# UCL-CCS/SCEMa

Hardware: AMD Instinct MI355X
Metric: stress_evals_per_sec (higher is better)
Workload: dtype f64; 1 GPU; 576 x PE-10368 OPLS replicas per update(), 10+100 MD steps each (dt 2 fs, 300 K, lj/cut/coul/long 12/9 + PPPM 1e-4 + SHAKE + NVT), persistent per-QP state, replica equilibrated for 2000 steps before the timed region; force_field=opls, strain_set=balanced (load/unload: odd updates take the draw with the opposite sign), n_sims=576, atoms_per_replica=10368, sims_on_rank0=576, allgathers=0

## Files before the change

include/scema_md.h:

```cpp
#ifndef SCEMA_MD_H
#define SCEMA_MD_H

#include <stdint.h>

#ifdef __cplusplus
extern "C" {
#endif

#define SCEMA_MD_OK 0
#define SCEMA_MD_ERR_ARG 1
#define SCEMA_MD_ERR_NOSTATE 2
#define SCEMA_MD_ERR_DEVICE 3
#define SCEMA_MD_ERR_BOX 4
#define SCEMA_MD_ERR_IO 5
#define SCEMA_MD_ERR_OVERFLOW 6

#define SCEMA_MD_NPART 8
#define SCEMA_MD_QP_NONE ((int32_t)0xFFFFFFFF)

typedef struct scema_md_engine scema_md_engine;

typedef struct {
  double cut_lj;
  double cut_coul;
// ... 106 lines not shown
int32_t scema_md_local_stress_count(const scema_md_engine *e);
int32_t scema_md_local_result_doubles(const scema_md_engine *e);
int scema_md_copy_local_stress(scema_md_engine *e, void *dst, int32_t dst_on_device);
int scema_md_scatter_gathered(scema_md_engine *e, const double *gathered, scema_mdsim *sims, int32_t n_sims);
int scema_md_settle_update(scema_md_engine *e, int32_t failed);
int64_t scema_md_unsettled_updates(const scema_md_engine *e);

typedef struct scema_plan_dir scema_plan_dir;
scema_plan_dir *scema_plan_dir_create(void);
void scema_plan_dir_destroy(scema_plan_dir *d);
int scema_plan_update(scema_plan_dir *d, const scema_mdsim *sims, int32_t n_sims, const double *cost, int32_t world,
                      int32_t *owner, int32_t *pos, int32_t *cap, int32_t *moves ,
                      int32_t *n_moves, int32_t commit);

int scema_md_has_state(const scema_md_engine *e, int32_t qp_id, const char *matid, int32_t replica);
int scema_md_get_state(scema_md_engine *e, int32_t qp_id, const char *matid, int32_t replica,
                       double box[9], double *x, double *v);
int scema_md_set_state(scema_md_engine *e, int32_t qp_id, const char *matid, int32_t replica,
                       const double box[9], const double *x, const double *v);
int scema_md_drop_state(scema_md_engine *e, int32_t qp_id, const char *matid, int32_t replica);
int scema_md_save_state_file(scema_md_engine *e, int32_t qp_id, const char *matid, int32_t replica, const char *path);
int scema_md_load_state_file(scema_md_engine *e, int32_t qp_id, const char *matid, int32_t replica, const char *path);
int scema_md_save_state_lammps(scema_md_engine *e, int32_t qp_id, const char *matid, int32_t replica, const char *path,
                               double timestep, int64_t ntimestep);

int scema_md_save_state_dump(scema_md_engine *e, int32_t qp_id, const char *matid, int32_t replica, const char *path,
                             int64_t ntimestep, int32_t precise);

typedef struct {
  double timestep_length;
  double temperature;
  int32_t nsteps_sample;
  double strain_ampl;
  double strain_rate;
} scema_md_eqparams;
int scema_md_init_material(scema_md_engine *e, const char *matid, int32_t replica, const scema_md_eqparams *p,
                           double length[3], double stress[6], double stiff[36]);

typedef struct {
  int32_t nsteps_equil;
  double timestep_length;
  double temperature;
  int64_t seed;
} scema_md_equilparams;
int scema_md_equilibrate(scema_md_engine *e, const char *matid, int32_t replica, const scema_md_equilparams *p, double length[3],
                         double *info);

int scema_md_debug_minimize(scema_md_engine *e, int32_t qp_id, const char *matid, int32_t replica, double etol, double ftol,
                            int32_t maxiter, int32_t maxeval, double *info);
int scema_md_debug_run_nh(scema_md_engine *e, int32_t qp_id, const char *matid, int32_t replica, int32_t nsteps, double dt,
                          double t_start, double t_stop, int32_t npt, double p_target, double p_period, double *lavg);
int scema_md_debug_compute(scema_md_engine *e, int32_t qp_id, const char *matid, int32_t replica, int32_t use_shake,
                           double *f, double *energies, double *virials, double *info );
int scema_md_debug_run(scema_md_engine *e, int32_t qp_id, const char *matid, int32_t replica, int32_t nsteps,
                       double dt, double temperature, int32_t nvt, int32_t use_shake, const double *rates,
                       double *press_avg);

int scema_md_reax_configure(scema_md_engine *e, const char *ffield_path, const char *const *elements, int32_t n_elements,
                            double qeq_tol, double skin);
int scema_md_reax_activate(scema_md_engine *e, int32_t on);
int scema_md_reax_set(scema_md_engine *e, int32_t exact_gradient, int32_t terms, int32_t qeq_maxiter);
int scema_md_reax_concurrency(scema_md_engine *e, int32_t halves, int32_t overlap);
int scema_md_batch_split(scema_md_engine *e, int32_t on);
int scema_md_get_concurrency(const scema_md_engine *e, int32_t *out);
int scema_md_pppm_tiling(scema_md_engine *e, int32_t mode, int32_t lds_bytes);
int scema_md_pppm_paths(const scema_md_engine *e, int32_t out[8]);
int scema_md_pppm_tile_shape(const int32_t grid[3], int32_t lds_bytes, int32_t which , int32_t out[4]);
int scema_md_pppm_plan_count(const scema_md_engine *e);
int scema_md_reax_debug_compute(scema_md_engine *e, int32_t qp_id, const char *matid, int32_t replica, double *f, double *eparts,
                                double *virial, double *q, double *info);
int scema_md_reax_stats(const scema_md_engine *e, double *out);

int scema_md_sw_configure(scema_md_engine *e, const char *matid, const char *sw_path, const char *const *elements, int32_t n_elements,
                          int32_t energy_unit, double skin);
int scema_md_sw_debug_compute(scema_md_engine *e, int32_t qp_id, const char *matid, int32_t replica, double *f, double *e2, double *e3,
                              double *virial, double *info);
int scema_md_sw_read_params(const char *sw_path, const char *const *elements, int32_t n_elements, int32_t energy_unit, int32_t *n_kept,
                            int32_t *type_map, double *values, char *errbuf, int32_t errcap);

int scema_md_tersoff_configure(scema_md_engine *e, const char *matid, const char *path, const char *const *elements, int32_t n_elements,
                               int32_t energy_unit, double skin);
int scema_md_tersoff_debug_compute(scema_md_engine *e, int32_t qp_id, const char *matid, int32_t replica, double *f, double *e_rep,
                                   double *e_att, double *virial, double *info);
int scema_md_tersoff_read_params(const char *path, const char *const *elements, int32_t n_elements, int32_t energy_unit, int32_t *n_kept,
                                 int32_t *type_map, double *values, char *errbuf, int32_t errcap);

int scema_md_tersoff_mod_configure(scema_md_engine *e, const char *matid, const char *path, const char *const *elements, int32_t n_elements,
                                   int32_t energy_unit, double skin);
int scema_md_tersoff_mod_debug_compute(scema_md_engine *e, int32_t qp_id, const char *matid, int32_t replica, double *f, double *e_rep,
                                       double *e_att, double *virial, double *info);
int scema_md_tersoff_zbl_configure(scema_md_engine *e, const char *matid, const char *path, const char *const *elements, int32_t n_elements,
                                   int32_t energy_unit, double skin);
int scema_md_tersoff_zbl_debug_compute(scema_md_engine *e, int32_t qp_id, const char *matid, int32_t replica, double *f, double *e_rep,
                                       double *e_att, double *virial, double *info);
int scema_md_tersoff_mod_read_params(const char *path, const char *const *elements, int32_t n_elements, int32_t energy_unit, int32_t *n_kept,
                                     int32_t *type_map, double *values, char *errbuf, int32_t errcap);
int scema_md_tersoff_zbl_read_params(const char *path, const char *const *elements, int32_t n_elements, int32_t energy_unit, int32_t *n_kept,
                                     int32_t *type_map, double *values, char *errbuf, int32_t errcap);

int scema_md_eam_configure(scema_md_engine *e, const char *matid, const char *path, const char *const *elements, int32_t n_elements,
                           int32_t energy_unit, double skin);
int scema_md_eam_debug_compute(scema_md_engine *e, int32_t qp_id, const char *matid, int32_t replica, double *f, double *e_pair,
                               double *e_embed, double *virial, double *info);
int scema_md_eam_read_setfl(const char *path, const char *const *elements, int32_t n_elements, int32_t energy_unit, int32_t *n_kept,
                            int32_t *type_map, double *head, double *masses, double *tables, int64_t tables_cap, char *errbuf, int32_t errcap);

// ... 48 lines not shown
```

scema_amd/capi.py:

```python
from __future__ import annotations

import ctypes as C
import os

import numpy as np

_HERE = os.path.dirname(os.path.abspath(__file__))
LIB_PATH = os.path.join(_HERE, os.environ.get("SCEMA_MD_LIB") or ("libscema_md_asan.so" if os.environ.get("SCEMA_SANITIZE") == "1" else "libscema_md.so"))

NPART = 8
PARTS = ["lj", "coul", "bond", "angle", "dihedral", "improper", "kspace", "shake"]
QP_NONE = -1

SYMBOLS = [
    "scema_md_default_params", "scema_md_create", "scema_md_destroy", "scema_md_last_error",
    "scema_md_register_replica", "scema_md_load_replica_file", "scema_md_write_replica_file",
    "scema_md_load_lammps_data", "scema_md_convert_lammps_data",
    "scema_md_probe_lammps_restart", "scema_md_read_lammps_restart_atoms", "scema_md_load_lammps_restart",
    "scema_md_convert_lammps_restart", "scema_md_write_lammps_restart",
    "scema_md_strain_batch", "scema_md_strain", "scema_md_local_stress_device_ptr",
    "scema_md_local_stress_count", "scema_md_local_result_doubles", "scema_md_copy_local_stress", "scema_md_scatter_gathered", "scema_md_settle_update", "scema_md_has_state", "scema_md_get_state",
    "scema_md_set_state", "scema_md_drop_state", "scema_md_save_state_file", "scema_md_load_state_file", "scema_md_save_state_lammps",
    "scema_md_init_material", "scema_md_debug_compute", "scema_md_debug_run", "scema_md_get_profile", "scema_md_env_overrides",
    "scema_md_comm_unique_id", "scema_md_comm_init_rccl", "scema_md_comm_init_host", "scema_md_comm_destroy",
    "scema_md_comm_world", "scema_md_comm_rank", "scema_md_comm_stats", "scema_md_comm_handshakes", "scema_md_state_owner", "scema_md_last_plan",
    "scema_plan_dir_create", "scema_plan_dir_destroy", "scema_plan_update", "scema_md_kspace_setup",
    "scema_md_save_state_dump", "scema_md_replica_natoms", "scema_md_save_replica_file", "scema_md_equilibrate", "scema_md_debug_minimize", "scema_md_debug_run_nh",
    "scema_md_reax_configure", "scema_md_reax_activate", "scema_md_reax_set", "scema_md_reax_concurrency", "scema_md_batch_split", "scema_md_get_concurrency", "scema_md_pppm_plan_count", "scema_md_pppm_tiling", "scema_md_pppm_paths", "scema_md_pppm_tile_shape", "scema_md_unsettled_updates", "scema_md_reax_debug_compute", "scema_md_reax_stats", "scema_md_box_fma_tflops",
    "scema_md_sw_configure", "scema_md_sw_debug_compute", "scema_md_sw_read_params",
    "scema_md_tersoff_configure", "scema_md_tersoff_debug_compute", "scema_md_tersoff_read_params",
    "scema_md_eam_configure", "scema_md_eam_debug_compute", "scema_md_eam_read_setfl",
    "scema_md_tersoff_mod_configure", "scema_md_tersoff_mod_debug_compute", "scema_md_tersoff_mod_read_params",
    "scema_md_tersoff_zbl_configure", "scema_md_tersoff_zbl_debug_compute", "scema_md_tersoff_zbl_read_params",
    "scema_md_vashishta_configure", "scema_md_vashishta_debug_compute", "scema_md_vashishta_read_params",
    "scema_md_adp_configure", "scema_md_adp_debug_compute", "scema_md_adp_read_setfl",
]
COMM_ID_BYTES = 128
HOST_ALLGATHER_FN = C.CFUNCTYPE(C.c_int, C.c_void_p, C.c_void_p, C.c_void_p, C.c_int64)
HOST_SEND_FN = C.CFUNCTYPE(C.c_int, C.c_void_p, C.c_void_p, C.c_int64, C.c_int32)
HOST_RECV_FN = C.CFUNCTYPE(C.c_int, C.c_void_p, C.c_void_p, C.c_int64, C.c_int32)


class EquilParams(C.Structure):
    _fields_ = [("nsteps_equil", C.c_int32), ("timestep_length", C.c_double), ("temperature", C.c_double), ("seed", C.c_int64)]


class Params(C.Structure):
    _fields_ = [("cut_lj", C.c_double), ("cut_coul", C.c_double), ("skin", C.c_double), ("neigh_delay", C.c_int32),
                ("kspace_accuracy", C.c_double), ("shake_tol", C.c_double), ("shake_maxiter", C.c_int32),
                ("shake_mass", C.c_double), ("t_period", C.c_double), ("t_chain", C.c_int32), ("device", C.c_int32),
                ("max_batch", C.c_int32), ("profile", C.c_int32), ("kspace_style", C.c_int32)]


_P = C.c_void_p


class System(C.Structure):
    _fields_ = [("natoms", C.c_int32), ("ntypes", C.c_int32), ("type", _P), ("charge", _P), ("mass", _P),
                ("eps", _P), ("sigma", _P),
                ("nbonds", C.c_int32), ("nbondtypes", C.c_int32), ("bond_atoms", _P), ("bond_type", _P), ("bond_coeff", _P),
                ("nangles", C.c_int32), ("nangletypes", C.c_int32), ("angle_atoms", _P), ("angle_type", _P), ("angle_coeff", _P),
                ("ndihedrals", C.c_int32), ("ndihedraltypes", C.c_int32), ("dihedral_atoms", _P), ("dihedral_type", _P),
                ("dihedral_coeff", _P),
                ("nimpropers", C.c_int32), ("nimpropertypes", C.c_int32), ("improper_atoms", _P), ("improper_type", _P),
                ("improper_coeff", _P),
                ("special_lj", C.c_double * 3), ("special_coul", C.c_double * 3), ("box", C.c_double * 9), ("x", _P), ("v", _P)]


class MDSim(C.Structure):
    _fields_ = [("qp_id", C.c_int32), ("most_recent_qp_id", C.c_int32), ("replica", C.c_int32), ("material", C.c_int32),
                ("matid", C.c_char_p), ("time_id", C.c_char_p), ("output_folder", C.c_char_p),
                ("restart_folder", C.c_char_p), ("scripts_folder", C.c_char_p), ("log_file", C.c_char_p),
                ("force_field", C.c_char_p),
                ("strain", C.c_double * 6), ("stiffness", C.c_double * 36),
                ("timestep_length", C.c_double), ("temperature", C.c_double), ("strain_rate", C.c_double),
                ("nsteps_sample", C.c_int32), ("output_homog", C.c_int32), ("checkpoint", C.c_int32),
# ... 264 lines not shown
        return bool(lib().scema_md_has_state(self.h, C.c_int32(qp), matid.encode(), C.c_int32(replica)))

    def natoms(self, matid, replica) -> int:
        if (matid, replica) not in self._natoms:
            n = int(lib().scema_md_replica_natoms(self.h, matid.encode(), C.c_int32(replica)))
            if n <= 0:
                raise EngineError(f"replica {matid}_{replica} is not registered")
            self._natoms[(matid, replica)] = n
        return self._natoms[(matid, replica)]

    def get_state(self, qp, matid, replica):
        n = self.natoms(matid, replica)
        box = np.zeros(9); x = np.zeros((n, 3)); v = np.zeros((n, 3))
        self._chk(lib().scema_md_get_state(self.h, C.c_int32(qp), matid.encode(), C.c_int32(replica), _p(box), _p(x), _p(v)))
        return box, x, v

    def set_state(self, qp, matid, replica, box, x, v):
        box = np.ascontiguousarray(box, np.float64); x = np.ascontiguousarray(x, np.float64); v = np.ascontiguousarray(v, np.float64)
        self._chk(lib().scema_md_set_state(self.h, C.c_int32(qp), matid.encode(), C.c_int32(replica), _p(box), _p(x), _p(v)))

    def drop_state(self, qp, matid, replica):
        self._chk(lib().scema_md_drop_state(self.h, C.c_int32(qp), matid.encode(), C.c_int32(replica)))

    def save_state_file(self, qp, matid, replica, path):
        self._chk(lib().scema_md_save_state_file(self.h, C.c_int32(qp), matid.encode(), C.c_int32(replica), path.encode()))

    def save_state_lammps(self, qp, matid, replica, path, timestep=2.0, ntimestep=0):
        self._chk(lib().scema_md_save_state_lammps(self.h, C.c_int32(qp), matid.encode(), C.c_int32(replica), path.encode(),
                                                   C.c_double(timestep), C.c_int64(ntimestep)))

    def save_state_dump(self, qp, matid, replica, path, ntimestep=0, precise=True):
        self._chk(lib().scema_md_save_state_dump(self.h, C.c_int32(qp), matid.encode(), C.c_int32(replica), path.encode(), C.c_int64(ntimestep),
                                                 C.c_int32(1 if precise else 0)))

    def load_state_file(self, qp, matid, replica, path):
        self._chk(lib().scema_md_load_state_file(self.h, C.c_int32(qp), matid.encode(), C.c_int32(replica), path.encode()))

    def debug_compute(self, matid, replica, qp=QP_NONE, use_shake=False):
        n = self._natoms[(matid, replica)]
        f = np.zeros((n, 3)); e = np.zeros(NPART); w = np.zeros((NPART, 6)); info = np.zeros(8)
        self._chk(lib().scema_md_debug_compute(self.h, C.c_int32(qp), matid.encode(), C.c_int32(replica),
                                               C.c_int32(1 if use_shake else 0), _p(f), _p(e), _p(w), _p(info)))
        return f, e, w, dict(g_ewald=info[0], nk=int(info[1]), npairs=info[2], tdof=info[3], t_current=info[4],
                             maxneigh_seen=int(info[5]), maxneigh=int(info[6]), nclus=int(info[7]))

    def debug_run(self, matid, replica, nsteps, dt, temperature, qp=QP_NONE, nvt=True, use_shake=True, rates=None, sample=False):
        r = None if rates is None else np.ascontiguousarray(rates, np.float64)
        pavg = np.zeros(6) if sample else None
        self._chk(lib().scema_md_debug_run(self.h, C.c_int32(qp), matid.encode(), C.c_int32(replica), C.c_int32(nsteps),
                                           C.c_double(dt), C.c_double(temperature), C.c_int32(1 if nvt else 0),
                                           C.c_int32(1 if use_shake else 0), _p(r), _p(pavg)))
        return pavg

    def init_material(self, matid, replica, dt=2.0, temperature=300.0, nss=100, strain_ampl=0.005, strain_rate=1e-4):
        p = EqParams(dt, temperature, nss, strain_ampl, strain_rate)
        length, stress, stiff = np.zeros(3), np.zeros(6), np.zeros(36)
        self._chk(lib().scema_md_init_material(self.h, matid.encode(), C.c_int32(replica), C.byref(p), _p(length), _p(stress), _p(stiff)))
        return length, stress, stiff.reshape(6, 6)

    def reax_configure(self, ffield: str, elements=("H", "C", "N", "O"), qeq_tol: float = 1e-6, skin: float = -1.0):
        arr = (C.c_char_p * len(elements))(*[e.encode() for e in elements])
        self._chk(lib().scema_md_reax_configure(self.h, ffield.encode(), arr, C.c_int32(len(elements)), C.c_double(qeq_tol), C.c_double(skin)))

    def reax_activate(self, on: bool = True):
        self._chk(lib().scema_md_reax_activate(self.h, C.c_int32(1 if on else 0)))

    def reax_set(self, exact_gradient: int = -1, terms: int = -1, qeq_maxiter: int = -1):
        self._chk(lib().scema_md_reax_set(self.h, C.c_int32(exact_gradient), C.c_int32(terms), C.c_int32(qeq_maxiter)))

    def reax_concurrency(self, halves: int = -1, overlap: int = -1):
        self._chk(lib().scema_md_reax_concurrency(self.h, C.c_int32(halves), C.c_int32(overlap)))

    def unsettled_updates(self) -> int:
        lib().scema_md_unsettled_updates.restype = C.c_int64
        return int(lib().scema_md_unsettled_updates(self.h))

    def batch_split(self, on: int = -1):
        self._chk(lib().scema_md_batch_split(self.h, C.c_int32(on)))

    def pppm_plan_count(self) -> int:
        lib().scema_md_pppm_plan_count.restype = C.c_int
        return int(lib().scema_md_pppm_plan_count(self.h))

    def pppm_tiling(self, mode: int = -1, lds_bytes: int = -1):
        self._chk(lib().scema_md_pppm_tiling(self.h, C.c_int32(mode), C.c_int32(lds_bytes)))

    def pppm_paths(self) -> dict:
        out = (C.c_int32 * 8)()
        self._chk(lib().scema_md_pppm_paths(self.h, out))
        return dict(spread=int(out[0]), force=int(out[1]), spread_tiles=(int(out[2]), int(out[3])), force_tiles=(int(out[4]), int(out[5])),
                    lds_bytes=int(out[6]), mode=int(out[7]))

    def concurrency(self) -> dict:
        out = (C.c_int32 * 3)()
        self._chk(lib().scema_md_get_concurrency(self.h, out))
        return dict(split=int(out[0]), reax_halves=int(out[1]), reax_overlap=int(out[2]))

    def reax_compute(self, matid, replica, qp=QP_NONE):
        n = self._natoms[(matid, replica)]
        f = np.zeros((n, 3)); e = np.zeros(len(REAX_PARTS)); w = np.zeros(6); q = np.zeros(n); info = np.zeros(6)
        self._chk(lib().scema_md_reax_debug_compute(self.h, C.c_int32(qp), matid.encode(), C.c_int32(replica), _p(f), _p(e), _p(w), _p(q), _p(info)))
        return dict(f=f, e=dict(zip(REAX_PARTS, e)), w=w, q=q, maxneigh_seen=int(info[0]), maxnb=int(info[1]), maxbd=int(info[2]),
                    qeq_iters=int(info[3]), image_search=int(info[4]), maxbonds_seen=int(info[5]))

    def _row_configure(self, symbol, matid, path, elements, energy_unit, skin):
        arr = (C.c_char_p * len(elements))(*[e.encode() for e in elements])
# ... 275 lines not shown
```

scema_amd/csrc/engine/engine.h:

```cpp
#pragma once
#include <hip/hip_runtime.h>
#include <rccl/rccl.h>

#include <algorithm>
#include <cmath>
#include <cstdarg>
#include <cstdio>
#include <cstdlib>
#include <chrono>
#include <thread>
#include <cstring>
#include <ctime>
#include <array>
#include <atomic>
#include <functional>
#include <map>
#include <memory>
#include <sstream>
#include <fstream>
#include <string>
#include <vector>

#include "../../../include/scema_md.h"
#include "host/reax_ffield.h"
// ... 112 lines not shown
  double skin_extra = 0.0;
  DevBuf qhist;
  bool qhist_valid = false;
};

struct RxSlot {
  int cap_pad = 0, cap_nb = 0, cap_bd = 0, cap_nbn = 0;
  size_t cap_col = 0;
  DevBuf nbn_cnt, nbn, nbnT, qpart, pm_len, pm_col, pm_raw, pm_val;
  DevBuf nb_cnt, nb_own0, nbT, hval, hcol, hlen, hown, hownlen, bd_cnt, bd, bd_rev, bd_bop, bd_c, bd_bo, bd_g, bd_cb, deltap, total_bo, cd_delta, hd, q, s, t, s_hist, t_hist, qwork, misc;
};

struct RowSlot {
  int cap_pad = 0;
  size_t cap_rows = 0;
  DevBuf cnt, rows, misc;
  DevBuf fp;
  DevBuf adp;
};

enum class RowKind { Opls, Reax, Sw, Tersoff, Eam, TersoffMod, TersoffZbl, Vashishta, Adp };

struct RowMaterial {
  RowKind kind = RowKind::Sw;
  std::vector<int> type_map;
  double cutmax = 0.0;
  double skin = 1.0;
  long long stamp = 0;
  DevBuf d_tab;
};

struct ListSig {
  bool valid = false;
  RowKind kind = RowKind::Opls;
  unsigned long long topo = 0;
  unsigned long long state = 0;
  int npad = 0;
  double rlist = 0.0;
  int nc[3] = {0, 0, 0}, capj = 0, maxneigh = 0;
  double cut_lj = 0.0, cut_coul = 0.0;
  long long stamp = 0;
  int mimg[3] = {0, 0, 0}, cap[2] = {0, 0};
  double corners_hold[24];
  int ago = 0, maxj_seen = 0;
  unsigned long long nentries = 0, nentries_ref = 0, nrowent = 0;
};
struct Slot {
  std::unique_ptr<RxSlot> rx;
  std::unique_ptr<RowSlot> row;
  ListSig sig;
  int cap_atoms = 0, cap_pad = 0, cap_neigh = 0, cap_cells = 0, cap_k = 0;
  size_t cap_jtab = 0;
  DevBuf virp, virb, fb, fs, slot_of, tile_nj, tile_jtab, tile_order, tile_wstart;
    DevBuf f, xq, stype, perm, slot_tmp, wrapn, xhold, cell_of, ckey, cell_count, cell_start, cell_fill, numneigh, neigh, sfac, kvec,
      xbak, vbak;
};

struct ActiveSim {
  State *st = nullptr;
  int user_index = -1;
  int nsteps = 0;
  double rates[6] = {0, 0, 0, 0, 0, 0};
  double dt = 0, temperature = 0;
  int nts = 0, nss = 0;
  double pavg[6];
  double box0[9], skin0 = 0.0;
};

struct CreatedState { std::string key; std::unique_ptr<State> displaced; };
struct PendingUpdate {
  bool active = false;
  std::vector<ActiveSim> act;
  std::vector<CreatedState> created;
  scema::SimPlan plan;
  std::vector<std::string> dst_keys;
  int rank = 0;
};

struct Comm {
  int kind = 0;
  int rank = 0, world = 1;
  ncclComm_t nccl = nullptr;
  scema_md_host_allgather_fn ag = nullptr;
  scema_md_host_send_fn send = nullptr;
  scema_md_host_recv_fn recv = nullptr;
  void *ctx = nullptr;
  DevBuf d_gather, d_box, d_word;
  std::vector<double> h_gather;
  std::vector<State *> mig_src, mig_dst;
  std::vector<double> h_box;
  long long migrations = 0, allgathers = 0, handshakes = 0;
};

double event_union_ms(const std::vector<hipEvent_t> &ev, size_t n);
struct Profile {
  long long pair_launches = 0;
  double pair_ms = 0, pair_alg_bytes = 0;
  long long pair_sims = 0;
  double pair_union_ms = 0.0, rx_sweep_union_ms = 0.0;
  long long box_flips = 0;
  long long md_steps = 0, neigh_builds = 0, evals = 0;
  double unique_pairs_sum = 0;
  long long unique_pairs_n = 0;
  double skin_sum = 0;
  long long rx_sweep_launches = 0;
  double rx_sweep_ms = 0, rx_sweep_entries = 0, rx_sweep_rows = 0;
  long long rx_sweep_col_bytes = 0, rx_sweep_symmetric = 0;
// ... 119 lines not shown
    ncclResult_t _r = (call);                                                                             \
    if (_r != ncclSuccess) return fail(e, SCEMA_MD_ERR_DEVICE, "%s failed: %s", #call, ncclGetErrorString(_r)); \
  } while (0)

std::string topo_key(const char *matid, int replica);
std::string state_key(int qp, const char *matid, int replica);

template <class T>
int upload(scema_md_engine *e, DevBuf &b, const std::vector<T> &v) {
  HIPCHK(b.ensure(v.size() * sizeof(T)));
  if (!v.empty()) HIPCHK(hipMemcpy(b.p, v.data(), v.size() * sizeof(T), hipMemcpyHostToDevice));
  return SCEMA_MD_OK;
}

int build_topo(scema_md_engine *e, const scema_md_system *s, Topo &t);
void ewald_setup(const scema_md_params &p, const Topo &t, const double *box, EwaldSetup &out, bool g_only = false);
void ewald_tables(EwaldSetup &out);
void pppm_setup_host(const scema_md_params &p, const Topo &t, const double *box, double &g, int pg[3]);
double cached_coul_poly(scema_md_engine *, double g, double rc, double *poly, int *npoly, double *uscale);
void tilt_closest(double tilt[3], double xprd_new, double yprd_new, double xy, double xz, double yz, double xprd, double yprd);
int tilt_flip(const double tilt[3], double xprd, double yprd, double flipped[3], int nflip[3]);
bool deform_trajectory(const double *box0, const double *rates, double dt, int nsteps, double *box_end, std::vector<FlipEvent> &events,
                       std::vector<HostBox> &extremes);
double wall_s();
double round_trip(const char *fmt, double v);
int settle_pending(scema_md_engine *e, bool failed);
int ensure_slot(scema_md_engine *e, Slot &sl, int natoms, int maxneigh, int ncells, int nk, int capj);
int run_phase(scema_md_engine *e, std::vector<ActiveSim> &sims, const RunSpec &spec);
int run_phase_reax(scema_md_engine *e, std::vector<ActiveSim> &sims, const RunSpec &spec);
int prepare_slots(scema_md_engine *e, std::vector<ActiveSim> &sims);
int reupload_scalars(scema_md_engine *e, int ns);
struct Part { int off = 0, n = 0; hipStream_t st = nullptr; };
std::vector<int> batch_order(const std::vector<ActiveSim> &sims, int nparts, const std::function<long(int)> &tie = nullptr);
std::vector<Part> split_parts(int ns, int nparts);
int part_of(const std::vector<Part> &parts, int pos);
int active_prefix(const std::vector<SimDev> &h_sims, const Part &p, int step);
int fork_parts(scema_md_engine *e, const std::vector<Part> &parts, hipEvent_t ev);
int join_parts(scema_md_engine *e, const std::vector<Part> &parts, const hipEvent_t *done);
struct BoxRange {
  std::vector<HostBox> boxes;
  double w[3] = {1e300, 1e300, 1e300};
  double vol_min = 1e300, vol_max = 0.0;
};
bool box_range(const RunSpec &spec, const ActiveSim &A, const double *box, BoxRange &out, std::vector<FlipEvent> &flips);
void sim_common(SimDev &S, const scema_md_params &P, const RunSpec &spec, const ActiveSim &A, const Slot &sl, SimScalars *sc);
int run_minimiser(scema_md_engine *e, const std::vector<int> &order, int maxatoms, const RunSpec &spec, bool stop_on_any_overflow,
                  const std::function<int()> &force, const std::function<int(int)> &map_fault);
using FlipSchedule = std::map<int, std::vector<std::pair<int, int>>>;
FlipSchedule flip_schedule(const std::vector<std::vector<FlipEvent>> &flips, const std::vector<SimDev> &h_sims);
int sum_timed_launches(scema_md_engine *e, size_t n, double &ms, long long &launches, double &union_ms);
int collect_faults(scema_md_engine *e, int ns);
void lists_hold(scema_md_engine *e, const std::vector<ActiveSim> &sims, bool valid, bool counts);
bool keep_list_switch();
void grow_after_overflow(scema_md_engine *e);
int eval_static(scema_md_engine *e, State *s, const RunSpec &spec);

struct RowNeed {
  double rlist = 0.0, skin = 0.0;
  long long stamp = 0;
  int cap[2] = {0, 0};
  int mimg[3] = {0, 0, 0};
};
struct RowRun;
struct RowStage {
  const RowKind kind;
  const int zero_extra;
  RowRun *run = nullptr;
  RowStage(RowKind kind_, int zero_extra_) : kind(kind_), zero_extra(zero_extra_) {}
  virtual ~RowStage() = default;
  virtual int nparts() const = 0;
  virtual int rows(Topo &T, const BoxRange &R, RowNeed &need) = 0;
  virtual int bind(int pos, const ActiveSim &A, Slot &sl, const SimDev &S, const RowNeed &need) = 0;
  virtual int upload() = 0;
  virtual int setup() = 0;
  virtual void forces(hipStream_t st, int pos0, int n, int step, int part) = 0;
  virtual int part_streams(std::vector<Part> &parts, std::vector<hipEvent_t> &done) = 0;
  virtual int read_back() = 0;
  virtual int after_read_back(int fault, double &need) = 0;
  virtual int faults(int fault) = 0;
};
struct RowRun {
  scema_md_engine *e;
  std::vector<ActiveSim> &sims;
  const RunSpec &spec;
  RowStage &stage;
  const int ns;
  std::vector<int> order;
  std::vector<std::vector<FlipEvent>> flips;
  std::vector<Part> parts;
  std::vector<hipEvent_t> done;
  int maxatoms = 0, maxpad = 0, maxsteps = 0;
  bool any_validate = false;
  const SimDev *D = nullptr;

  RowRun(scema_md_engine *e_, std::vector<ActiveSim> &sims_, const RunSpec &spec_, RowStage &stage_)
      : e(e_), sims(sims_), spec(spec_), stage(stage_), ns((int)sims_.size()), flips(sims_.size()) { stage.run = this; }
  int lay_out();
  int lay_out_sim(int pos);
  int setup_step();
  int minimise();
  int make_parts(int nparts);
  void run_steps();
  int read_scalars();
  int finish();
};
int run_rows(scema_md_engine *e, std::vector<ActiveSim> &sims, const RunSpec &spec, RowStage &stage);
// ... 33 lines not shown
```

scema_amd/csrc/engine/engine_core.cpp:

```cpp
#include <algorithm>
#include "engine.h"
#include "../md_env.h"

namespace scema_eng {

int fail(scema_md_engine *e, int code, const char *fmt, ...) {
  char buf[1024];
  va_list ap;
  va_start(ap, fmt);
  vsnprintf(buf, sizeof buf, fmt, ap);
  va_end(ap);
  if (e) e->err = buf;
  return code;
}

std::string topo_key(const char *matid, int replica) { return std::string(matid ? matid : "") + "_" + std::to_string(replica); }
std::string state_key(int qp, const char *matid, int replica) { return std::to_string(qp) + "." + topo_key(matid, replica); }

}

namespace scema_eng {
double event_union_ms(const std::vector<hipEvent_t> &ev, size_t n) {
  if (n == 0) return 0.0;
  std::vector<std::pair<float, float>> iv(n);
  for (size_t l = 0; l < n; l++) {
    float a = 0.f, b = 0.f;
    if (hipEventElapsedTime(&a, ev[0], ev[2 * l]) != hipSuccess || hipEventElapsedTime(&b, ev[0], ev[2 * l + 1]) != hipSuccess) return 0.0;
    iv[l] = {a, b};
  }
  std::sort(iv.begin(), iv.end());
  double total = 0.0;
  float lo = iv[0].first, hi = iv[0].second;
  for (size_t l = 1; l < n; l++) {
    if (iv[l].first > hi) { total += hi - lo; lo = iv[l].first; hi = iv[l].second; }
    else hi = std::max(hi, iv[l].second);
  }
  return total + (hi - lo);
}
}

namespace {
struct EnvSwitch { const char *name, *what; };
const EnvSwitch k_env[] = {
    {"SCEMA_MD_SPLIT", "0: never run a launch group of 9 simulations and more as part batches on streams of their own"},
    {"SCEMA_MD_PARTS", "2-4: this many part batches for every launch group that is split, if it has 2 replicas per part (default: by the size of the group, engine_run.cpp)"},
    {"SCEMA_MD_ONE_STREAM", "no side stream (bonded / k-space chain beside the pair kernel)"},
    {"SCEMA_MD_KEEP_LIST", "0: the sampling run of an evaluation rebuilds its neighbour rows at its start even where those of the straining run still hold"},
    {"SCEMA_MD_SKIN_EXTRA", "list skin = params.skin + this many Angstrom (results do not depend on it)"},
    {"SCEMA_MD_SKIN_ADAPT", "1: per-state adaptation of the extra skin from the rebuild interval (round-1 behaviour)"},
    {"SCEMA_MD_PPPM_SOLVE_WIDE", "1 / 0: the in-LDS PPPM solve with 1 024 threads and three LDS grids / 512 threads and two (default: by batch size)"},
    {"SCEMA_MD_PPPM_SOLVE_TWO", "0 / 1: the in-LDS PPPM solve of the 1 024-thread shape as one / two workgroups per replica, one per transform back (default: two for batches under 8 replicas)"},
    {"SCEMA_MD_PPPM_PADX", "0: the LDS grid of the PPPM spreading kernel without the five pad points per x row (an address addition per stencil point instead of a constant offset)"},
    {"SCEMA_MD_PPPM_FFT", "hipFFT for every PPPM grid (default: grids of up to 2 900 points are solved in LDS)"},
    {"SCEMA_MD_FUSED_TAIL", "0 / 1: force assembly + SHAKE + second kick as three kernels / as k_finish (default: by batch size)"},
    {"SCEMA_MD_BONDED_SIDE", "0: the bonded kernel of a small batch always on the main stream behind the pair kernel (default: behind the PPPM chain on the side stream on steps without a new influence function)"},
    {"SCEMA_MD_SMALL_BATCH_MAX", "largest batch that takes the cell grid with the most cells instead of the largest cells (default: launch groups of up to 31 replicas that run whole, i.e. not as part batches)"},
    {"SCEMA_MD_REBUILD_TOGETHER", "0 / 1: every replica rebuilds its neighbour rows on its own trigger / the replicas of a launch rebuild together as soon as one asks for it (default: together in launches of fewer than 128 replicas)"},
    {"SCEMA_MD_CELL_BUILD", "0: cell binning as k_bin + k_cell_scan + k_cell_fill instead of the one-launch k_cell_build"},
    {"SCEMA_MD_POLY_TOL", "fit target of the real-space Ewald polynomial (default 2e-13); parity tolerances assume the default"},
    {"SCEMA_REAX_DROP_DSBO2", "ReaxFF valence-angle gradient without the dSBO2 term, as USER-REAXC is believed to compute it"},
    {"SCEMA_MD_RX_ITEM_LDS", "0 (test hook): the ReaxFF angle and torsion items add forces and dE/dDelta to the work set with device-wide atomics instead of through a workgroup's LDS tables (replicas too large for the tables do)"},
    {"SCEMA_MD_RX_NEAR_FULL", "1 (test hook): the ReaxFF near rows hold every pair within the 5 A bond cutoff + skin instead of the pairs within reach of their type pair's bond order"},
    {"SCEMA_REAX_SKIN", "ReaxFF list skin in Angstrom"},
    {"SCEMA_REAX_HALVES", "number of part batches a ReaxFF batch runs as, each on its own stream (default 2; 0 or 1: one sequence of launches)"},
    {"SCEMA_REAX_OVERLAP", "0: the bond-order chain of the ReaxFF force stage on the same stream as the charge chain instead of next to it"},
    {"SCEMA_REAX_QEQ_PRECOND", "0: the conjugate gradients of the charge equilibration with the Jacobi preconditioner of fix qeq/reax instead of the bonded-pattern approximate inverse"},
    {"SCEMA_REAX_QEQ_SYM", "0: the matrix of the charge equilibration as full rows (every pair in both rows) instead of each pair once in its owner's row"},
    {"SCEMA_REAX_QEQ_ZLDS", "0: the matrix sweep of the charge equilibration gathers through the caches instead of from an LDS copy"},
    {"SCEMA_REAX_QEQ_LAUNCH", "conjugate-gradient iterations issued as launches per charge solve (default: adaptive)"},
    {"SCEMA_MD_NEIGH_GROW0", "start with undersized neighbour capacities: overflow -> restore -> regrow"},
    {"SCEMA_MD_NEIGH_EXACT", "1: every list build tests its candidates in FP64 at the exact list radius; 0: none does (default: the first build of a run)"},
    {"SCEMA_MD_TEST_FAIL_INCOMING", "rank on which the allocation of a state that migrates in fails (-1: on whichever rank receives one); the failure must reach every rank through the handshake"},
    {"SCEMA_MD_TEST_FAIL_MIGRATE", "<what>[:<rank>] -- an injected failure of the exchange of replica states: dbox / upload (before the handshake: every rank ends the call, nothing is posted), enqueue / group / hostcopy (after it: the exchange is completed, the error travels in the status word of the stress all-gather)"},
    {"SCEMA_MD_TEST_SELF_MOVE", "1 (RCCL, one rank): every simulation that continues from a state held here receives it through ncclSend / ncclRecv from this very rank"},
    {"SCEMA_MD_TEST_QEQ_PRECOND_FAILS", "1: a ReaxFF run whose charge solve uses the approximate-inverse preconditioner reports that it did not converge (the evaluation must come back from its one retry with the Jacobi preconditioner)"},
    {"SCEMA_MD_QCAP16", "capacity of k_neigh_build's group lists in sixteenths of the table: small values force the whole-table walk"},
    {"SCEMA_MD_RX_COL32", "32-bit column indices in the ReaxFF charge matrix whatever the replica size"},
    {"SCEMA_MD_RX_NB_ONCE", "0: the both-ends ReaxFF non-bonded kernel"},
    {"SCEMA_MD_RX_ITEMCAP", "capacity of the work-item lists of the ReaxFF angle and torsion kernels: small values force their in-place path"},
    {"SCEMA_MD_TIMING", "per-chunk wall times and the PAIR_TIMING / PAIR_COUNT counters on stderr"},
};
}

const char *scema_env(const char *name) {
  for (const EnvSwitch &s : k_env)
    if (strcmp(s.name, name) == 0) return getenv(name);
  fprintf(stderr, "[scema_md] environment switch %s is not declared in engine_core.cpp\n", name);
  abort();
}

extern "C" {

int scema_md_env_overrides(char *buf, int cap) {
  std::string out;
  int n = 0;
  for (const EnvSwitch &s : k_env)
    if (const char *v = getenv(s.name)) { out += (n ? "\n" : ""); out += s.name; out += "="; out += v; n++; }
  if (buf && cap > 0) { strncpy(buf, out.c_str(), (size_t)cap - 1); buf[cap - 1] = 0; }
  return n;
}
// ... 137 lines not shown
```

scema_amd/csrc/engine/engine_debug.cpp:

```cpp
#include "engine.h"
#include "../md_env.h"

namespace scema_eng {

void print_run_timing(const scema_md_engine *e, int ns, double layout_ms, double kspace_ms, double box_ms, double grid_ms, double rest_ms) {
  if (!scema_env("SCEMA_MD_TIMING") || ns <= 0) return;
  const SimScalars &c = e->h_sc[0];
  const SimDev &S0 = e->h_sims[0];
  fprintf(stderr, "[scema_md] sim 0: cells %dx%dx%d, j table max %d of %d, row max %d of %d, row entries/cluster %.1f, listed pairs/atom %.1f, builds %d\n",
          S0.nc[0], S0.nc[1], S0.nc[2], c.maxj_seen, S0.capj, c.maxneigh_seen, S0.maxneigh, (double)c.nrowent / (S0.npad / MD_CLUSTER),
          (double)c.nentries / S0.natoms, c.nbuilds);
  fprintf(stderr, "[scema_md] host: %.2f ms laying out %d simulations before the first launch of this run (k-space set-up on host threads %.2f, box range %.2f, cell grid %.2f, rest of the loop %.2f)\n",
          layout_ms, ns, kspace_ms, box_ms, grid_ms, rest_ms);
  fprintf(stderr, "[scema_md] sim 0: far skin band walked on %d of %d steps; list skin %.2f A\n", c.nfar_steps, c.step, S0.skin);
#ifdef PAIR_COUNT
  fprintf(stderr, "[scema_md] k_pair lanes (sim 0, this run): %llu wave-chunks (%llu with work); atom blocks run %llu = %.2f per working chunk, %.1f lanes of 64 in them; "
          "LJ block run in %llu of them with %.1f lanes; coulomb block in %llu with %.1f lanes; pairs inside the LJ cutoff %llu, inside the coulomb cutoff %llu\n",
          c.dbg[0], c.dbg[1], c.dbg[2], (double)c.dbg[2] / std::max(1ull, c.dbg[1]), (double)c.dbg[3] / std::max(1ull, c.dbg[2]), c.dbg[5],
          (double)c.dbg[4] / std::max(1ull, c.dbg[5]), c.dbg[7], (double)c.dbg[6] / std::max(1ull, c.dbg[7]), c.dbg[4], c.dbg[6]);
#endif
#ifdef PAIR_TIMING
  if (c.dbg2[7])
    fprintf(stderr, "[scema_md] k_pppm_solve clocks (sim 0, thread 0, mean per launch): grid in %.0f, forward passes %.0f, spectra %.0f + %.0f, inverse passes %.0f + %.0f, out + sums %.0f\n",
            (double)c.dbg2[0] / c.dbg2[7], (double)c.dbg2[1] / c.dbg2[7], (double)c.dbg2[2] / c.dbg2[7], (double)c.dbg2[4] / c.dbg2[7], (double)c.dbg2[3] / c.dbg2[7],
            (double)c.dbg2[5] / c.dbg2[7], (double)c.dbg2[6] / c.dbg2[7]);
  fprintf(stderr, "[scema_md] k_pair wave clocks (sim 0, mean per wave): prologue %.0f, rows %.0f, barrier wait %.0f, flush %.0f (%llu waves)\n",
          (double)c.dbg[0] / c.dbg[4], (double)c.dbg[1] / c.dbg[4], (double)c.dbg[2] / c.dbg[4], (double)c.dbg[3] / c.dbg[4], c.dbg[4]);
  {
    unsigned long long a[6] = {0, 0, 0, 0, 0, 0};
    for (int i = 0; i < ns; i++) for (int k = 0; k < 6; k++) a[k] += e->h_sc[i].dbg[k];
    if (a[4]) fprintf(stderr, "[scema_md] pair kernel wave clocks (whole batch, mean per wave and tile visit): prologue %.0f, rows %.0f, wait %.0f, flush %.0f (of which staging %.0f) (%llu visits)\n",
                      (double)a[0] / a[4], (double)a[1] / a[4], (double)a[2] / a[4], (double)a[3] / a[4], (double)a[5] / a[4], a[4]);
  }
  if (c.nbuilds > 0) {
    const double nw = (double)c.nbuilds * S0.ncells * MD_TILE_WAVES;
    fprintf(stderr, "[scema_md] k_neigh_build wave clocks (sim 0, mean per wave and build): table %.0f (boxes and runs %.0f, candidates %.0f), rows %.0f, schedule %.0f; %llu waves of %.0f; %.2f rows per wave of %.1f chunks\n",
            (double)c.dbg[5] / nw, (double)c.dbg[8] / nw, (double)(c.dbg[5] - c.dbg[8]) / nw, (double)c.dbg[6] / nw, (double)c.dbg[7] / nw, c.dbg[9], nw,
            (double)c.dbg[11] / nw, (double)c.dbg[10] / std::max(1ull, c.dbg[11]));
    const double nr = (double)std::max(1ull, c.dbg[11]);
    fprintf(stderr, "[scema_md] k_neigh_build per row (sim 0, cycles): set-up %.0f, chunk loop %.0f = %.0f per chunk, row end %.0f; of %.1f chunks %.2f walk exclusion lists, %.2f are own-cell chunks\n",
            (double)c.dbg[12] / nr, (double)c.dbg[13] / nr, (double)c.dbg[13] / std::max(1ull, c.dbg[10]), (double)c.dbg[14] / nr, (double)c.dbg[10] / nr,
            (double)c.dbg[15] / nr, (double)c.dbg[16] / nr);
  }
#endif
}

int debug_state(scema_md_engine *e, int32_t qp_id, const char *matid, int32_t replica, State **out, std::unique_ptr<State> &tmp) {
  Topo *t = find_topo(e, matid, replica);
  if (!t) return fail(e, SCEMA_MD_ERR_NOSTATE, "replica %s_%d not registered", matid, replica);
  if (qp_id == SCEMA_MD_QP_NONE) {
    int rc = make_state(e, t, t->init_box, t->init_x.data(), t->init_v.data(), false, tmp);
    if (rc) return rc;
    *out = tmp.get();
    return SCEMA_MD_OK;
  }
  State *s = find_state(e, qp_id, matid, replica);
  if (!s) return fail(e, SCEMA_MD_ERR_NOSTATE, "no state for qp %d", qp_id);
  *out = s;
  return SCEMA_MD_OK;
}

}

extern "C" {

int scema_md_debug_compute(scema_md_engine *e, int32_t qp_id, const char *matid, int32_t replica, int32_t use_shake, double *f,
                           double *energies, double *virials, double *info) {
  if (e) (void)settle_pending(e, false);
  if (!e) return SCEMA_MD_ERR_ARG;
  HIPCHK(hipSetDevice(e->p.device));
  State *s = nullptr;
  std::unique_ptr<State> tmp;
  int rc = debug_state(e, qp_id, matid, replica, &s, tmp);
  if (rc) return rc;
  RunSpec R;
  R.use_shake = use_shake;
  R.ev_always = 1;
  R.static_only = 1;
  R.nvt = 0;
  if ((rc = eval_static(e, s, R))) return rc;
  const SimScalars &sc = e->h_sc[0];
  if (f) HIPCHK(hipMemcpy(f, e->slots[0]->f.p, 3 * (size_t)s->topo->natoms * 8, hipMemcpyDeviceToHost));
  if (energies) std::memcpy(energies, sc.eng, sizeof sc.eng);
  if (virials) std::memcpy(virials, sc.vir, sizeof sc.vir);
  if (info) {
    info[0] = e->h_sims[0].g_ewald;
    info[1] = e->h_sims[0].nk;
    info[2] = 0.5 * (double)sc.nentries;
    info[3] = e->h_sims[0].tdof;
    info[4] = sc.t_current;
    info[5] = sc.maxneigh_seen;
    info[4] = (double)sc.nrowent;
    info[6] = e->h_sims[0].maxneigh;
    info[7] = s->topo->nclus;
  }
  return SCEMA_MD_OK;
}

int scema_md_debug_run(scema_md_engine *e, int32_t qp_id, const char *matid, int32_t replica, int32_t nsteps, double dt,
                       double temperature, int32_t nvt, int32_t use_shake, const double *rates, double *press_avg) {
  if (e) (void)settle_pending(e, false);
  if (!e || nsteps < 0) return SCEMA_MD_ERR_ARG;
  HIPCHK(hipSetDevice(e->p.device));
  if (qp_id == SCEMA_MD_QP_NONE) return fail(e, SCEMA_MD_ERR_ARG, "debug_run needs a stored state (scema_md_set_state first)");
  State *s = nullptr;
  std::unique_ptr<State> tmp;
  int rc = debug_state(e, qp_id, matid, replica, &s, tmp);
  if (rc) return rc;
  std::vector<ActiveSim> sims(1);
  sims[0].st = s;
  sims[0].nsteps = nsteps;
  sims[0].dt = dt;
  sims[0].temperature = temperature;
  if (rates) for (int k = 0; k < 6; k++) sims[0].rates[k] = rates[k];
  if ((rc = prepare_slots(e, sims))) return rc;
  RunSpec R;
  R.nvt = nvt;
  R.use_shake = use_shake;
  R.deform = rates ? 1 : 0;
  R.sample = press_avg ? 1 : 0;
  rc = run_phase(e, sims, R);
  if (rc) return rc;
  const SimScalars &sc = e->h_sc[0];
  std::memcpy(s->box, sc.box, 9 * sizeof(double));
  if (press_avg) for (int k = 0; k < 6; k++) press_avg[k] = sc.psum[k] / (double)std::max(sc.nsamples, 1);
  return SCEMA_MD_OK;
}

}
```

scema_amd/csrc/engine/engine_rows.cpp:

```cpp
#include "engine.h"
#include "../md_env.h"

namespace scema_eng {

std::vector<int> batch_order(const std::vector<ActiveSim> &sims, int nparts, const std::function<long(int)> &tie) {
  const int ns = (int)sims.size();
  std::vector<int> by_len(ns), order;
  for (int i = 0; i < ns; i++) by_len[i] = i;
  std::stable_sort(by_len.begin(), by_len.end(), [&](int a, int b) {
    if (sims[a].nsteps != sims[b].nsteps) return sims[a].nsteps > sims[b].nsteps;
    return tie && tie(a) < tie(b);
  });
  order.reserve(ns);
  for (int p = 0; p < nparts; p++)
    for (int r = p; r < ns; r += nparts) order.push_back(by_len[r]);
  return order;
}
std::vector<Part> split_parts(int ns, int nparts) {
  std::vector<Part> parts(nparts);
  for (int p = 0, off = 0; p < nparts; p++) {
    parts[p].off = off;
    parts[p].n = (ns - p + nparts - 1) / nparts;
    off += parts[p].n;
  }
// ... 122 lines not shown
  }
  HIPCHK(hipGetLastError());
  int fault = 0;
  for (int i = 0; i < ns; i++) fault |= e->h_sc[i].overflow;
  if (fault & 16) return fail(e, SCEMA_MD_ERR_ARG, "a simulation became unstable during the minimisation (non-finite positions)");
  e->overflow_need_j = e->overflow_need_row = 1.0;
  if (const int rc = map_fault(fault)) return rc;
  if (!done) return fail(e, SCEMA_MD_ERR_ARG, "minimiser did not stop within its evaluation budget");
  return SCEMA_MD_OK;
}

FlipSchedule flip_schedule(const std::vector<std::vector<FlipEvent>> &flips, const std::vector<SimDev> &h_sims) {
  FlipSchedule at;
  for (size_t pos = 0; pos < flips.size(); pos++)
    for (size_t k = 0; k < flips[pos].size(); k++)
      if (flips[pos][k].step < h_sims[pos].nsteps) at[flips[pos][k].step].push_back({(int)pos, (int)k});
  return at;
}

int sum_timed_launches(scema_md_engine *e, size_t n, double &ms, long long &launches, double &union_ms) {
  for (size_t l = 0; l < n; l++) {
    float t = 0.f;
    HIPCHK(hipEventElapsedTime(&t, e->ev_pool[2 * l], e->ev_pool[2 * l + 1]));
    ms += t;
    launches += 1;
  }
  union_ms += event_union_ms(e->ev_pool, n);
  return SCEMA_MD_OK;
}

int collect_faults(scema_md_engine *e, int ns) {
  int fault = 0;
  for (int i = 0; i < ns; i++) {
    fault |= e->h_sc[i].overflow;
    e->prof.neigh_builds += e->h_sc[i].nbuilds;
  }
  return fault;
}

void lists_hold(scema_md_engine *e, const std::vector<ActiveSim> &sims, bool valid, bool counts) {
  for (size_t i = 0; i < sims.size(); i++) {
    ListSig &g = e->slots[i]->sig;
    const SimScalars &c = e->h_sc[i];
    g.valid = valid;
    g.state = sims[i].st->id;
    std::memcpy(g.corners_hold, c.corners_hold, sizeof g.corners_hold);
    g.ago = c.ago;
    if (counts) { g.maxj_seen = c.maxj_seen; g.nentries = c.nentries; g.nentries_ref = c.nentries_ref; g.nrowent = c.nrowent; }
  }
}

bool keep_list_switch() {
  static const bool on = !(scema_env("SCEMA_MD_KEEP_LIST") && atoi(scema_env("SCEMA_MD_KEEP_LIST")) == 0);
  return on;
}

void grow_after_overflow(scema_md_engine *e) {
  if (e->overflow_bits & 4) e->jtab_grow *= std::max(1.25, std::min(8.0, 1.1 * e->overflow_need_j));
  if ((e->overflow_bits & 8) || !(e->overflow_bits & 4)) e->neigh_grow *= std::max(1.5, std::min(8.0, 1.1 * e->overflow_need_row));
}

int eval_static(scema_md_engine *e, State *s, const RunSpec &spec) {
  std::vector<ActiveSim> sims(1);
  sims[0].st = s;
  sims[0].nsteps = 0;
  sims[0].dt = 1.0;
  sims[0].temperature = 300.0;
  int rc = SCEMA_MD_OK;
  for (int attempt = 0; attempt < 6; attempt++) {
    if ((rc = prepare_slots(e, sims))) return rc;
    rc = run_phase(e, sims, spec);
    if (rc != SCEMA_MD_ERR_OVERFLOW) break;
    grow_after_overflow(e);
  }
  return rc;
}


int RowRun::lay_out_sim(int pos) {
  const int i = order[pos];
  ActiveSim &A = sims[i];
  Topo &T = *A.st->topo;
  const SimScalars &hsc = e->h_sc[i];
  BoxRange R;
  if (!box_range(spec, A, hsc.box, R, flips[pos]))
    return fail(e, SCEMA_MD_ERR_BOX, "fix deform is changing yz too much with xy: the strain would tilt yz past half the box");
  RowNeed N;
  int rc = stage.rows(T, R, N);
  if (rc) return rc;
  bool small = false;
  for (int d = 0; d < 3; d++) small = small || R.w[d] < 2.0 * N.rlist;
  for (int d = 0; d < 3; d++) {
    N.mimg[d] = small ? (int)std::ceil(N.rlist / R.w[d]) : 0;
    if (N.mimg[d] > 2) return fail(e, SCEMA_MD_ERR_BOX, "box width %.3f < (cutoff+skin)/2 = %.3f in dim %d", R.w[d], 0.5 * N.rlist, d);
  }
  const int n = T.natoms, npad = (n + 63) / 64 * 64;
  Slot &sl = *e->slots[i];
  ListSig &g = sl.sig;
  const bool keep = spec.keep_list && keep_list_switch() && g.valid && g.kind == stage.kind && g.stamp == N.stamp && g.topo == T.id && g.rlist == N.rlist &&
                    g.npad == npad && (spec.keep_list == 1 || g.state == A.st->id) && !hsc.force_rebuild && !hsc.overflow && N.cap[0] <= g.cap[0] &&
                    N.cap[1] <= g.cap[1] && g.mimg[0] == N.mimg[0] && g.mimg[1] == N.mimg[1] && g.mimg[2] == N.mimg[2];
  if (keep)
    for (int k = 0; k < 2; k++) N.cap[k] = g.cap[k];
  g.valid = false;
  g.kind = stage.kind;
  g.stamp = N.stamp;
  g.topo = T.id;
  g.rlist = N.rlist; g.npad = npad;
  for (int k = 0; k < 2; k++) g.cap[k] = N.cap[k];
  for (int d = 0; d < 3; d++) g.mimg[d] = N.mimg[d];
  if ((rc = ensure_slot(e, sl, n, 64, 1, 0, 64))) return rc;
  SimDev S;
  std::memset(&S, 0, sizeof S);
  S.keep_list = keep ? spec.keep_list : 0;
  any_validate = any_validate || S.keep_list == 2;
  sim_common(S, e->p, spec, A, sl, e->d_sc.as<SimScalars>() + i);
  S.natoms = n; S.npad = npad; S.ntypes = T.ntypes;
  S.use_shake = 0;
  if (spec.minimize) S.min_incremental = 1;
  S.neigh_delay = 0;
  S.tdof = 3.0 * n - 3.0;
  S.skin = N.skin;
  S.far_band = N.skin;
  e->h_zerotab.push_back(MdkZero{sl.wrapn.as<int>(), 3 * (long long)n});
  if ((rc = stage.bind(pos, A, sl, S, N))) return rc;
  e->h_sims[pos] = S;
  maxatoms = std::max(maxatoms, n); maxpad = std::max(maxpad, npad); maxsteps = std::max(maxsteps, A.nsteps);
  return SCEMA_MD_OK;
}

int RowRun::lay_out() {
  e->h_sims.assign(ns, SimDev());
  e->h_zerotab.clear();
  for (int pos = 0; pos < ns; pos++)
    if (const int rc = lay_out_sim(pos)) return rc;
  HIPCHK(e->d_sims.ensure((size_t)ns * sizeof(SimDev)));
  HIPCHK(hipMemcpyAsync(e->d_sims.p, e->h_sims.data(), (size_t)ns * sizeof(SimDev), hipMemcpyHostToDevice, e->stream));
  D = e->d_sims.as<SimDev>();
  if (const int rc = stage.upload()) return rc;
  HIPCHK(e->d_zerotab.ensure(e->h_zerotab.size() * sizeof(MdkZero)));
  HIPCHK(hipMemcpyAsync(e->d_zerotab.p, e->h_zerotab.data(), e->h_zerotab.size() * sizeof(MdkZero), hipMemcpyHostToDevice, e->stream));
  mdk_zero_many(e->stream, e->d_zerotab.as<MdkZero>(), (int)e->h_zerotab.size(), 3 * (long long)maxatoms + stage.zero_extra);
  return SCEMA_MD_OK;
}

int RowRun::setup_step() {
  hipStream_t st = e->stream;
  mdk_phase_init(st, D, ns);
  if (any_validate) mdk_keep_validate(st, D, ns, maxatoms);
  if (const int rc = stage.setup()) return rc;
  stage.forces(st, 0, ns, 0, 0);
  mdk_final_integrate(st, D, ns, maxatoms, 0);
  if (spec.nh) mdk_setup_post_nh(st, D, ns);
  else mdk_setup_post(st, D, ns);
  return SCEMA_MD_OK;
}

int RowRun::minimise() {
  auto force = [&] {
    stage.forces(e->stream, 0, ns, 1, 0);
    return SCEMA_MD_OK;
  };
  auto map_fault = [&](int fault) {
    if (const int rc = stage.faults(fault)) return rc;
    e->overflow_bits = (fault & 1) ? (1 | 8) : 0;
    return (fault & 1) ? SCEMA_MD_ERR_OVERFLOW : SCEMA_MD_OK;
  };
  return run_minimiser(e, order, maxatoms, spec, false, force, map_fault);
}

int RowRun::make_parts(int nparts) {
  parts = split_parts(ns, nparts);
  parts[0].st = e->stream;
  if (nparts > 1) {
    if (const int rc = stage.part_streams(parts, done)) return rc;
    if (!e->row_fork) HIPCHK(hipEventCreateWithFlags(&e->row_fork, hipEventDisableTiming));
// ... 74 lines not shown
```

scema_amd/csrc/engine/engine_run.cpp:

```cpp
#include "engine.h"
#include "../md_env.h"

namespace scema_eng {

static int padded_slots(int natoms, int ncells) { return (natoms + (MD_CLUSTER - 1) * ncells + 255) / 256 * 256; }

int ensure_slot(scema_md_engine *e, Slot &sl, int natoms, int maxneigh, int ncells, int nk, int capj) {
  const int npad = padded_slots(natoms, ncells);
  if (natoms > sl.cap_atoms || npad > sl.cap_pad) {
    HIPCHK(sl.f.ensure(3 * (size_t)natoms * 8));
    HIPCHK(sl.slot_of.ensure((size_t)natoms * 4));
    HIPCHK(sl.fs.ensure(3 * (size_t)npad * 8));
    HIPCHK(sl.fb.ensure(3 * (size_t)npad * 8));
    HIPCHK(sl.virb.ensure(((size_t)natoms / BT_OWNERS + 2) * 6 * 8));
    HIPCHK(sl.tile_order.ensure((size_t)npad * 4));
    HIPCHK(sl.wrapn.ensure(3 * (size_t)natoms * 4));
    HIPCHK(sl.xhold.ensure(3 * (size_t)natoms * 8));
    HIPCHK(sl.cell_of.ensure((size_t)natoms * 4));
    HIPCHK(sl.ckey.ensure((size_t)natoms * 4));
    HIPCHK(sl.slot_tmp.ensure((size_t)npad * 4));
    HIPCHK(sl.xbak.ensure(3 * (size_t)natoms * 8));
    HIPCHK(sl.vbak.ensure(3 * (size_t)natoms * 8));
    HIPCHK(sl.xq.ensure((size_t)npad * 32));
    HIPCHK(sl.stype.ensure((size_t)npad * 4));
    HIPCHK(sl.perm.ensure((size_t)npad * 4));
    HIPCHK(sl.numneigh.ensure((size_t)npad * 4));
    sl.cap_atoms = natoms;
    sl.cap_pad = npad;
    sl.cap_neigh = 0;
  }
  if (maxneigh > sl.cap_neigh || sl.cap_neigh == 0) {
    HIPCHK(sl.neigh.ensure((size_t)maxneigh * (npad / MD_CLUSTER) * 4 + 8192));
    sl.cap_neigh = maxneigh;
  }
  if (ncells + 1 > sl.cap_cells) {
    HIPCHK(sl.cell_count.ensure((size_t)(ncells + 1) * 4));
    HIPCHK(sl.cell_start.ensure((size_t)(ncells + 1) * 4));
    HIPCHK(sl.cell_fill.ensure((size_t)(ncells + 1) * 4));
    HIPCHK(sl.tile_nj.ensure((size_t)(ncells + 1) * 4));
    HIPCHK(sl.tile_wstart.ensure((size_t)(ncells + 1) * 9 * 4));
    HIPCHK(sl.virp.ensure((size_t)(ncells + 1) * MD_TILE_WAVES * 6 * 8));
    sl.cap_cells = ncells + 1;
  }
  if ((size_t)ncells * capj > sl.cap_jtab || sl.cap_jtab == 0) {
    HIPCHK(sl.tile_jtab.ensure((size_t)ncells * capj * 4 + 1024));
    sl.cap_jtab = (size_t)ncells * capj;
  }
  if (nk > sl.cap_k || sl.cap_k == 0) {
    const int kc = std::max(nk, 64);
    HIPCHK(sl.sfac.ensure((size_t)kc * 2 * 8));
    HIPCHK(sl.kvec.ensure((size_t)kc * 4 * 8));
    sl.cap_k = kc;
  }
  return SCEMA_MD_OK;
}

namespace {

constexpr int MAXP = 4;

struct Policy {
  int kspace_threads = 1;
  int nparts = 1;
  int launch = 0;
  bool small_batch = false, nb_together = false, fuse_pack = false, keep_lists = true;
  bool pppm_in_lds = false, pppm_side = false, fused_tail = false, bonded_side = false, recip_side = false;
  bool recip_side_for(int na) const { return recip_side && na >= 16; }
};

Policy plan_launch(const scema_md_engine *e, int ns) {
  static const int parts_env = [] { const char *s = scema_env("SCEMA_MD_PARTS"); return s ? std::min(4, std::max(2, atoi(s))) : 0; }();
  static const int small_max = scema_env("SCEMA_MD_SMALL_BATCH_MAX") ? atoi(scema_env("SCEMA_MD_SMALL_BATCH_MAX")) : -1;
  static const int together_env = scema_env("SCEMA_MD_REBUILD_TOGETHER") ? atoi(scema_env("SCEMA_MD_REBUILD_TOGETHER")) : -1;
  Policy pol;
  pol.kspace_threads = ns >= 64 ? std::max(1, std::min(8, (int)std::thread::hardware_concurrency())) : 1;
  if (e->split_streams && e->stream3 != nullptr && ns >= 9) {
    pol.nparts = parts_env > 0 ? (ns >= 2 * parts_env ? parts_env : 2) : ns < 10 ? 3 : ns < 64 ? 4 : 2;
    if (e->stream2 == nullptr || e->rx_side1 == nullptr) pol.nparts = std::min(pol.nparts, 2);
    pol.nparts = std::max(1, std::min(pol.nparts, ns / 2));
// ... 212 lines not shown
  if (!box_range(spec, A, hsc.box, R, flips[pos]))
    return fail(e, SCEMA_MD_ERR_BOX, "fix deform is changing yz too much with xy: the strain would tilt yz past half the box (a yz flip changes xz by xy, "
                "which LAMMPS refuses while xy is deformed too, as in.strain.lammps always does)");
  SimDev S;
  std::memset(&S, 0, sizeof S);
  if (!e->skin_adapt) A.st->skin_extra = e->skin_extra_fixed;
  for (int d = 0; d < 3; d++)
    if (R.w[d] < 2.0 * (cutmax_all + P.skin + A.st->skin_extra)) A.st->skin_extra = 0.0;
  const double skin_i = P.skin + A.st->skin_extra;
  const double rlist = cutmax_all + skin_i;
  for (int d = 0; d < 3; d++)
    if (R.w[d] < 2.0 * rlist) return fail(e, SCEMA_MD_ERR_BOX, "box width %.3f < 2*(cutoff+skin) = %.3f in dim %d", R.w[d], 2 * rlist, d);
  const auto tl1 = Clock::now();
  Slot &sl = *e->slots[i];
  const ListSig &g = sl.sig;
  const bool may_keep = spec.keep_list && pol.keep_lists && g.valid && g.kind == RowKind::Opls && g.topo == T.id && g.rlist == rlist && g.cut_lj == P.cut_lj &&
                        g.cut_coul == P.cut_coul && (spec.keep_list == 1 || g.state == A.st->id) && !hsc.force_rebuild && !hsc.overflow;
  int capj = 0, maxneigh = 0;
  bool keep = false;
  if (!choose_grid(e, T.natoms, R, rlist, pol.small_batch, may_keep ? &g : nullptr, S, capj, maxneigh, keep))
    return fail(e, SCEMA_MD_ERR_ARG, "the j table of a cell tile (%d entries) does not fit the LDS of the pair kernel (system too dense for the cutoff)", capj);
  S.keep_list = keep ? spec.keep_list : 0;
  L.any_validate = L.any_validate || S.keep_list != 0;
  S.ncells = S.nc[0] * S.nc[1] * S.nc[2];
  const auto tl2 = Clock::now();
  const EwaldSetup &ew = ews[pos];
  if (P.kspace_style == 1 && T.qsqsum > 0.0) {
    for (int d = 0; d < 3; d++) S.pg[d] = -ew.kmaxd[d];
    L.maxgrid = std::max(L.maxgrid, S.pg[0] * S.pg[1] * S.pg[2]);
    if (S.pg[0] < 5) L.padx_ok = false;
    L.maxgridp = std::max(L.maxgridp, (S.pg[0] + 5) * S.pg[1] * S.pg[2]);
    for (int which = 0; which < 2; which++) {
      const PppmTile t = pppm_tile_shape(S.pg[0], S.pg[1], S.pg[2], L.tl.budget, which);
      bool &fits = which ? L.tl_fo_fits : L.tl_sp_fits;
      if (t.ty == 0) { fits = false; continue; }
      int &my = which ? L.tl.fo_ty : L.tl.sp_ty, &mz = which ? L.tl.fo_tz : L.tl.sp_tz, &mt = which ? L.tl.fo_tiles : L.tl.sp_tiles;
      size_t &ml = which ? L.tl.fo_lds : L.tl.sp_lds;
      my = std::max(my, t.ty); mz = std::max(mz, t.tz); mt = std::max(mt, t.ty * t.tz);
      ml = std::max(ml, (size_t)pppm_tile_bytes(S.pg[0], S.pg[1], S.pg[2], t.by, t.bz, which));
    }
  }
  S.nk = (int)ew.kn.size() / 3;
  for (int d = 0; d < 3; d++) S.kmaxd[d] = std::max(ew.kmaxd[d], 0);
  S.g_ewald = ew.g;
  {
    const double perr = cached_coul_poly(e, ew.g, P.cut_coul, S.coul_poly, &S.coul_npoly, &S.coul_uscale);
    if (perr > 1e-12 && !scema_env("SCEMA_MD_POLY_TOL")) return fail(e, SCEMA_MD_ERR_ARG, "real-space Ewald polynomial fit error %.3e too large (g*rc = %.3f)", perr, ew.g * P.cut_coul);
    for (int m = 0; m < MD_MAXPOLY; m++) S.coul_poly_g[m] = S.coul_poly[m] * ew.g;
  }
  {
    const double m = 0.1 * P.skin;
    S.seg_a2 = (P.cut_coul + m) * (P.cut_coul + m);
    S.seg_b2 = (P.cut_lj + m) * (P.cut_lj + m);
    double frac = 0.65;
    S.far_band = frac * skin_i;
    const double cm = std::max(P.cut_coul, P.cut_lj) + S.far_band;
    S.seg_c2 = cm * cm;
  }
  S.natoms = T.natoms;
  S.npad = padded_slots(T.natoms, S.ncells);
  S.ntypes = T.ntypes;
  int rc = ensure_slot(e, sl, T.natoms, maxneigh, S.ncells, S.nk, capj);
  if (rc) return rc;
  S.maxneigh = maxneigh;
  S.capj = capj;
  {
    ListSig &gs = sl.sig;
    gs.valid = false;
    gs.kind = RowKind::Opls;
    gs.topo = T.id;
    for (int d = 0; d < 3; d++) gs.nc[d] = S.nc[d];
    gs.capj = capj; gs.maxneigh = maxneigh; gs.npad = S.npad;
    gs.rlist = rlist; gs.cut_lj = P.cut_lj; gs.cut_coul = P.cut_coul;
  }
  sim_common(S, P, spec, A, sl, e->d_sc.as<SimScalars>() + i);
  S.nbonds = T.nbonds; S.nbonds_noshake = T.nbonds_noshake; S.nangles = T.nangles; S.ndihedrals = T.ndihedrals;
  S.nimpropers = T.nimpropers; S.nspecial = T.nspecial; S.nclus = T.nclus;
  S.use_shake = (spec.use_shake && T.nclus > 0) ? 1 : 0;
  S.neigh_delay = P.neigh_delay;
  S.shake_maxiter = P.shake_maxiter;
  S.tdof = 3.0 * T.natoms - 3.0 - (S.use_shake ? T.ncons : 0);
  S.qsqsum = T.qsqsum; S.qsum = T.qsum;
  S.cut_lj2 = P.cut_lj * P.cut_lj; S.cut_coul2 = P.cut_coul * P.cut_coul; S.rlist2 = rlist * rlist;
  S.skin = skin_i;
  S.rlist_ref2 = (cutmax_all + P.skin) * (cutmax_all + P.skin);
  S.excl_cut2 = std::min(T.excl_cut * T.excl_cut, S.rlist2);
  S.shake_tol = P.shake_tol;
  S.lj = T.d_lj.as<double>();
  S.bt_terms = T.d_bt_terms.as<unsigned long long>(); S.bt_coef = T.d_bt_coef.as<double>(); S.bt_ncoef = T.bt_ncoef;
  for (int k = 0; k < 4; k++) S.bt_cf_off[k] = T.bt_cf_off[k];
  for (int k = 0; k < 6; k++) S.sp_w[k] = T.sp_w[k];
  S.ex_start = T.d_ex_start.as<int>(); S.ex_list = T.d_ex_list.as<int>();
  S.bt_desc = T.d_bt_desc.as<int>(); S.bt_atoms = T.d_bt_atoms.as<int>(); S.bt_rank = T.d_bt_rank.as<int>(); S.bt_ntile = T.bt_ntile;
  S.clus_at = T.d_clus_at.as<int>(); S.clus_n = T.d_clus_n.as<int>(); S.clus_d = T.d_clus_d.as<double>();
  S.free_at = T.d_free_at.as<int>(); S.nfree = T.nfree;
  S.xq = sl.xq.as<double4>(); S.stype = sl.stype.as<int>(); S.perm = sl.perm.as<int>(); S.slot_tmp = sl.slot_tmp.as<int>();
  S.cell_of = sl.cell_of.as<int>(); S.ckey = sl.ckey.as<int>(); S.cell_start = sl.cell_start.as<int>();
  S.cell_fill = sl.cell_fill.as<int>(); S.numneigh = sl.numneigh.as<int>(); S.neigh = sl.neigh.as<int>();
  S.fs = sl.fs.as<double>(); S.fb = sl.fb.as<double>(); S.slot_of = sl.slot_of.as<int>(); S.tile_nj = sl.tile_nj.as<int>(); S.tile_jtab = sl.tile_jtab.as<int>(); S.tile_order = sl.tile_order.as<int>(); S.tile_wstart = sl.tile_wstart.as<int>(); S.virp = sl.virp.as<double>(); S.virb = sl.virb.as<double>();
  S.kvec = sl.kvec.as<double>();
  if (S.nk > 0) {
    std::vector<int> &kpack = e->h_kpack;
    koff[pos] = kpack.size();
    kpack.insert(kpack.end(), ew.kn.begin(), ew.kn.end());
    kpack.insert(kpack.end(), ew.krun.begin(), ew.krun.end());
    while (kpack.size() % 4) kpack.push_back(0);
    kpack.insert(kpack.end(), ew.kgrp.begin(), ew.kgrp.end());
    S.ngrp = (int)ew.kgrp.size() / 8;
    L.maxgrp = std::max(L.maxgrp, S.ngrp);
  }
  e->h_sims[pos] = S;
  t_box += ms_between(tl0, tl1); t_grid += ms_between(tl1, tl2); t_rest += ms_between(tl2, Clock::now());
  L.maxrow = std::max(L.maxrow, maxneigh); L.maxcapj = std::max(L.maxcapj, capj);
  L.maxbt = std::max(L.maxbt, T.bt_ntile); L.maxloc = std::max(L.maxloc, T.bt_maxloc); L.maxcoef = std::max(L.maxcoef, T.bt_ncoef);
  L.maxatoms = std::max(L.maxatoms, S.natoms); L.maxpad = std::max(L.maxpad, S.npad); L.maxcells = std::max(L.maxcells, S.ncells);
  L.maxk = std::max(L.maxk, S.nk);
  L.maxpoly = std::max(L.maxpoly, S.coul_npoly);
  for (int d = 0; d < 3; d++) L.mmax = std::max(L.mmax, S.kmaxd[d] + 1);
  L.maxclus = std::max(L.maxclus, S.use_shake ? S.nclus : 0);
  L.maxunits = std::max(L.maxunits, S.use_shake ? S.nclus + S.nfree : S.natoms);
  L.maxsteps = std::max(L.maxsteps, A.nsteps);
  return SCEMA_MD_OK;
}

int OplsRun::lay_out_kspace() {
  if ((size_t)64 * 3 * L.mmax * 16 + 4096 > 160 * 1024)
    return fail(e, SCEMA_MD_ERR_ARG, "k-space index range (|n| up to %d) too large for the LDS phase tables; raise cut_coul or loosen kspace_accuracy", L.mmax - 1);
  const std::vector<int> &kpack = e->h_kpack;
  HIPCHK(e->d_kpack.ensure(kpack.size() * sizeof(int) + 64));
  if (!kpack.empty()) HIPCHK(hipMemcpyAsync(e->d_kpack.p, kpack.data(), kpack.size() * sizeof(int), hipMemcpyHostToDevice, e->stream));
  for (int pos = 0; pos < ns; pos++) {
    SimDev &S = e->h_sims[pos];
    if (S.nk <= 0) continue;
    const int *base = e->d_kpack.as<int>() + koff[pos];
    S.kn = base;
    S.krun = base + 3 * (size_t)S.nk;
    S.kgrp = base + ((4 * (size_t)S.nk + 3) / 4) * 4;
  }
  if (!L.tl_sp_fits) L.tl.sp_tiles = 0;
  if (!L.tl_fo_fits) L.tl.fo_tiles = 0;
  if (L.maxgrid > 0) {
    const size_t mg = (size_t)L.maxgrid;
    const size_t gfs = mg + ((size_t)L.maxatoms + 1) / 2;
    HIPCHK(e->d_pppm.ensure((size_t)ns * (mg * 4 * sizeof(double2) + gfs * sizeof(double))));
    double *gbase = e->d_pppm.as<double>(), *ebase = gbase + (size_t)ns * mg * 2, *fbase = gbase + (size_t)ns * mg * 8;
    for (int pos = 0; pos < ns; pos++) {
      SimDev &S = e->h_sims[pos];
      S.pgrid = gbase + (size_t)pos * mg * 2;
      S.pfield = ebase + (size_t)pos * mg * 6;
      S.pgstride = (long long)L.maxgrid;
      S.pgf = fbase + (size_t)pos * gfs;
// ... 362 lines not shown
```

scema_amd/csrc/md_equil.hip:

```cpp
#include <hip/hip_runtime.h>

#include "md_device.h"
#include "md_equil.h"
#include "md_types.h"

__device__ inline double pressure_scalar(const SimDev &S, const SimScalars &sc) {
  BoxD b;
  box_derive(sc.box, b);
  double w = 0.0;
  for (int p = 0; p < MD_NPART; p++) w += sc.vir[p * 6] + sc.vir[p * 6 + 1] + sc.vir[p * 6 + 2];
  return (S.tdof * MD_BOLTZ * sc.t_current + w) / (3.0 * b.vol) * MD_NKTV2P;
}
__device__ inline void nhc_press_half(const SimDev &S, SimScalars &sc, double t_target) {
  const int mp = 3;
  const double dt = S.dt, dthalf = 0.5 * dt, dt4 = 0.25 * dt, dt8 = 0.125 * dt, kt = MD_BOLTZ * t_target;
  double kecurrent = 3.0 * sc.omega_mass * sc.omega_dot * sc.omega_dot;
  sc.etap_dotdot[0] = (kecurrent - kt) / sc.etap_mass[0];
  double expfac;
  for (int k = mp - 1; k > 0; k--) {
    expfac = exp(-dt8 * sc.etap_dot[k + 1]);
    sc.etap_dot[k] *= expfac;
    sc.etap_dot[k] += sc.etap_dotdot[k] * dt4;
    sc.etap_dot[k] *= expfac;
  }
// ... 44 lines not shown
  for (int d = 0; d < 3; d++) { sc.lsum[d] = 0.0; sc.lrun[d] = 0.0; }
  sc.nlwin = 0;
  if (S.npt) {
    const double pf2 = S.p_freq * S.p_freq;
    sc.omega_mass = (S.natoms + 1) * kt / pf2;
    for (int k = 0; k < 3; k++) sc.etap_mass[k] = kt / pf2;
    for (int k = 1; k < 3; k++) sc.etap_dotdot[k] = (sc.etap_mass[k - 1] * sc.etap_dot[k - 1] * sc.etap_dot[k - 1] - kt) / sc.etap_mass[k];
  }
}

__global__ void k_pre_nh(const SimDev *sims) {
  const SimDev &S = sims[blockIdx.x];
  SimScalars &sc = *S.sc;
  if (threadIdx.x == 0) {
    sc.step += 1;
    sc.nh_step += 1;
    sc.ago += 1;
    sc.rebuild = sc.force_rebuild;
    sc.force_rebuild = 0;
    sc.check = (sc.ago >= S.neigh_delay) ? 1 : 0;
    if (S.npt) nhc_press_half(S, sc, sc.t_target_now);
    sc.t_target_now = S.t_start + (S.t_stop - S.t_start) * ((double)sc.nh_step / (double)S.nh_total);
    double vs = nhc_half(S, sc);
    sc.dil = 1.0;
    if (S.npt) {
      nh_omega_dot(S, sc);
      const double fp = exp(-0.25 * S.dt * (sc.omega_dot + sc.mtk_term2));
      vs *= fp;
      vs *= fp;
      const double E = exp(0.5 * S.dt * sc.omega_dot);
      sc.dil = E;
      for (int d = 0; d < 3; d++) {
        const double c = 0.5 * (sc.box[d] + sc.box[3 + d]);
        sc.cen[d] = c;
        double lo = sc.box[d], hi = sc.box[3 + d];
        lo = (lo - c) * E + c; hi = (hi - c) * E + c;
        lo = (lo - c) * E + c; hi = (hi - c) * E + c;
        sc.box[d] = lo; sc.box[3 + d] = hi;
      }
      for (int k = 6; k < 9; k++) { sc.box[k] *= E; sc.box[k] *= E; }
    }
    sc.vscale *= vs;
    double c[24];
    box_corners(sc.box, c);
    double d1 = 0.0, d2 = 0.0;
    for (int k = 0; k < 8; k++) {
      const double dx = c[3 * k] - sc.corners_hold[3 * k], dy = c[3 * k + 1] - sc.corners_hold[3 * k + 1], dz = c[3 * k + 2] - sc.corners_hold[3 * k + 2];
      const double d = sqrt(dx * dx + dy * dy + dz * dz);
      if (d > d1) { d2 = d1; d1 = d; }
      else if (d > d2) d2 = d;
    }
    const double delta = 0.5 * (S.skin - (d1 + d2));
    sc.deltasq = (delta > 0.0) ? delta * delta : -1.0;
    const double far = 0.5 * (S.far_band - (d1 + d2));
    sc.far_dsq = (far > 0.0) ? far * far * (1.0 - 1.0e-9) : -1.0;
    sc.need_far = 0;
    for (int k = 0; k < 6; k++) sc.ke[k] = 0.0;
    for (int k = 0; k < MD_NPART * 6; k++) sc.vir[k] = 0.0;
    for (int k = 0; k < MD_NPART; k++) sc.eng[k] = 0.0;
  }
  for (int k = threadIdx.x; k < 2 * S.nk; k += blockDim.x) S.sfac[k] = 0.0;
  for (int k = threadIdx.x; k < S.ncells; k += blockDim.x) S.cell_count[k] = 0;
}

__global__ __launch_bounds__(TPB) void k_initial_integrate_nh(const SimDev *sims) {
  const SimDev &S = sims[blockIdx.y];
  const int i = blockIdx.x * TPB + threadIdx.x;
  if (i >= S.natoms) return;
  SimScalars &sc = *S.sc;
  const double vs = sc.vscale, E = sc.dil;
  const double dtfm = 0.5 * S.dt * MD_FTM2V / S.mass[i];
  double dsq = 0.0, vn[3], xn[3];
  bool sane = true;
#pragma unroll
  for (int k = 0; k < 3; k++) {
    vn[k] = S.v[3 * i + k] * vs + dtfm * S.f[3 * i + k];
    const double x1 = S.npt ? sc.cen[k] + (S.x[3 * i + k] - sc.cen[k]) * E : S.x[3 * i + k];
    const double x2 = x1 + S.dt * vn[k];
    xn[k] = S.npt ? sc.cen[k] + (x2 - sc.cen[k]) * E : x2;
    sane = sane && fabs(xn[k]) < 1.0e8;
  }
  if (!sane) {
    atomicOr(&sc.overflow, 16);
#pragma unroll
    for (int k = 0; k < 3; k++) { vn[k] = 0.0; xn[k] = S.x[3 * i + k]; }
  }
#pragma unroll
  for (int k = 0; k < 3; k++) {
    S.v[3 * i + k] = vn[k];
    S.x[3 * i + k] = xn[k];
    const double d = xn[k] - S.xhold[3 * i + k];
    dsq += d * d;
  }
  if (sc.check && dsq > sc.deltasq) sc.rebuild = 1;
  if (dsq >= sc.far_dsq) sc.need_far = 1;
}

__global__ void k_post_nh(const SimDev *sims) {
  const SimDev &S = sims[blockIdx.x];
  SimScalars &sc = *S.sc;
  if (threadIdx.x != 0) return;
  sc.nfar_steps += sc.need_far;
  double f2 = 1.0;
  if (S.npt) {
    const double fp = exp(-0.25 * S.dt * (sc.omega_dot + sc.mtk_term2));
    f2 *= fp;
    f2 *= fp;
    for (int k = 0; k < 6; k++) sc.ke[k] *= f2 * f2;
  }
  sc.t_current = (sc.ke[0] + sc.ke[1] + sc.ke[2]) / (S.tdof * MD_BOLTZ);
  if (S.npt) nh_omega_dot(S, sc);
  const double ft = nhc_half(S, sc);
  for (int k = 0; k < 6; k++) sc.ke[k] *= ft * ft;
  sc.vscale = f2 * ft;
  if (S.npt) nhc_press_half(S, sc, sc.t_target_now);
  if (S.lavg_nav > 0 && sc.nh_step <= 2 * S.lavg_nav) {
    for (int d = 0; d < 3; d++) sc.lsum[d] += sc.box[3 + d] - sc.box[d];
    if (sc.nh_step % S.lavg_nav == 0) {
      for (int d = 0; d < 3; d++) { sc.lrun[d] += sc.lsum[d] / S.lavg_nav; sc.lsum[d] = 0.0; }
      sc.nlwin += 1;
    }
  }
  if (S.npt)
    for (int d = 0; d < 3; d++) {
      const double r = (sc.box[3 + d] - sc.box[d]) / sc.len0[d];
      if (r > 1.0 + S.box_margin || r < 1.0 - S.box_margin) atomicOr(&sc.overflow, 64);
    }
}

enum { MIN_INIT = 0, MIN_TRIAL = 1, MIN_QUAD = 2, MIN_RESET = 3, MIN_DONE = 4 };
#define MIN_ALPHA_MAX 1.0
#define MIN_ALPHA_REDUCE 0.5
#define MIN_BACKTRACK_SLOPE 0.4
#define MIN_QUADRATIC_TOL 0.1
#define MIN_EMACH 1.0e-8
#define MIN_EPS_QUAD 1.0e-28
#define MIN_EPS_ENERGY 1.0e-8

__global__ void k_min_pre(const SimDev *sims) {
  const SimDev &S = sims[blockIdx.x];
  SimScalars &sc = *S.sc;
  if (threadIdx.x == 0) {
    sc.step += 1;
    sc.ago += 1;
    sc.rebuild = 0;
    sc.check = 1;
    const double delta = 0.5 * S.skin;
    sc.deltasq = delta * delta;
    const double far = 0.5 * S.far_band;
    sc.far_dsq = far * far * (1.0 - 1.0e-9);
    sc.need_far = 0;
    for (int k = 0; k < 6; k++) sc.ke[k] = 0.0;
    for (int k = 0; k < MD_NPART * 6; k++) sc.vir[k] = 0.0;
    for (int k = 0; k < MD_NPART; k++) sc.eng[k] = 0.0;
    for (int k = 0; k < 4; k++) sc.min_dots[k] = 0.0;
    sc.min_alpha_now = sc.min_alpha_next;
    sc.min_alpha_next = (sc.min_phase == MIN_RESET) ? 0.0 : sc.min_alpha;
  }
  for (int k = threadIdx.x; k < 2 * S.nk; k += blockDim.x) S.sfac[k] = 0.0;
  for (int k = threadIdx.x; k < S.ncells; k += blockDim.x) S.cell_count[k] = 0;
}
__global__ __launch_bounds__(TPB) void k_min_move(const SimDev *sims, double *const *x0s, double *const *hs) {
  const SimDev &S = sims[blockIdx.y];
  const int i = blockIdx.x * TPB + threadIdx.x;
  if (i >= S.natoms) return;
  SimScalars &sc = *S.sc;
  if (sc.min_phase == MIN_DONE) return;
  double *x0 = x0s[blockIdx.y], *h = hs[blockIdx.y];
  const double alpha = (sc.min_phase == MIN_RESET) ? 0.0 : sc.min_alpha;
  const double anow = sc.min_newdir ? 0.0 : sc.min_alpha_now;
  double dsq = 0.0;
#pragma unroll
  for (int k = 0; k < 3; k++) {
    if (sc.min_newdir) { x0[3 * i + k] = S.x[3 * i + k]; h[3 * i + k] = S.f[3 * i + k]; }
    const double xn = S.min_incremental ? S.x[3 * i + k] + (alpha - anow) * h[3 * i + k] : x0[3 * i + k] + alpha * h[3 * i + k];
    S.x[3 * i + k] = xn;
    const double d = xn - S.xhold[3 * i + k];
    dsq += d * d;
  }
  if (dsq > sc.deltasq) sc.rebuild = 1;
  if (dsq >= sc.far_dsq) sc.need_far = 1;
}
__global__ __launch_bounds__(TPB) void k_min_reduce(const SimDev *sims, double *const *hs) {
  const SimDev &S = sims[blockIdx.y];
  SimScalars &sc = *S.sc;
  __shared__ double s_red[3][TPB / 64];
  const int i = blockIdx.x * TPB + threadIdx.x;
  double fh = 0.0, ff = 0.0, fm = 0.0;
  if (i < S.natoms) {
    const double *h = hs[blockIdx.y];
#pragma unroll
    for (int k = 0; k < 3; k++) {
      const double f = S.f[3 * i + k];
      fh += f * h[3 * i + k];
      ff += f * f;
      fm = fmax(fm, fabs(f));
    }
  }
  fh = wave_sum(fh); ff = wave_sum(ff);
#pragma unroll
  for (int o = 32; o > 0; o >>= 1) fm = fmax(fm, __shfl_down(fm, o, 64));
  const int lane = threadIdx.x & 63, wave = threadIdx.x >> 6;
  if (lane == 0) { s_red[0][wave] = fh; s_red[1][wave] = ff; s_red[2][wave] = fm; }
  __syncthreads();
  if (threadIdx.x == 0) {
    double a = 0.0, b = 0.0, c = 0.0;
    for (int w = 0; w < TPB / 64; w++) { a += s_red[0][w]; b += s_red[1][w]; c = fmax(c, s_red[2][w]); }
    atomicAdd(&sc.min_dots[0], a);
    atomicAdd(&sc.min_dots[1], b);
    atomicMax((unsigned long long *)&sc.min_dots[2], (unsigned long long)__double_as_longlong(c));
  }
}
__global__ void k_min_decide(const SimDev *sims) {
  const SimDev &S = sims[blockIdx.x];
  SimScalars &sc = *S.sc;
  if (threadIdx.x != 0 || sc.min_phase == MIN_DONE) return;
  double ecurrent = 0.0;
  for (int k = 0; k < MD_NPART; k++) ecurrent += sc.eng[k];
  const double fh = sc.min_dots[0], ff = sc.min_dots[1], fmaxv = sc.min_dots[2];
  sc.min_ecur = ecurrent;
  sc.min_newdir = 0;
  bool accept = false, backtrack = false;
  switch (sc.min_phase) {
    case MIN_INIT:
      sc.min_einit = ecurrent;
      sc.min_eprev = ecurrent;
      sc.min_iter = 0;
      sc.min_neval = 0;
      accept = true;
      break;
    case MIN_TRIAL: {
      sc.min_neval += 1;
      const double delfh = fh - sc.min_fhprev;
      if (fabs(fh) < MIN_EPS_QUAD || fabs(delfh) < MIN_EPS_QUAD) { sc.min_phase = MIN_RESET; sc.min_stop = 4; return; }
// ... 94 lines not shown
```

scema_amd/csrc/md_kernels.h:

```cpp
#pragma once
#include <hip/hip_runtime.h>
struct SimDev;
void mdk_phase_init(hipStream_t st, const SimDev *d, int ns);
void mdk_keep_validate(hipStream_t st, const SimDev *d, int ns, int maxatoms);
void mdk_setup_post(hipStream_t st, const SimDev *d, int ns);
void mdk_pre(hipStream_t st, const SimDev *d, int ns);
void mdk_initial_integrate(hipStream_t st, const SimDev *d, int ns, int maxatoms, bool pack = false);
void mdk_neighbor(hipStream_t st, const SimDev *d, int ns, int maxatoms, int maxpad, int maxcells, int maxrow, int capj, bool pack = true, bool together = false);
void mdk_neigh_build(hipStream_t st, const SimDev *d, int ns, int maxcells, int maxrow, int capj);
size_t mdk_pair_lds_bytes(int capj);
size_t mdk_neigh_lds_bytes(int capj, int maxrow);
void mdk_pair(hipStream_t st, const SimDev *d, int ns, int maxcells, int capj, int vir, int eng, int npoly, int cle = 0);
void mdk_bonded(hipStream_t st, const SimDev *d, int ns, int maxtiles, int maxloc, int maxcoef, int parts);
void mdk_ewald_recip(hipStream_t st, const SimDev *d, int ns, int maxk, int mmax, int maxgrp);
void mdk_ewald_force(hipStream_t st, const SimDev *d, int ns, int maxatoms, int pairvir, int fkeep = 0);
void mdk_shake(hipStream_t st, const SimDev *d, int ns, int maxclus, double dtfsq_scale);
void mdk_finish(hipStream_t st, const SimDev *d, int ns, int maxunits, int pairvir, int fkeep);
void mdk_final_integrate(hipStream_t st, const SimDev *d, int ns, int maxatoms, int kick);
void mdk_post(hipStream_t st, const SimDev *d, int ns, int next_pre = 0);
void mdk_remap(hipStream_t st, const SimDev *d, int ns, int maxatoms);
void mdk_flip(hipStream_t st, const SimDev *sim, double xy, double xz, double yz);
void mdk_phase_end(hipStream_t st, const SimDev *d, int ns, int maxatoms);
struct MdkCopy { const double *src; double *dst; long long n; };
void mdk_copy_many(hipStream_t st, const MdkCopy *tab, int ncopies, long long maxn);
struct MdkZero { int *p; long long n; };
void mdk_zero_many(hipStream_t st, const MdkZero *tab, int nfills, long long maxn);
```

scema_amd/csrc/md_kernels.hip:

```cpp
#include <hip/hip_runtime.h>

#include <algorithm>
#include <cstdlib>

#include "md_device.h"
#include "md_env.h"
#include "md_kernels.h"
#include "md_types.h"


__global__ void k_phase_init(const SimDev *sims) {
  const SimDev &S = sims[blockIdx.x];
  SimScalars &sc = *S.sc;
  if (threadIdx.x == 0) {
    if (!sc.keep_nh)
      for (int k = 0; k <= MD_MAXCHAIN; k++) sc.eta[k] = sc.eta_dot[k] = sc.eta_dotdot[k] = sc.eta_mass[k] = 0.0;
    for (int k = 0; k < 9; k++) { sc.box0[k] = sc.box[k]; sc.box_prev[k] = sc.box[k]; }
    for (int k = 0; k < 6; k++) { sc.psum[k] = 0.0; sc.ke[k] = 0.0; }
    for (int k = 0; k < MD_NPART * 6; k++) sc.vir[k] = 0.0;
    for (int k = 0; k < MD_NPART; k++) sc.eng[k] = 0.0;
    sc.vscale = 1.0;
    sc.nsamples = 0;
    sc.step = 0;
    int keep = S.keep_list && !sc.force_rebuild;
    sc.deltasq = 0.0;
    if (keep) {
      double c[24];
      box_corners(sc.box, c);
      double d1 = 0.0, d2 = 0.0;
      for (int k = 0; k < 8; k++) {
        const double dx = c[3 * k] - sc.corners_hold[3 * k], dy = c[3 * k + 1] - sc.corners_hold[3 * k + 1], dz = c[3 * k + 2] - sc.corners_hold[3 * k + 2];
        const double d = sqrt(dx * dx + dy * dy + dz * dz);
        if (d > d1) { d2 = d1; d1 = d; }
        else if (d > d2) d2 = d;
      }
      const double delta = 0.5 * (S.skin - (d1 + d2));
      if (delta > 0.0) sc.deltasq = delta * delta;
      else keep = 0;
    }
    if (!keep) sc.ago = 0;
    sc.check = 1;
    sc.rebuild = keep ? 0 : 1;
    sc.force_rebuild = 0;
    sc.far_dsq = 1.0e300;
    sc.need_far = keep ? 1 : 0;
    sc.nfar_steps = 0;
#if defined(PAIR_TIMING) || defined(PAIR_COUNT)
    for (int k = 0; k < 20; k++) sc.dbg[k] = 0;
    for (int k = 0; k < 8; k++) sc.dbg2[k] = 0;
#endif
  }
  for (int k = threadIdx.x; k < 2 * S.nk; k += blockDim.x) S.sfac[k] = 0.0;
  for (int k = threadIdx.x; k < S.ncells; k += blockDim.x) S.cell_count[k] = 0;
}

__global__ __launch_bounds__(TPB) void k_keep_validate(const SimDev *sims) {
  const SimDev &S = sims[blockIdx.y];
  if (!S.keep_list) return;
  SimScalars &sc = *S.sc;
  if (sc.rebuild) return;
  const int i = blockIdx.x * TPB + threadIdx.x;
  if (i >= S.natoms) return;
  const double dx = S.x[3 * i] - S.xhold[3 * i], dy = S.x[3 * i + 1] - S.xhold[3 * i + 1], dz = S.x[3 * i + 2] - S.xhold[3 * i + 2];
  if (!(dx * dx + dy * dy + dz * dz <= sc.deltasq)) sc.rebuild = 1;
}

__global__ void k_setup_post(const SimDev *sims) {
  const SimDev &S = sims[blockIdx.x];
  SimScalars &sc = *S.sc;
  if (threadIdx.x == 0) {
    sc.t_current = (sc.ke[0] + sc.ke[1] + sc.ke[2]) / (S.tdof * MD_BOLTZ);
    if (S.nvt) {
      const double tf2 = S.t_freq * S.t_freq;
      sc.eta_mass[0] = S.tdof * MD_BOLTZ * S.t_target / tf2;
      for (int k = 1; k < S.t_chain; k++) sc.eta_mass[k] = MD_BOLTZ * S.t_target / tf2;
      for (int k = 1; k < S.t_chain; k++)
        sc.eta_dotdot[k] = (sc.eta_mass[k - 1] * sc.eta_dot[k - 1] * sc.eta_dot[k - 1] - MD_BOLTZ * S.t_target) / sc.eta_mass[k];
    }
  }
}

__device__ __forceinline__ double corner_disp(const SimScalars &sc, int k) {
  BoxD b;
  box_derive(sc.box, b);
  const int ix = k & 1, iy = (k >> 1) & 1, iz = k >> 2;
  const double dx = b.h[0] * ix + b.h[5] * iy + b.h[4] * iz + b.lo[0] - sc.corners_hold[3 * k];
  const double dy = b.h[1] * iy + b.h[3] * iz + b.lo[1] - sc.corners_hold[3 * k + 1];
  const double dz = b.h[2] * iz + b.lo[2] - sc.corners_hold[3 * k + 2];
  return sqrt(dx * dx + dy * dy + dz * dz);
}
__device__ __forceinline__ void two_largest(const double *d, double &d1, double &d2) {
  d1 = 0.0; d2 = 0.0;
  for (int k = 0; k < 8; k++) {
    if (d[k] > d1) { d2 = d1; d1 = d[k]; }
    else if (d[k] > d2) d2 = d[k];
  }
}
__device__ __forceinline__ void pre_scalars(const SimDev &S, SimScalars &sc, double d1, double d2) {
  {
    sc.step += 1;
    sc.ago += 1;
    sc.rebuild = sc.force_rebuild;
    sc.force_rebuild = 0;
    sc.check = (sc.ago >= S.neigh_delay) ? 1 : 0;
    const double delta = 0.5 * (S.skin - (d1 + d2));
    sc.deltasq = delta > 0.0 ? delta * delta : 0.0;
    const double far = 0.5 * (S.far_band - (d1 + d2));
    sc.far_dsq = (far > 0.0) ? far * far * (1.0 - 1.0e-9) : -1.0;
    sc.need_far = 0;
    if (S.nvt) sc.vscale *= nhc_half(S, sc);
    for (int k = 0; k < 6; k++) sc.ke[k] = 0.0;
    for (int k = 0; k < MD_NPART * 6; k++) sc.vir[k] = 0.0;
    for (int k = 0; k < MD_NPART; k++) sc.eng[k] = 0.0;
  }
}
__device__ __forceinline__ void pre_scalars(const SimDev &S, SimScalars &sc) {
  double d[8], d1, d2;
  for (int k = 0; k < 8; k++) d[k] = corner_disp(sc, k);
  two_largest(d, d1, d2);
  pre_scalars(S, sc, d1, d2);
}
__global__ void k_pre(const SimDev *sims) {
  const SimDev &S = sims[blockIdx.x];
  if (threadIdx.x == 0) pre_scalars(S, *S.sc);
  for (int k = threadIdx.x; k < 2 * S.nk; k += blockDim.x) S.sfac[k] = 0.0;
  for (int k = threadIdx.x; k < S.ncells; k += blockDim.x) S.cell_count[k] = 0;
}

template <bool PACK>
__global__ __launch_bounds__(TPB) void k_initial_integrate(const SimDev *sims) {
  const SimDev &S = sims[blockIdx.y];
  const int i = blockIdx.x * TPB + threadIdx.x;
  if (i >= S.natoms) return;
  SimScalars &sc = *S.sc;
  const double vs = sc.vscale;
  const double dtfm = 0.5 * S.dt * MD_FTM2V / S.mass[i];
  double dsq = 0.0;
  double vn[3], xn[3];
  bool sane = true;
#pragma unroll
  for (int k = 0; k < 3; k++) {
    vn[k] = S.v[3 * i + k] * vs + dtfm * S.f[3 * i + k];
    xn[k] = S.x[3 * i + k] + S.dt * vn[k];
    sane = sane && fabs(xn[k]) < 1.0e8;
  }
  if (!sane) {
    atomicOr(&sc.overflow, 16);
#pragma unroll
    for (int k = 0; k < 3; k++) { vn[k] = 0.0; xn[k] = S.x[3 * i + k]; }
  }
#pragma unroll
  for (int k = 0; k < 3; k++) {
    S.v[3 * i + k] = vn[k];
    S.x[3 * i + k] = xn[k];
    double d = xn[k] - S.xhold[3 * i + k];
    dsq += d * d;
  }
  if (sc.check && dsq > sc.deltasq) sc.rebuild = 1;
  if (dsq >= sc.far_dsq) sc.need_far = 1;
  if (PACK) {
    BoxD b;
    box_derive(sc.box, b);
    const size_t s = (size_t)S.slot_of[i], np = (size_t)S.npad;
    const int w0 = S.wrapn[3 * i], w1 = S.wrapn[3 * i + 1], w2 = S.wrapn[3 * i + 2];
    double *xy = (double *)S.xq + 2 * s, *zq = (double *)S.xq + 2 * np + 2 * s;
    xy[0] = xn[0] - (b.h[0] * w0 + b.h[5] * w1 + b.h[4] * w2);
    xy[1] = xn[1] - (b.h[1] * w1 + b.h[3] * w2);
    zq[0] = xn[2] - (b.h[2] * w2);
    S.fs[s] = 0.0; S.fs[np + s] = 0.0; S.fs[2 * np + s] = 0.0;
  }
}

#define BIN_APT 4
#define BIN_MAXCELLS 2048
__global__ __launch_bounds__(TPB) void k_bin(const SimDev *sims) {
  const SimDev &S = sims[blockIdx.y];
  SimScalars &sc = *S.sc;
  if (!sc.rebuild) return;
  if ((int)(blockIdx.x * TPB * BIN_APT) >= S.natoms) return;
  __shared__ int s_cnt[BIN_MAXCELLS];
  const bool in_lds = S.ncells <= BIN_MAXCELLS;
  if (in_lds) {
    for (int k = threadIdx.x; k < S.ncells; k += TPB) s_cnt[k] = 0;
    __syncthreads();
  }
  if (blockIdx.x == 0 && threadIdx.x == 0) {
    box_corners(sc.box, sc.corners_hold);
    sc.force_rebuild = 0;
    sc.far_dsq = 1.0e300;
    sc.need_far = 0;
  }
  BoxD b;
  box_derive(sc.box, b);
  int nsub[3];
#pragma unroll
  for (int d = 0; d < 3; d++) {
    const double edge = (d == 0 ? b.h[0] : d == 1 ? b.h[1] : b.h[2]) / S.nc[d];
    const int n = (int)ceil(edge / 1.1);
    nsub[d] = n < 2 ? 2 : (n > 16 ? 16 : n);
  }
  for (int u = 0; u < BIN_APT; u++) {
    const int i = (blockIdx.x * BIN_APT + u) * TPB + threadIdx.x;
    if (i >= S.natoms) break;
    double x0 = S.x[3 * i], x1 = S.x[3 * i + 1], x2 = S.x[3 * i + 2];
    S.xhold[3 * i] = x0; S.xhold[3 * i + 1] = x1; S.xhold[3 * i + 2] = x2;
    double d0 = x0 - b.lo[0], d1 = x1 - b.lo[1], d2 = x2 - b.lo[2];
    double l[3];
    l[0] = b.hinv[0] * d0 + b.hinv[5] * d1 + b.hinv[4] * d2;
    l[1] = b.hinv[1] * d1 + b.hinv[3] * d2;
    l[2] = b.hinv[2] * d2;
    int c[3];
    int key = 0;
#pragma unroll
    for (int d = 0; d < 3; d++) {
      double fl = floor(l[d]);
      double w = l[d] - fl;
      if (w >= 1.0) { w = 0.0; fl += 1.0; }
      S.wrapn[3 * i + d] = (int)fl;
      int cc = (int)(w * S.nc[d]);
      if (cc >= S.nc[d]) cc = S.nc[d] - 1;
      if (cc < 0) cc = 0;
      c[d] = cc;
      int sub = (int)((w * S.nc[d] - cc) * nsub[d]);
      sub = sub < 0 ? 0 : (sub > nsub[d] - 1 ? nsub[d] - 1 : sub);
      key |= ((sub & 1) << d) | ((sub & 2) << (d + 2)) | ((sub & 4) << (d + 4)) | ((sub & 8) << (d + 6));
    }
    S.ckey[i] = key;
    const int cell = (c[2] * S.nc[1] + c[1]) * S.nc[0] + c[0];
    S.cell_of[i] = cell;
    if (in_lds) atomicAdd(&s_cnt[cell], 1);
    else atomicAdd(&S.cell_count[cell], 1);
  }
  if (in_lds) {
    __syncthreads();
    for (int k = threadIdx.x; k < S.ncells; k += TPB) {
      const int n = s_cnt[k];
      if (n) atomicAdd(&S.cell_count[k], n);
    }
  }
}

__global__ __launch_bounds__(TPB) void k_cell_scan(const SimDev *sims) {
  const SimDev &S = sims[blockIdx.x];
  SimScalars &sc = *S.sc;
// ... 24 lines not shown
    if (threadIdx.x == TPB - 1) s_base = base + incl;
    __syncthreads();
  }
  if (threadIdx.x == 0) {
    S.cell_start[S.ncells] = s_base;
    sc.ago = 0;
    sc.nbuilds += 1;
    sc.nentries = 0ull;
    if (!(S.rlist_ref2 < S.rlist2) || sc.step == 0) sc.nentries_ref = 0ull;
    sc.nrowent = 0ull;
  }
}

__global__ __launch_bounds__(TPB) void k_cell_fill(const SimDev *sims) {
  const SimDev &S = sims[blockIdx.y];
  if (!S.sc->rebuild) return;
  if ((int)(blockIdx.x * TPB * BIN_APT) >= S.natoms) return;
  __shared__ int s_cnt[BIN_MAXCELLS];
  const bool in_lds = S.ncells <= BIN_MAXCELLS;
  int cell[BIN_APT], rank[BIN_APT];
  if (in_lds) {
    for (int k = threadIdx.x; k < S.ncells; k += TPB) s_cnt[k] = 0;
    __syncthreads();
  }
#pragma unroll
  for (int u = 0; u < BIN_APT; u++) {
    const int i = (blockIdx.x * BIN_APT + u) * TPB + threadIdx.x;
    cell[u] = -1; rank[u] = 0;
    if (i < S.natoms) {
      cell[u] = S.cell_of[i];
      rank[u] = in_lds ? atomicAdd(&s_cnt[cell[u]], 1) : atomicAdd(&S.cell_fill[cell[u]], 1);
    }
  }
  if (in_lds) {
    __syncthreads();
    for (int k = threadIdx.x; k < S.ncells; k += TPB) {
      const int n = s_cnt[k];
      s_cnt[k] = n ? atomicAdd(&S.cell_fill[k], n) : 0;
    }
    __syncthreads();
  }
#pragma unroll
  for (int u = 0; u < BIN_APT; u++) {
    const int i = (blockIdx.x * BIN_APT + u) * TPB + threadIdx.x;
    if (cell[u] >= 0) S.slot_tmp[S.cell_start[cell[u]] + (in_lds ? s_cnt[cell[u]] : 0) + rank[u]] = i;
  }
}

__device__ __forceinline__ void pack_slot(const SimDev &S, int s, int a, double x, double y, double z) {
  double *xy = (double *)S.xq + 2 * (size_t)s, *zq = (double *)S.xq + 2 * (size_t)S.npad + 2 * (size_t)s;
  if (a < 0) { xy[0] = 1.0e15 + 1.0e6 * (double)s; xy[1] = 1.0e15; zq[0] = 1.0e15; zq[1] = 0.0; S.stype[s] = 0; }
  else { xy[0] = x; xy[1] = y; zq[0] = z; zq[1] = S.q[a]; S.stype[s] = S.type[a]; }
  S.fs[s] = 0.0; S.fs[(size_t)S.npad + s] = 0.0; S.fs[2 * (size_t)S.npad + s] = 0.0;
}

#define CB_TPB 1024
#define CB_MAXATOMS 65536
__global__ __launch_bounds__(CB_TPB) void k_cell_build(const SimDev *sims, int coord) {
  const SimDev &S = sims[blockIdx.x];
  SimScalars &sc = *S.sc;
  if (coord > 0) {
    int any = 0;
    for (int j = threadIdx.x; j < coord; j += CB_TPB) any |= sims[j].sc->rebuild;
    any = __syncthreads_or(any);
    if (!any) return;
    if (threadIdx.x == 0) sc.rebuild = 1;
  } else if (!sc.rebuild) return;
  __shared__ int s_cnt[BIN_MAXCELLS], s_start[BIN_MAXCELLS];
  __shared__ int s_wsum[CB_TPB / 64];
  const int ncells = S.ncells, natoms = S.natoms;
  for (int k = threadIdx.x; k < ncells; k += CB_TPB) s_cnt[k] = 0;
  if (threadIdx.x == 0) {
    box_corners(sc.box, sc.corners_hold);
    sc.force_rebuild = 0;
    sc.far_dsq = 1.0e300;
    sc.need_far = 0;
  }
  BoxD b;
  box_derive(sc.box, b);
  int nsub[3];
#pragma unroll
  for (int d = 0; d < 3; d++) {
    const double edge = (d == 0 ? b.h[0] : d == 1 ? b.h[1] : b.h[2]) / S.nc[d];
    const int n = (int)ceil(edge / 1.1);
    nsub[d] = n < 2 ? 2 : (n > 16 ? 16 : n);
  }
  __syncthreads();
  for (int i = threadIdx.x; i < natoms; i += CB_TPB) {
    const double x0 = S.x[3 * i], x1 = S.x[3 * i + 1], x2 = S.x[3 * i + 2];
    S.xhold[3 * i] = x0; S.xhold[3 * i + 1] = x1; S.xhold[3 * i + 2] = x2;
    const double d0 = x0 - b.lo[0], d1 = x1 - b.lo[1], d2 = x2 - b.lo[2];
    double l[3];
    l[0] = b.hinv[0] * d0 + b.hinv[5] * d1 + b.hinv[4] * d2;
    l[1] = b.hinv[1] * d1 + b.hinv[3] * d2;
    l[2] = b.hinv[2] * d2;
    int c[3];
    int key = 0;
#pragma unroll
    for (int d = 0; d < 3; d++) {
      double fl = floor(l[d]);
      double w = l[d] - fl;
      if (w >= 1.0) { w = 0.0; fl += 1.0; }
      S.wrapn[3 * i + d] = (int)fl;
      int cc = (int)(w * S.nc[d]);
      if (cc >= S.nc[d]) cc = S.nc[d] - 1;
      if (cc < 0) cc = 0;
      c[d] = cc;
      int sub = (int)((w * S.nc[d] - cc) * nsub[d]);
      sub = sub < 0 ? 0 : (sub > nsub[d] - 1 ? nsub[d] - 1 : sub);
      key |= ((sub & 1) << d) | ((sub & 2) << (d + 2)) | ((sub & 4) << (d + 4)) | ((sub & 8) << (d + 6));
    }
    S.ckey[i] = key;
    const int cell = (c[2] * S.nc[1] + c[1]) * S.nc[0] + c[0];
    S.cell_of[i] = cell;
    S.slot_of[i] = atomicAdd(&s_cnt[cell], 1);
  }
  __syncthreads();
#ifdef PAIR_WHATIF_TILE_ORDER
  for (int c = threadIdx.x; c < ncells; c += CB_TPB) {
    const int mine = s_cnt[c];
    int rank = 0;
    for (int o = 0; o < ncells; o++) rank += (s_cnt[o] > mine || (s_cnt[o] == mine && o < c)) ? 1 : 0;
    S.cell_fill[rank] = c;
  }
#endif
  {
    const int lane = threadIdx.x & 63, wave = threadIdx.x >> 6;
    const int i0 = 2 * (int)threadIdx.x, i1 = i0 + 1;
    const int n0 = (i0 < ncells) ? s_cnt[i0] : 0, n1 = (i1 < ncells) ? s_cnt[i1] : 0;
    const int v0 = (n0 + MD_CLUSTER - 1) / MD_CLUSTER * MD_CLUSTER, v1 = (n1 + MD_CLUSTER - 1) / MD_CLUSTER * MD_CLUSTER;
// ... 663 lines not shown
      const double *vp = S.virp + (size_t)r * 6;
#pragma unroll
      for (int k = 0; k < 6; k++) pv[k] += vp[k];
    }
    for (int r = blockIdx.x * TPB + threadIdx.x; r < S.bt_ntile; r += nblk * TPB) {
      const double *vp = S.virb + (size_t)r * 6;
#pragma unroll
      for (int k = 0; k < 6; k++) pv[k] += vp[k];
    }
    block_atomic_add<6>(pv, sc.vir + P_LJ * 6, s_red);
  }
  if (S.use_shake) block_atomic_add<6>(sv, sc.vir + P_SHAKE * 6, s_red);
  block_atomic_add<6>(ke, sc.ke, s_red);
}

__device__ __forceinline__ void post_scalars(const SimDev &S, SimScalars &sc);
__global__ void k_post(const SimDev *sims, int next_pre) {
  const SimDev &S = sims[blockIdx.x];
  __shared__ SimScalars s_sc;
  __shared__ int s_more;
  static_assert(sizeof(SimScalars) % 8 == 0 && offsetof(SimScalars, keep_nh) % 4 == 0, "SimScalars is copied in 8- and 4-byte words");
  {
    const unsigned long long *src = (const unsigned long long *)S.sc;
    unsigned long long *dst = (unsigned long long *)&s_sc;
    for (int k = threadIdx.x; k < (int)(sizeof(SimScalars) / 8); k += blockDim.x) dst[k] = src[k];
  }
  __syncthreads();
  __shared__ double s_d[8];
  if (threadIdx.x == 0) {
    post_scalars(S, s_sc);
    s_more = next_pre && s_sc.step < S.nsteps;
  }
  __syncthreads();
  if (s_more) {
    if (threadIdx.x < 8) s_d[threadIdx.x] = corner_disp(s_sc, threadIdx.x);
    __syncthreads();
    if (threadIdx.x == 0) {
      double d1, d2;
      two_largest(s_d, d1, d2);
      pre_scalars(S, s_sc, d1, d2);
    }
  }
  __syncthreads();
  {
    const int *src = (const int *)&s_sc;
    int *dst = (int *)S.sc;
    for (int k = threadIdx.x; k < (int)(offsetof(SimScalars, keep_nh) / 4); k += blockDim.x) dst[k] = src[k];
  }
  if (!s_more) return;
  for (int k = threadIdx.x; k < 2 * S.nk; k += blockDim.x) S.sfac[k] = 0.0;
  for (int k = threadIdx.x; k < S.ncells; k += blockDim.x) S.cell_count[k] = 0;
}
__device__ __forceinline__ void post_scalars(const SimDev &S, SimScalars &sc) {
  sc.nfar_steps += sc.need_far;
  sc.t_current = (sc.ke[0] + sc.ke[1] + sc.ke[2]) / (S.tdof * MD_BOLTZ);
  double f2 = 1.0;
  if (S.nvt) f2 = nhc_half(S, sc);
  sc.vscale = f2;
  for (int k = 0; k < 6; k++) sc.ke[k] *= f2 * f2;
  if (S.nav > 0 && sc.step <= S.nwin * S.nav) {
    BoxD b;
    box_derive(sc.box, b);
    for (int k = 0; k < 6; k++) {
      double w = 0.0;
      for (int p = 0; p < MD_NPART; p++) w += sc.vir[p * 6 + k];
      sc.psum[k] += (sc.ke[k] + w) / b.vol * MD_NKTV2P;
    }
    sc.nsamples += 1;
  }
  if (S.deform) {
    for (int k = 0; k < 9; k++) sc.box_prev[k] = sc.box[k];
    const double t = sc.step * S.dt;
    double nb[9];
    for (int d = 0; d < 3; d++) {
      const double L0 = sc.box0[3 + d] - sc.box0[d];
      nb[d] = sc.box0[d] - 0.5 * L0 * S.rates[d] * t;
      nb[3 + d] = sc.box0[3 + d] + 0.5 * L0 * S.rates[d] * t;
    }
    double tilt[3] = {sc.box0[6] + S.rates[3] * (sc.box0[4] - sc.box0[1]) * t, sc.box0[7] + S.rates[4] * (sc.box0[5] - sc.box0[2]) * t,
                      sc.box0[8] + S.rates[5] * (sc.box0[5] - sc.box0[2]) * t};
    const double xprd_n = nb[3] - nb[0], yprd_n = nb[4] - nb[1];
    const double xprd = sc.box[3] - sc.box[0], yprd = sc.box[4] - sc.box[1];
    const double denom[3] = {xprd_n, xprd_n, yprd_n};
    const double current[3] = {sc.box[6] / xprd, sc.box[7] / xprd, sc.box[8] / yprd};
    for (int i = 0; i < 3; i++) {
      int guard = 0;
      while (tilt[i] / denom[i] - current[i] > 0.0 && guard++ < 64) tilt[i] -= denom[i];
      while (tilt[i] / denom[i] - current[i] < 0.0 && guard++ < 128) tilt[i] += denom[i];
      if (fabs(tilt[i] / denom[i] - 1.0 - current[i]) < fabs(tilt[i] / denom[i] - current[i])) tilt[i] -= denom[i];
    }
    for (int k = 0; k < 6; k++) sc.box[k] = nb[k];
    sc.box[6] = tilt[0]; sc.box[7] = tilt[1]; sc.box[8] = tilt[2];
  }
}

__global__ void k_flip(const SimDev *sim, double xy, double xz, double yz) {
  SimScalars &sc = *sim->sc;
  if (threadIdx.x == 0) {
    sc.box[6] = xy; sc.box[7] = xz; sc.box[8] = yz;
    sc.force_rebuild = 1;
    sc.rebuild = 1;
  }
}

__global__ __launch_bounds__(TPB) void k_remap(const SimDev *sims) {
  const SimDev &S = sims[blockIdx.y];
  if (!S.deform) return;
// ... 110 lines not shown
```

scema_amd/csrc/md_neigh.hip:

```cpp
#include <hip/hip_runtime.h>

#include <cstdlib>
#include <type_traits>

#include "md_env.h"
#include "md_pair_dev.h"

struct ClusterI {
  double x[NI], y[NI], z[NI];
  int atom[NI];
};

extern __shared__ int s_build[];
#define NQ 4
#define NB_MAXRUN 128
#define NB_MAXUNIT 1024
#define NB_UPW 4
#define NB_LISTPAD 256
#define NB_RECPAD 64
#define NB_FAR 1.0e18f

__device__ __forceinline__ float nb_eps(double M, double r2) {
  const double r = sqrt(r2);
  return (float)(1.0001 * 5.9604644775390625e-8 * (96.0 * M * r + 8.0 * r2));
}
__device__ __forceinline__ float nb_up(double t, float eps) { return (float)(t * (1.0 + 2.4e-7)) + eps; }

__global__ __launch_bounds__(TT, 4) void k_neigh_build(const SimDev *__restrict__ sims, int ntiles, int nsims, int capj, int capB, int qcap, int exact_mode) {
  int sim, cell;
  sim = blockIdx.x / ntiles;
  cell = blockIdx.x % ntiles;
  if (sim >= nsims) return;
  const SimDev &S = sims[sim];
  SimScalars &sc = *S.sc;
  if (!sc.rebuild) return;
  if (cell >= S.ncells) return;
#ifdef PAIR_TIMING
  const unsigned long long tb0 = __builtin_readcyclecounter();
#endif
  const int cs = __builtin_amdgcn_readfirstlane(S.cell_start[cell]), ce = __builtin_amdgcn_readfirstlane(S.cell_start[cell + 1]), nown = ce - cs;
  if (nown == 0) {
    if (threadIdx.x == 0) S.tile_nj[cell] = 0;
    return;
  }
  __shared__ double s_shift[27 * 3];
  __shared__ int s_rjb[NB_MAXRUN], s_rlen[NB_MAXRUN], s_rcode[NB_MAXRUN], s_ub[NB_MAXRUN + 1];
  __shared__ unsigned char s_urun[NB_MAXUNIT];
  __shared__ int s_ucnt[2][1 + NQ][TW * NB_UPW];
  __shared__ double s_qbox[NQ][6];
  __shared__ float s_qboxf[NQ][6];
  __shared__ int s_qn[NQ];
  const int capr = capj + NB_RECPAD;
  float *s_rx = (float *)s_build, *s_ry = s_rx + capr, *s_rz = s_ry + capr;
  unsigned short *s_qlist = (unsigned short *)(s_build + 3 * capr) + TW * capB;
  const int lane = lane_id();
  const int wave = __builtin_amdgcn_readfirstlane(threadIdx.x >> 6);
  unsigned short *lb = (unsigned short *)(s_build + 3 * capr) + wave * capB;

  BoxD b;
  box_derive(sc.box, b);
  if (threadIdx.x < 27) {
    const int s0 = threadIdx.x % 3 - 1, s1 = (threadIdx.x / 3) % 3 - 1, s2 = threadIdx.x / 9 - 1;
    s_shift[3 * threadIdx.x + 0] = b.h[0] * s0 + b.h[5] * s1 + b.h[4] * s2;
    s_shift[3 * threadIdx.x + 1] = b.h[1] * s1 + b.h[3] * s2;
    s_shift[3 * threadIdx.x + 2] = b.h[2] * s2;
  }
  const int capjs = S.capj;
  if (threadIdx.x == 32) { s_rx[capjs] = NB_FAR; s_ry[capjs] = NB_FAR; s_rz[capjs] = NB_FAR; }
  const GLOBAL_AS double *xq = as_global((const double *)S.xq);
  const GLOBAL_AS double *zq = xq + 2 * (size_t)S.npad;
  const int nclus_cell = nown / NI;
  if (wave < NQ) {
    const int c_lo = (wave * nclus_cell) / NQ, c_hi = ((wave + 1) * nclus_cell) / NQ;
    double lo[3] = {1e300, 1e300, 1e300}, hi[3] = {-1e300, -1e300, -1e300};
    for (int sl = cs + c_lo * NI + lane; sl < cs + c_hi * NI; sl += 64)
      if (S.perm[sl] >= 0) {
        const double x = xq[2 * (size_t)sl], y = xq[2 * (size_t)sl + 1], z = zq[2 * (size_t)sl];
// ... 112 lines not shown
    unsigned long long m[NB_UPW];
    float xf[NB_UPW], yf[NB_UPW], zf[NB_UPW];
#pragma unroll
    for (int i = 0; i < NB_UPW; i++) {
      xf[i] = (float)(px[i] + (s_shift[3 * cv[i]] - ox)); yf[i] = (float)(py[i] + (s_shift[3 * cv[i] + 1] - oy)); zf[i] = (float)(pz[i] + (s_shift[3 * cv[i] + 2] - oz));
      okq[i] = 0;
#pragma unroll
      for (int q = 0; q < NQ; q++) {
        const float *bq = s_qboxf[q];
        const float ex = fmaxf(0.f, fmaxf(bq[0] - xf[i], xf[i] - bq[3])), ey = fmaxf(0.f, fmaxf(bq[1] - yf[i], yf[i] - bq[4])), ez = fmaxf(0.f, fmaxf(bq[2] - zf[i], zf[i] - bq[5]));
        okq[i] |= (valid[i] && ex * ex + ey * ey + ez * ez < rl2e) ? (1u << q) : 0u;
      }
      ok[i] = valid[i] && (home[i] || okq[i] != 0u);
      m[i] = __ballot(ok[i]);
      const int ui = wave * NB_UPW + i;
      if (lane == 0) s_ucnt[par][0][ui] = __popcll(m[i]);
#pragma unroll
      for (int q = 0; q < NQ; q++) {
        const unsigned long long mq = __ballot((okq[i] >> q) & 1u);
        if (lane == 0) s_ucnt[par][1 + q][ui] = __popcll(mq);
      }
    }
    __syncthreads();
    int ex_c[1 + NQ], tot_c[1 + NQ];
#pragma unroll
    for (int c = 0; c <= NQ; c++) {
      const int v = (lane < TW * NB_UPW) ? s_ucnt[par][c][lane] : 0;
      const int incl = scan32_incl(v);
      ex_c[c] = incl - v;
      tot_c[c] = __builtin_amdgcn_readlane(incl, TW * NB_UPW - 1);
    }
#pragma unroll
    for (int i = 0; i < NB_UPW; i++) {
      const int ui = wave * NB_UPW + i;
      const int pos = nj + __builtin_amdgcn_readlane(ex_c[0], ui) + popc_below(m[i]);
      if (ok[i] && pos < capjs) {
        gj[pos] = jv[i] | (cv[i] << 23) | (tv[i] << 28);
        s_rx[pos] = xf[i]; s_ry[pos] = yf[i]; s_rz[pos] = zf[i];
      }
#pragma unroll
      for (int q = 0; q < NQ; q++) {
        const bool in_q = (okq[i] >> q) & 1u;
        const unsigned long long mq = __ballot(in_q);
        const int lp = qn[q] + __builtin_amdgcn_readlane(ex_c[1 + q], ui) + popc_below(mq);
        if (in_q && lp < qcap) s_qlist[q * qcap + lp] = (unsigned short)(pos | (tv[i] << 12));
      }
    }
    nj += tot_c[0];
#pragma unroll
    for (int q = 0; q < NQ; q++) qn[q] += tot_c[1 + q];
  }
  if (!runs_ok || nj > capjs || nown / NI > 64 * TW) {
    if (threadIdx.x == 0) { S.tile_nj[cell] = 0; atomicOr(&sc.overflow, 1 | 4); atomicMax(&sc.maxj_seen, runs_ok ? nj : 2 * S.capj); }
    for (int cl = cs / NI + threadIdx.x; cl < ce / NI; cl += TT) { S.numneigh[2 * cl] = 0; S.numneigh[2 * cl + 1] = 0; }
    return;
  }
  if (threadIdx.x == 0) { S.tile_nj[cell] = nj; atomicMax(&sc.maxj_seen, nj); }
#pragma unroll
  for (int q = 0; q < NQ; q++) {
    const bool fits = qn[q] + NB_LISTPAD <= qcap;
    if ((int)threadIdx.x == q) s_qn[q] = fits ? qn[q] : -1;
    if (fits && threadIdx.x < NB_LISTPAD) s_qlist[q * qcap + qn[q] + threadIdx.x] = (unsigned short)capjs;
  }
  __builtin_amdgcn_fence(__ATOMIC_RELEASE, "workgroup");
  __syncthreads();

#ifdef PAIR_TIMING
  const unsigned long long tb1 = __builtin_readcyclecounter();
#endif
  const int maxrow = S.maxneigh;
  const double ra2 = S.seg_a2, rb2 = fmax(S.seg_a2, S.seg_b2), rc2 = fmax(rb2, S.seg_c2), excl2 = S.excl_cut2;
  unsigned int npairs = 0, npairs_ref = 0;
  unsigned long long nrowent = 0;
  const bool wider = S.rlist_ref2 < S.rlist2;
  const bool exact = exact_mode == 1 || (exact_mode != 0 && sc.step == 0);
  const bool count_ref = wider && exact && sc.step == 0;
  const float ra2e = nb_up(ra2, eps), rb2e = nb_up(rb2, eps), rc2e = nb_up(rc2, eps), excl2e = nb_up(excl2, eps);
  const GLOBAL_AS int *gjr = (const GLOBAL_AS int *)gj;
  const int capD = capB >> 2, capBC = capB - capD;
  int nmax = 0, over = 0;
  for (int cl = cs / NI + wave; cl < ce / NI; cl += TW) {
    const int s0slot = cl * NI;
#ifdef PAIR_TIMING
    const unsigned long long tr0 = __builtin_readcyclecounter();
    unsigned nslow = 0, nownc = 0;
#endif
    ClusterI ci;
#pragma unroll
    for (int a = 0; a < NI; a++) {
      ci.atom[a] = S.perm[s0slot + a];
      ci.x[a] = XQ_X(S, s0slot + a); ci.y[a] = XQ_Y(S, s0slot + a); ci.z[a] = XQ_Z(S, s0slot + a);
    }
    if (ci.atom[0] < 0) {
      if (lane == 0) { S.numneigh[2 * cl] = 0; S.numneigh[2 * cl + 1] = 0; }
      continue;
    }
    GLOBAL_AS int *row = as_global_w(S.neigh) + (size_t)cl * maxrow;
    int exb[NI], exn[NI];
#pragma unroll
    for (int a = 0; a < NI; a++) {
      exb[a] = (ci.atom[a] >= 0) ? S.ex_start[ci.atom[a]] : 0;
      exn[a] = (ci.atom[a] >= 0) ? S.ex_start[ci.atom[a] + 1] - exb[a] : 0;
    }
    int exv;
    {
      const int a = lane >> 4, e = lane & 15;
      const int na = (a == 0) ? exn[0] : (a == 1) ? exn[1] : (a == 2) ? exn[2] : exn[3];
      const int ba = (a == 0) ? exb[0] : (a == 1) ? exb[1] : (a == 2) ? exb[2] : exb[3];
      exv = (e < na) ? S.slot_of[S.ex_list[ba + e]] : -1;
    }
    const unsigned long long exvalid = __ballot(exv >= 0);
    const bool exlong = max(max(exn[0], exn[1]), max(exn[2], exn[3])) > 16;
    int nA = 0, nB = 0, nC = 0, nD = 0;
    int qq = 0;
#pragma unroll
    for (int q = 1; q < NQ; q++) qq += (cl - cs / NI >= (q * nclus_cell) / NQ) ? 1 : 0;
    const int qnl = s_qn[qq];
    const bool qall = qnl < 0;
    const int nl = qall ? nj : qnl;
    const unsigned short *ql = s_qlist + qq * qcap;
    auto list_at = [&](int k) -> int { return qall ? ((k < nl) ? k : capjs) : (int)ql[k]; };
#ifdef PAIR_TIMING
    if (lane == 0) { atomicAdd(&sc.dbg[10], (unsigned long long)((nl + 63) >> 6)); atomicAdd(&sc.dbg[11], 1ull); }
    __builtin_amdgcn_s_waitcnt(0);
    const unsigned long long tr1 = __builtin_readcyclecounter();
#define NB_T_SLOW() nslow++
#define NB_T_OWN() nownc++
#else
#define NB_T_SLOW()
#define NB_T_OWN()
#endif
    bool own_chunks = true;
    const int dump = maxrow - 64 + lane;
    int posA_prev = dump, entA_prev = 0;
#define NB_CHUNK_TAIL(RMIN, RA, RB, RC, EXCL)                                                                                            \
      const int l = lt & 0xFFF;                                                                                                           \
      const int j = jt & MD_JMASK;                                                                                                        \
      if (own_chunks) {                        \
        NB_T_OWN();                                                                                                                       \
         \
                               \
        const bool own = l < nown;                                                                                                        \
        const int d = j - s0slot;                                                                                                         \
        const int drop = !own ? 0 : (d <= 0 ? 0xF : (d > 3 ? 0 : (0xF << d) & 0xF));                                                      \
        mask &= ~drop; refm &= ~drop;                                                                                                     \
        own_chunks = __ballot(own) != 0ull;                                                                                               \
      }                                                                                                                                   \
       \
         \
            \
               \
               \
                                 \
      if (__ballot(mask != 0 && RMIN < EXCL) != 0ull) {                                                                                   \
        NB_T_SLOW();                                                                                                                      \
        unsigned long long todo = exvalid;                                                                                                \
        while (todo) {                                                                                                                    \
          const int b = __builtin_ctzll(todo);                                                                                            \
          todo &= todo - 1;                                                                                                               \
          const int sp = __builtin_amdgcn_readlane(exv, b);                                                                               \
          const int bit = 1 << (b >> 4);                                                                                                  \
          if (j == sp) { mask &= ~bit; refm &= ~bit; }                      \
        }                                                                                                                                 \
        if (exlong) {            \
          _Pragma("unroll") for (int a = 0; a < NI; a++)                                                                                  \
            for (int e = 16; e < exn[a]; e++)                                                                                             \
              if (S.slot_of[S.ex_list[exb[a] + e]] == j) { mask &= ~(1 << a); refm &= ~(1 << a); }                                        \
        }                                                                                                                                 \
      }                                                                                                                                   \
       \
            \
        \
                          \
      {                                                                                                                                   \
        typedef decltype(RMIN) nb_rm_t;                                                                                                   \
        const nb_rm_t rmx = mask ? RMIN : (nb_rm_t)3.0e38f;                                                                               \
        const bool inA = rmx < RA, inAB = rmx < RB, inABC = rmx < RC, inAll = mask != 0;                                                  \
        const unsigned long long mA = __ballot(inA), mAB = __ballot(inAB), mABC = __ballot(inABC), mAll = __ballot(inAll);                \
        const unsigned long long mB = mAB & ~mA, mC = mABC & ~mAB, mD = mAll & ~mABC;                                                     \
        const int pB = nB + popc_below(mB), pC = capBC - 1 - (nC + popc_below(mC)), pD = capBC + nD + popc_below(mD);                     \
        const int idx = min(max(inAB ? pB : (inABC ? pC : pD), 0), capB - 1);                                                             \
        if (inAll && !inA) lb[idx] = (unsigned short)((base + lane) | (mask << 12));                                                      \
        if (inA) {                                                                                                                        \
          const int pos = nA + popc_below(mA);                                                                                            \
          const int ty = qall ? (int)((unsigned)jt >> 28) : (lt >> 12);                                                                   \
          if (pos < maxrow - 64) { posA_prev = pos; entA_prev = l | (ty << E_TYPE_SHIFT) | (mask << E_MASK_SHIFT); }                      \
        }                                                                                                                                 \
        nA += __popcll(mA); nB += __popcll(mB); nC += __popcll(mC); nD += __popcll(mD);                                                   \
      }                                                                                                                                   \
      npairs += __popc(mask);

    if (exact) {
      int lt_n = list_at(lane);
      int jt_n = (lane < nl) ? gjr[lt_n & 0xFFF] : 0;
      double pn0, pn1, pn2;
      {
        const size_t jn = (size_t)(jt_n & MD_JMASK);
        pn0 = xq[2 * jn]; pn1 = xq[2 * jn + 1]; pn2 = zq[2 * jn];
      }
      auto row_loop = [&](auto cref_tag) __attribute__((always_inline)) {
        constexpr bool CREF = decltype(cref_tag)::value;
        for (int base = 0; base < nl; base += 64) {
          const int lt = lt_n;
          const int jt = jt_n;
          const double px = pn0, py = pn1, pz = pn2;
          row[posA_prev] = entA_prev;
          posA_prev = dump; entA_prev = 0;
          {
            lt_n = list_at(base + 64 + lane);
            jt_n = (base + 64 + lane < nl) ? gjr[lt_n & 0xFFF] : 0;
            const size_t jn = (size_t)(jt_n & MD_JMASK);
            pn0 = xq[2 * jn]; pn1 = xq[2 * jn + 1]; pn2 = zq[2 * jn];
          }
          const bool in = base + lane < nl;
          const int code = (jt >> 23) & 31;
          const double xj = px + s_shift[3 * code], yj = py + s_shift[3 * code + 1], zj = pz + s_shift[3 * code + 2];
          int mask = 0, refm = 0;
          double r2a[NI];
#pragma unroll
          for (int a = 0; a < NI; a++) {
            const double dx = ci.x[a] - xj, dy = ci.y[a] - yj, dz = ci.z[a] - zj;
            const double r2 = dx * dx + dy * dy + dz * dz;
            mask |= (r2 < S.rlist2) ? (1 << a) : 0;
            if (CREF) refm |= (r2 < S.rlist_ref2) ? (1 << a) : 0;
            r2a[a] = r2;
          }
          const double rmin = vmin_f64(vmin_f64(r2a[0], r2a[1]), vmin_f64(r2a[2], r2a[3]));
          if (!in) { mask = 0; refm = 0; }
          NB_CHUNK_TAIL(rmin, ra2, rb2, rc2, excl2)
          if (CREF) npairs_ref += __popc(refm);
        }
      };
      if (count_ref) row_loop(std::true_type{}); else row_loop(std::false_type{});
    } else {
      float cx[NI], cy[NI], cz[NI];
#pragma unroll
      for (int a = 0; a < NI; a++) {
        const bool real = ci.atom[a] >= 0;
        cx[a] = __int_as_float(__builtin_amdgcn_readfirstlane(__float_as_int(real ? (float)(ci.x[a] - ox) : -NB_FAR)));
        cy[a] = __int_as_float(__builtin_amdgcn_readfirstlane(__float_as_int(real ? (float)(ci.y[a] - oy) : -NB_FAR)));
        cz[a] = __int_as_float(__builtin_amdgcn_readfirstlane(__float_as_int(real ? (float)(ci.z[a] - oz) : -NB_FAR)));
      }
      auto process = [&](const int base, const int lt, const int jt, const float xf, const float yf, const float zf) __attribute__((always_inline)) {
        row[posA_prev] = entA_prev;
        posA_prev = dump; entA_prev = 0;
        int mask = 0, refm = 0;
        (void)refm;
        float r2a[NI];
#pragma unroll
        for (int a = 0; a < NI; a++) {
          const float dx = cx[a] - xf, dy = cy[a] - yf, dz = cz[a] - zf;
          const float r2 = dx * dx + dy * dy + dz * dz;
          mask |= (r2 < rl2e) ? (1 << a) : 0;
          r2a[a] = r2;
        }
        const float rmin = vmin3_f32(vmin_f32(r2a[0], r2a[1]), r2a[2], r2a[3]);
        NB_CHUNK_TAIL(rmin, ra2e, rb2e, rc2e, excl2e)
      };
      int ltA = list_at(lane), ltB = list_at(64 + lane);
      float xA = s_rx[ltA & 0xFFF], yA = s_ry[ltA & 0xFFF], zA = s_rz[ltA & 0xFFF];
      int jtA = gjr[ltA & 0xFFF];
      for (int base = 0; base < nl; base += 128) {
        const float xB = s_rx[ltB & 0xFFF], yB = s_ry[ltB & 0xFFF], zB = s_rz[ltB & 0xFFF];
        const int jtB = gjr[ltB & 0xFFF];
        const int ltC = list_at(base + 128 + lane);
        process(base, ltA, jtA, xA, yA, zA);
        xA = s_rx[ltC & 0xFFF]; yA = s_ry[ltC & 0xFFF]; zA = s_rz[ltC & 0xFFF];
        jtA = gjr[ltC & 0xFFF];
        const int ltD = list_at(base + 192 + lane);
        process(base + 64, ltB, jtB, xB, yB, zB);
        ltA = ltC; ltB = ltD;
      }
    }
    row[posA_prev] = entA_prev;
#ifdef PAIR_TIMING
    const unsigned long long tr2 = __builtin_readcyclecounter();
#endif
    const int n = nA + nB + nC + nD;
    const bool bad = nB + nC > capBC || nD > capD || n > maxrow - 64;
    if (bad) over = 1;
    if (!bad) {
      auto expand = [&](int e16) -> int {
        const int lt = list_at(e16 & 0xFFF), l = lt & 0xFFF;
        const int ty = qall ? (int)((unsigned)gjr[l] >> 28) : (lt >> 12);
        return l | (ty << E_TYPE_SHIFT) | ((e16 >> 12) << E_MASK_SHIFT);
      };
      for (int k = lane; k < nB; k += 64) row[nA + k] = expand(lb[k]);
      for (int k = lane; k < nC; k += 64) row[nA + nB + k] = expand(lb[capBC - 1 - k]);
      for (int k = lane; k < nD; k += 64) row[nA + nB + nC + k] = expand(lb[capBC + k]);
      if (n + lane < ((n + 63) & ~63)) row[n + lane] = 0;
    }
    if (lane == 0) {
      S.numneigh[2 * cl] = bad ? 0 : nA + nB + nC; S.numneigh[2 * cl + 1] = bad ? 0 : nD;
    }
    nmax = max(nmax, n);
    nrowent += n;
#ifdef PAIR_TIMING
    __builtin_amdgcn_s_waitcnt(0);
    if (lane == 0) {
      const unsigned long long tr3 = __builtin_readcyclecounter();
      atomicAdd(&sc.dbg[12], tr1 - tr0); atomicAdd(&sc.dbg[13], tr2 - tr1); atomicAdd(&sc.dbg[14], tr3 - tr2);
      atomicAdd(&sc.dbg[15], (unsigned long long)nslow); atomicAdd(&sc.dbg[16], (unsigned long long)nownc);
    }
#endif
  }
#undef NB_CHUNK_TAIL
#undef NB_T_SLOW
#undef NB_T_OWN
#ifdef PAIR_TIMING
  const unsigned long long tb2 = __builtin_readcyclecounter();
#endif
  if (wave == 0) {
    const int c0i = cs / NI, nclus = nown / NI;
    int *wst = S.tile_wstart + (size_t)cell * (TW + 1);
    for (int w = lane; w <= TW; w += 64) {
      int st = 0;
      for (int u = 0; u < w; u++) st += (nclus - u + TW - 1) / TW;
      wst[w] = st;
    }
    for (int i = lane; i < nclus; i += 64) {
      const int w = i % TW;
      int st = 0;
      for (int u = 0; u < w; u++) st += (nclus - u + TW - 1) / TW;
      S.tile_order[2 * c0i + st + i / TW] = (c0i + i) | (16 << 25);
    }
  }
#ifdef PAIR_TIMING
  if (lane == 0) {
    const unsigned long long tb3 = __builtin_readcyclecounter();
    atomicAdd(&sc.dbg[5], tb1 - tb0); atomicAdd(&sc.dbg[6], tb2 - tb1); atomicAdd(&sc.dbg[7], tb3 - tb2);
    atomicAdd(&sc.dbg[8], tb05 - tb0); atomicAdd(&sc.dbg[9], 1ull);
  }
#endif
  {
    const double cnt = wave_sum((double)npairs), cnt_ref = count_ref ? wave_sum((double)npairs_ref) : (wider ? 0.0 : cnt);
    if (lane == 0) {
      atomicAdd(&sc.nentries, 2ull * (unsigned long long)cnt);
      atomicAdd(&sc.nentries_ref, 2ull * (unsigned long long)cnt_ref);
    }
  }
  if (lane == 0) {
    if (over) atomicOr(&sc.overflow, 1 | 8);
    atomicMax(&sc.maxneigh_seen, nmax);
    atomicAdd(&sc.nrowent, nrowent);
  }
}

// ... 25 lines not shown
```

scema_amd/csrc/md_pair.hip:

```cpp
#include <hip/hip_runtime.h>

#include <cstdlib>
#include <type_traits>

#include "md_device.h"
#include "md_env.h"
#include "md_kernels.h"

#include "md_pair_dev.h"

extern __shared__ double s_pair[];

template <bool VIR, bool ENG, int NP, bool CLE = false>
__global__ __launch_bounds__(TT, 4) void k_pair(const SimDev *__restrict__ sims, int ntiles, int nsims, int capj) {
  int sim, cell;
  if (!xcd_map(ntiles, nsims, sim, cell)) return;
  const SimDev &S = sims[sim];
  if (cell >= S.ncells) return;
#ifdef PAIR_WHATIF_TILE_ORDER
  cell = S.cell_fill[cell];
#endif
  const int cs = S.cell_start[cell], ce = S.cell_start[cell + 1];
  if (ce == cs) {
    if (VIR && !ENG && threadIdx.x < TW * 6) S.virp[(size_t)cell * TW * 6 + threadIdx.x] = 0.0;
    return;
  }
  SimScalars &sc = *S.sc;
#ifdef PAIR_TIMING
  const unsigned long long tm0 = __builtin_readcyclecounter();
#endif
  __shared__ double s_shift[27 * 4];
  __shared__ __attribute__((aligned(16))) double s_lj[2 * MD_MAXTYPES * MD_MAXTYPES];
  __shared__ double s_red[8 * TW];
  double *s_f = s_pair;
  int *s_jtab = (int *)(s_pair + 3 * (size_t)capj);
  if (threadIdx.x < 27) {
    BoxD b;
    box_derive(sc.box, b);
    const int s0 = threadIdx.x % 3 - 1, s1 = (threadIdx.x / 3) % 3 - 1, s2 = threadIdx.x / 9 - 1;
    s_shift[4 * threadIdx.x + 0] = b.h[0] * s0 + b.h[5] * s1 + b.h[4] * s2;
    s_shift[4 * threadIdx.x + 1] = b.h[1] * s1 + b.h[3] * s2;
    s_shift[4 * threadIdx.x + 2] = b.h[2] * s2;
    s_shift[4 * threadIdx.x + 3] = 0.0;
  }
  const int nt = S.ntypes, nt2 = nt * nt;
  for (int k = threadIdx.x; k < 2 * nt2; k += TT) s_lj[k] = S.lj[(k & 1) * nt2 + (k >> 1)];
  const int nj = S.tile_nj[cell];
  const int lane = lane_id();
  const int wave = __builtin_amdgcn_readfirstlane(threadIdx.x >> 6);
  const int maxrow = S.maxneigh;
  const int need_far = __builtin_amdgcn_readfirstlane(S.sc->need_far);
  const int p_begin = S.tile_wstart[(size_t)cell * (TW + 1) + wave], p_end = S.tile_wstart[(size_t)cell * (TW + 1) + wave + 1];
  const int nrows = __builtin_amdgcn_readfirstlane((nj > 0) ? min(p_end - p_begin, 64) : 0);
  if (p_end - p_begin > 64 && lane == 0) atomicOr(&sc.overflow, 1 | 4);
  int h_cl = 0, h_nn = 0;
  if (lane < nrows) {
    const int ent = S.tile_order[2 * (cs / NI) + p_begin + lane];
    h_cl = ent & 0xFFFFF;
    const int n = S.numneigh[2 * h_cl] + (need_far ? S.numneigh[2 * h_cl + 1] : 0);
    const int C = (n + 63) >> 6, pa = (ent >> 20) & 31, pb = (ent >> 25) & 31;
    const int kb = 64 * ((C * pa) >> 4), ke = 64 * ((C * pb) >> 4);
    h_nn = (max(ke, kb) << 16) | kb;
  }
#define H_KB(v) ((v) & 0xFFFF)
#define H_KE(v) ((int)((unsigned)(v) >> 16))
  const GLOBAL_AS int *neigh = as_global(S.neigh);
  int pr = 0;
  int pcl = __builtin_amdgcn_readlane(h_cl, 0), pnn = __builtin_amdgcn_readlane(h_nn, 0);
  int pk = H_KB(pnn);
  pnn = H_KE(pnn);
  const unsigned lane4 = 4u * (unsigned)lane;
  auto fetch = [&]() -> int {
    int v = 0;
    if (pr < nrows) {
      const GLOBAL_AS char *row = (const GLOBAL_AS char *)(neigh + (size_t)pcl * maxrow);
      if (pk < pnn) v = *(const GLOBAL_AS int *)(row + (4u * (unsigned)pk + lane4));
      pk += 64;
      if (pk >= pnn) {
        pr += 1;
        const int q = min(pr, nrows - 1);
        pcl = __builtin_amdgcn_readlane(h_cl, q); pnn = __builtin_amdgcn_readlane(h_nn, q);
        pk = H_KB(pnn);
        pnn = H_KE(pnn);
      }
    }
    return v;
  };
  int e_n = 0, e_nn = 0;
  if (nrows > 0) { e_n = fetch(); e_nn = fetch(); }
  {
    const GLOBAL_AS int *gj = as_global(S.tile_jtab) + (size_t)cell * S.capj;
    for (int l = threadIdx.x; l < nj; l += TT) {
      s_jtab[l] = gj[l];
      s_f[3 * l] = 0.0; s_f[3 * l + 1] = 0.0; s_f[3 * l + 2] = 0.0;
    }
  }
  double cp[NP];
#pragma unroll
  for (int m = 0; m < NP; m++) cp[m] = S.coul_poly_g[m];
  double cp_top = cp[NP - 1];
  asm volatile("" : "+v"(cp_top));
  __syncthreads();
  const GLOBAL_AS double *xq = as_global((const double *)S.xq);
  const GLOBAL_AS double *zq = xq + 2 * (size_t)S.npad;
  const double g = S.g_ewald, g2u = g * g * S.coul_uscale;
  const double cutc2 = S.cut_coul2, cutl2 = S.cut_lj2;
  const double cutmax2 = fmax(cutc2, cutl2);
  double vl[6] = {0, 0, 0, 0, 0, 0}, vc[6] = {0, 0, 0, 0, 0, 0};
  double elj = 0, ecoul = 0;
#ifdef PAIR_TIMING
  const unsigned long long tm1 = __builtin_readcyclecounter();
#endif
// ... 189 lines not shown
        vl[3] = fma(px, ay, vl[3]); vl[4] = fma(px, az, vl[4]); vl[5] = fma(py, az, vl[5]);
      }
    }
  }
  {
    double *fs = S.fs;
    const size_t np = (size_t)S.npad;
    for (int l = threadIdx.x; l < nj; l += TT) {
      const double ax = s_f[3 * l], ay = s_f[3 * l + 1], az = s_f[3 * l + 2];
      if (ax != 0.0 || ay != 0.0 || az != 0.0) {
        const size_t slot = (size_t)(s_jtab[l] & MD_JMASK);
#if defined(PAIR_WHATIF_NOFLUSH)
        if (ax == 1.2345e300) fs[slot] = ax;
#elif defined(PAIR_WHATIF_STOREFLUSH)
        fs[slot] = ax; fs[np + slot] = ay; fs[2 * np + slot] = az;
#else
        atomicAdd(fs + slot, ax); atomicAdd(fs + np + slot, ay); atomicAdd(fs + 2 * np + slot, az);
#endif
      }
    }
  }
  if (VIR && !ENG) {
    double *vp = S.virp + ((size_t)cell * TW + wave) * 6;
#pragma unroll
    for (int k = 0; k < 6; k++) {
      const double t = wave_sum(vl[k]);
      if (lane == 0) vp[k] = t;
    }
  }
#ifdef PAIR_TIMING
  {
    __builtin_amdgcn_s_waitcnt(0);
    const unsigned long long tm4 = __builtin_readcyclecounter();
    if (lane == 0) {
      atomicAdd(&sc.dbg[0], tm1 - tm0); atomicAdd(&sc.dbg[1], tm2 - tm1); atomicAdd(&sc.dbg[2], tm3 - tm2);
      atomicAdd(&sc.dbg[3], tm4 - tm3); atomicAdd(&sc.dbg[4], 1ull);
    }
  }
#endif
  if (VIR && ENG) {
    tile_atomic_add<6>(vl, sc.vir + P_LJ * 6, s_red);
    tile_atomic_add<6>(vc, sc.vir + P_COUL * 6, s_red);
  }
  if (ENG) {
    double e1[1];
    e1[0] = elj;
    tile_atomic_add<1>(e1, sc.eng + P_LJ, s_red);
    e1[0] = ecoul;
    tile_atomic_add<1>(e1, sc.eng + P_COUL, s_red);
  }
}


size_t mdk_pair_lds_bytes(int capj) { return (size_t)capj * (3 * sizeof(double) + sizeof(int)); }
template <bool VIR, bool ENG, int NP, bool CLE = false>
static void launch_pair_v(hipStream_t st, const SimDev *d, int ns, int ntiles, int capj) {
  const size_t lds = mdk_pair_lds_bytes(capj);
  static size_t optin_tab[16] = {0};
  size_t &optin = lds_optin_slot(optin_tab);
  if (lds > 48 * 1024 && lds > optin) { (void)hipFuncSetAttribute((const void *)k_pair<VIR, ENG, NP, CLE>, hipFuncAttributeMaxDynamicSharedMemorySize, (int)lds); optin = lds; }
  hipLaunchKernelGGL((k_pair<VIR, ENG, NP, CLE>), grid_xcd(ntiles, ns), dim3(TT), lds, st, d, ntiles, ns, capj);
}

template <int NP>
static void launch_pair(hipStream_t st, const SimDev *d, int ns, int ntiles, int capj, int vir, int eng, int cle) {
  if (eng) launch_pair_v<true, true, NP>(st, d, ns, ntiles, capj);
  else if (vir) { if (cle) launch_pair_v<true, false, NP, true>(st, d, ns, ntiles, capj); else launch_pair_v<true, false, NP>(st, d, ns, ntiles, capj); }
  else { if (cle) launch_pair_v<false, false, NP, true>(st, d, ns, ntiles, capj); else launch_pair_v<false, false, NP>(st, d, ns, ntiles, capj); }
}

void mdk_pair(hipStream_t st, const SimDev *d, int ns, int maxcells, int capj, int vir, int eng, int npoly, int cle) {
  if (npoly <= 6) launch_pair<6>(st, d, ns, maxcells, capj, vir, eng, cle);
  else if (npoly <= 8) launch_pair<8>(st, d, ns, maxcells, capj, vir, eng, cle);
  else if (npoly <= 10) launch_pair<10>(st, d, ns, maxcells, capj, vir, eng, cle);
  else if (npoly <= 12) launch_pair<12>(st, d, ns, maxcells, capj, vir, eng, cle);
  else if (npoly <= 14) launch_pair<14>(st, d, ns, maxcells, capj, vir, eng, cle);
  else if (npoly <= 15) launch_pair<15>(st, d, ns, maxcells, capj, vir, eng, cle);
  else if (npoly <= 16) launch_pair<16>(st, d, ns, maxcells, capj, vir, eng, cle);
  else if (npoly <= 18) launch_pair<18>(st, d, ns, maxcells, capj, vir, eng, cle);
  else if (npoly <= 20) launch_pair<20>(st, d, ns, maxcells, capj, vir, eng, cle);
  else if (npoly <= 24) launch_pair<24>(st, d, ns, maxcells, capj, vir, eng, cle);
  else if (npoly <= 32) launch_pair<32>(st, d, ns, maxcells, capj, vir, eng, cle);
  else launch_pair<MD_MAXPOLY>(st, d, ns, maxcells, capj, vir, eng, cle);
}
```

scema_amd/csrc/md_pair_dev.h:

```cpp
#pragma once
#include <hip/hip_runtime.h>

#include "md_device.h"
#include "md_kernels.h"

#define TW MD_TILE_WAVES
#define TT (TW * 64)
#define NI MD_CLUSTER
#define E_LMASK 0x1FFF
#define E_TYPE_SHIFT 13
#define E_MASK_SHIFT 17
#define E_FAR (1 << 21)
#define CODE_HOME 13

#define XQ_X(S, s) (((const double *)(S).xq)[2 * (size_t)(s)])
#define XQ_Y(S, s) (((const double *)(S).xq)[2 * (size_t)(s) + 1])
#define XQ_Z(S, s) (((const double *)(S).xq)[2 * (size_t)(S).npad + 2 * (size_t)(s)])
#define XQ_Q(S, s) (((const double *)(S).xq)[2 * (size_t)(S).npad + 2 * (size_t)(s) + 1])


__device__ __forceinline__ bool xcd_map(int ntiles, int nsims, int &sim, int &tile) {
  const int L = blockIdx.x;
  const int full = nsims & ~7;
  if (L < full * ntiles) {
    const int x = L & 7, w = L >> 3;
    sim = (w / ntiles) * 8 + x;
    tile = w % ntiles;
  } else {
    const int Lr = L - full * ntiles;
    sim = full + Lr / ntiles;
    tile = Lr % ntiles;
  }
  return sim < nsims;
}

__device__ __forceinline__ int lane_id() { return threadIdx.x & 63; }

__device__ __forceinline__ double rsqrt_f64(double x) {
  const double y = __builtin_amdgcn_rsq(x);
  const double e = fma(-x * y, y, 1.0);
  return fma(y, e * fma(0.375, e, 0.5), y);
}
__device__ __forceinline__ int popc_below(unsigned long long m) {
  return __builtin_amdgcn_mbcnt_hi((unsigned)(m >> 32), __builtin_amdgcn_mbcnt_lo((unsigned)m, 0));
}
template <int CTRL, int ROWMASK>
__device__ __forceinline__ double dpp_keep(double v) {
  const int lo = __builtin_amdgcn_update_dpp(__double2loint(v), __double2loint(v), CTRL, ROWMASK, 0xF, false);
  const int hi = __builtin_amdgcn_update_dpp(__double2hiint(v), __double2hiint(v), CTRL, ROWMASK, 0xF, false);
  return __hiloint2double(hi, lo);
}
__device__ __forceinline__ double wave_max_dpp(double v) {
  SCEMA_ASSERT_FULL_WAVE();
  v = fmax(v, dpp_keep<0x111, 0xF>(v)); v = fmax(v, dpp_keep<0x112, 0xF>(v)); v = fmax(v, dpp_keep<0x114, 0xF>(v)); v = fmax(v, dpp_keep<0x118, 0xF>(v));
  v = fmax(v, dpp_keep<0x142, 0xA>(v));
  v = fmax(v, dpp_keep<0x143, 0xC>(v));
  return __hiloint2double(__builtin_amdgcn_readlane(__double2hiint(v), 63), __builtin_amdgcn_readlane(__double2loint(v), 63));
}
template <int CTRL>
__device__ __forceinline__ double dpp_mov(double v) {
  const int lo = __builtin_amdgcn_update_dpp(0, __double2loint(v), CTRL, 0xF, 0xF, true);
  const int hi = __builtin_amdgcn_update_dpp(0, __double2hiint(v), CTRL, 0xF, 0xF, true);
  return __hiloint2double(hi, lo);
}
#define DPP_QUAD_XOR1 0xB1
// ... 57 lines not shown
```

scema_amd/csrc/md_types.h:

```cpp
#pragma once
#include <stdint.h>

#define MD_MAXCHAIN 8
#define MD_NPART 8
#define MD_MAXTYPES 16
#define MD_MAXPOLY 48
#define MD_TILE_WAVES 8
#define MD_CLUSTER 4
#define MD_JMASK 0x007FFFFF
#define MD_MAXJTAB 8191


#define MD_BOLTZ 0.0019872067
#define MD_MVV2E (48.88821291 * 48.88821291)
#define MD_FTM2V (1.0 / 48.88821291 / 48.88821291)
#define MD_NKTV2P 68568.415
#define MD_QQRD2E 332.06371
#define MD_EWALD_F 1.12837916709551257390
#define MD_PI 3.14159265358979323846

enum { BT_BOND = 0, BT_BOND_SHAKEN = 1, BT_ANGLE = 2, BT_DIHEDRAL = 3, BT_IMPROPER = 4, BT_SPECIAL = 5, BT_NKIND = 6 };
#define BT_DESC 16
#define BT_D_LMASK 0x3FF
#define BT_D_TYPE_SHIFT 40
#define BT_D_TMASK 0xFFF
#define BT_D_LVL_SHIFT 52
#define BT_D_NOCOUNT (1ull << 54)
#define BT_D_KIND_SHIFT 55
#define BT_D_VALID (1ull << 58)
#define BT_MAXCOEF 768
#define BT_OWNERS 192

enum { P_LJ = 0, P_COUL = 1, P_BOND = 2, P_ANGLE = 3, P_DIHEDRAL = 4, P_IMPROPER = 5, P_KSPACE = 6, P_SHAKE = 7 };

struct SimScalars {
  double box[9];
  double box_prev[9];
  double box0[9];
  double vir[MD_NPART * 6];
  double eng[MD_NPART];
  double ke[6];
  double t_current;
  double eta[MD_MAXCHAIN + 1], eta_dot[MD_MAXCHAIN + 1], eta_dotdot[MD_MAXCHAIN + 1], eta_mass[MD_MAXCHAIN + 1];
  double vscale;
  double psum[6];
  double deltasq;
  double far_dsq;
  double corners_hold[24];
  unsigned long long nentries;
  unsigned long long nentries_ref;
  unsigned long long nrowent;
  int nsamples;
  int step;
  int ago;
  int check;
  int rebuild;
  int force_rebuild;
  int overflow;
  int maxneigh_seen;
  int nfar_steps;
  int need_far;
  int maxj_seen;
  int nbuilds;
  int keep_nh;
  int nh_step;
  double t_target_now;
  double omega_dot, omega_mass, mtk_term2;
  double etap[MD_MAXCHAIN + 1], etap_dot[MD_MAXCHAIN + 1], etap_dotdot[MD_MAXCHAIN + 1], etap_mass[MD_MAXCHAIN + 1];
  double dil;
  double cen[3];
  double len0[3];
  double lsum[3], lrun[3];
  int nlwin;
  int pppm_ticket;
  int min_phase, min_stop, min_iter, min_neval, min_newdir, pad2_;
  double min_alpha_now, min_alpha_next;
  double min_alpha, min_alphamax, min_fdothall, min_eorig, min_eprev, min_fhprev, min_engprev, min_alphaprev, min_fh_trial, min_ecur, min_einit;
  double min_dots[4];
#if defined(PAIR_TIMING) || defined(PAIR_COUNT)
  unsigned long long dbg[20];
  unsigned long long dbg2[8];
#endif
};

#if defined(__HIP_DEVICE_COMPILE__)
#define MD_G __attribute__((address_space(1)))
#else
#define MD_G
#endif
struct SimDev {
  int natoms, npad, ntypes;
  int nbonds, nangles, ndihedrals, nimpropers, nspecial, nclus;
  int maxneigh;
  int capj;
  int nc[3], ncells, mst[3];
  int nk, kmaxd[3];
  int nsteps;
  int nav, nwin;
  int nvt, use_shake, deform;
  int t_chain, neigh_delay, shake_maxiter;
  int npt;
  int ramp;
  int nh_total;
  int lavg_nav;
  double t_start, t_stop, p_target, p_freq, box_margin;
  double min_etol, min_ftol, min_dmax;
  int min_maxiter, min_maxeval;
  int min_incremental;
  double dt, t_target, t_freq, tdof, g_ewald, qsqsum, qsum;
  double cut_lj2, cut_coul2, rlist2, skin, excl_cut2, shake_tol;
  double rates[6];
  int coul_npoly;
  double coul_uscale;
  double coul_poly[MD_MAXPOLY];
  double coul_poly_g[MD_MAXPOLY];
  int nfree;
  int keep_list;
  double rlist_ref2;
  double seg_a2, seg_b2;
  double far_band;
  double seg_c2;
  const int MD_G *type;
  const double MD_G *q, *mass;
  const double MD_G *lj;
  const unsigned long long MD_G *bt_terms;
  const double MD_G *bt_coef;
  int bt_ncoef, bt_cf_off[4];
  int nbonds_noshake;
  double sp_w[6];
  const int MD_G *ex_start, *ex_list;
  const int MD_G *bt_desc, *bt_atoms;
  const int MD_G *bt_rank;
  int bt_ntile;
  const int MD_G *clus_at, *clus_n; const double MD_G *clus_d;
  const int MD_G *free_at;
  double MD_G *x, *v, *f;
  double MD_G *fs;
  double MD_G *fb;
  double MD_G *virb;
  int MD_G *slot_of;
  int MD_G *tile_nj;
  int MD_G *tile_order;
  double MD_G *virp;
  int MD_G *tile_wstart;
  int MD_G *tile_jtab;
  double4 MD_G *xq;
  int MD_G *stype;
  int MD_G *perm;
  int MD_G *slot_tmp;
  int MD_G *wrapn;
  double MD_G *xhold;
  int MD_G *cell_of, *ckey, *cell_count, *cell_start, *cell_fill;
  int MD_G *numneigh, *neigh;
  const int MD_G *kn;
  const int MD_G *krun;
  const int MD_G *kgrp;
  int ngrp;
  double MD_G *sfac;
  double MD_G *kvec;
  int pg[3], pad_pg_;
  double MD_G *pgrid;
  double MD_G *pfield;
  long long pgstride;
  double MD_G *pgf;
  SimScalars MD_G *sc;
};
static_assert(sizeof(double MD_G *) == sizeof(double *), "the qualified pointers of SimDev have the size of plain ones: host and device passes see one layout");
```

Before: 461.2 evals/s.

## Split neighbour-row skin into per-cluster displacement bands walked only when reachable

Replaces the single replica-wide far-skin flag with several skin bands per cluster row, stored as cumulative counts. Per-atom displacements since the last rebuild are recorded in a float buffer and quantised into global level flags. The pair kernel then walks only the bands that the cluster's maximum displacement, the replica's bound and the box-corner drift could bring inside the cutoff. The aim is to skip skin entries that cannot interact, at the cost of extra per-step displacement writes, atomics on level flags, a wider count array, and more complex row building.

New measurement: 469.3 evals/s (median of 6 runs). 1.7% higher.

```diff
diff --git a/include/scema_md.h b/include/scema_md.h
--- a/include/scema_md.h
+++ b/include/scema_md.h
@@ -182,6 +182,7 @@
                           double t_start, double t_stop, int32_t npt, double p_target, double p_period, double *lavg);
 int scema_md_debug_compute(scema_md_engine *e, int32_t qp_id, const char *matid, int32_t replica, int32_t use_shake,
                            double *f, double *energies, double *virials, double *info );
+int scema_md_debug_skin_bands(scema_md_engine *e, int32_t pos, uint64_t *out, int32_t cap);
 int scema_md_debug_run(scema_md_engine *e, int32_t qp_id, const char *matid, int32_t replica, int32_t nsteps,
                        double dt, double temperature, int32_t nvt, int32_t use_shake, const double *rates,
                        double *press_avg);
diff --git a/scema_amd/capi.py b/scema_amd/capi.py
--- a/scema_amd/capi.py
+++ b/scema_amd/capi.py
@@ -21,7 +21,7 @@
     "scema_md_strain_batch", "scema_md_strain", "scema_md_local_stress_device_ptr",
     "scema_md_local_stress_count", "scema_md_local_result_doubles", "scema_md_copy_local_stress", "scema_md_scatter_gathered", "scema_md_settle_update", "scema_md_has_state", "scema_md_get_state",
     "scema_md_set_state", "scema_md_drop_state", "scema_md_save_state_file", "scema_md_load_state_file", "scema_md_save_state_lammps",
-    "scema_md_init_material", "scema_md_debug_compute", "scema_md_debug_run", "scema_md_get_profile", "scema_md_env_overrides",
+    "scema_md_init_material", "scema_md_debug_compute", "scema_md_debug_run", "scema_md_debug_skin_bands", "scema_md_get_profile", "scema_md_env_overrides",
     "scema_md_comm_unique_id", "scema_md_comm_init_rccl", "scema_md_comm_init_host", "scema_md_comm_destroy",
     "scema_md_comm_world", "scema_md_comm_rank", "scema_md_comm_stats", "scema_md_comm_handshakes", "scema_md_state_owner", "scema_md_last_plan",
     "scema_plan_dir_create", "scema_plan_dir_destroy", "scema_plan_update", "scema_md_kspace_setup",
@@ -392,6 +392,13 @@
                                            C.c_int32(1 if use_shake else 0), _p(r), _p(pavg)))
         return pavg
 
+    def debug_skin_bands(self, pos=0):
+        out = np.zeros(64, np.uint64)
+        self._chk(lib().scema_md_debug_skin_bands(self.h, C.c_int32(pos), out.ctypes.data_as(C.c_void_p), C.c_int32(out.size)))
+        k = int(out[0])
+        return dict(K=k, listed=[int(v) for v in out[1:1 + k]], walked=[int(v) for v in out[1 + k:1 + 2 * k]],
+                    rows=int(out[1 + 2 * k]), rows_open=int(out[2 + 2 * k]), rows_all_open=int(out[3 + 2 * k]))
+
     def init_material(self, matid, replica, dt=2.0, temperature=300.0, nss=100, strain_ampl=0.005, strain_rate=1e-4):
         p = EqParams(dt, temperature, nss, strain_ampl, strain_rate)
         length, stress, stiff = np.zeros(3), np.zeros(6), np.zeros(36)
diff --git a/scema_amd/csrc/engine/engine.h b/scema_amd/csrc/engine/engine.h
--- a/scema_amd/csrc/engine/engine.h
+++ b/scema_amd/csrc/engine/engine.h
@@ -188,7 +188,7 @@
   int cap_atoms = 0, cap_pad = 0, cap_neigh = 0, cap_cells = 0, cap_k = 0;
   size_t cap_jtab = 0;
   DevBuf virp, virb, fb, fs, slot_of, tile_nj, tile_jtab, tile_order, tile_wstart;
-    DevBuf f, xq, stype, perm, slot_tmp, wrapn, xhold, cell_of, ckey, cell_count, cell_start, cell_fill, numneigh, neigh, sfac, kvec,
+    DevBuf f, xq, stype, perm, slot_tmp, wrapn, xhold, cell_of, ckey, cell_count, cell_start, cell_fill, numneigh, dslot, neigh, sfac, kvec,
       xbak, vbak;
 };
 
@@ -414,6 +414,7 @@
 int collect_faults(scema_md_engine *e, int ns);
 void lists_hold(scema_md_engine *e, const std::vector<ActiveSim> &sims, bool valid, bool counts);
 bool keep_list_switch();
+bool skin_bands_switch();
 void grow_after_overflow(scema_md_engine *e);
 int eval_static(scema_md_engine *e, State *s, const RunSpec &spec);
 
diff --git a/scema_amd/csrc/engine/engine_core.cpp b/scema_amd/csrc/engine/engine_core.cpp
--- a/scema_amd/csrc/engine/engine_core.cpp
+++ b/scema_amd/csrc/engine/engine_core.cpp
@@ -46,6 +46,7 @@
     {"SCEMA_MD_PARTS", "2-4: this many part batches for every launch group that is split, if it has 2 replicas per part (default: by the size of the group, engine_run.cpp)"},
     {"SCEMA_MD_ONE_STREAM", "no side stream (bonded / k-space chain beside the pair kernel)"},
     {"SCEMA_MD_KEEP_LIST", "0: the sampling run of an evaluation rebuilds its neighbour rows at its start even where those of the straining run still hold"},
+    {"SCEMA_MD_SKIN_BANDS", "0: the pair kernel walks every listed entry of a row on every step (default: the skin part of a row only as far as its cluster's and the replica's displacement bounds allow a pair inside the cutoff; results do not depend on it)"},
     {"SCEMA_MD_SKIN_EXTRA", "list skin = params.skin + this many Angstrom (results do not depend on it)"},
     {"SCEMA_MD_SKIN_ADAPT", "1: per-state adaptation of the extra skin from the rebuild interval (round-1 behaviour)"},
     {"SCEMA_MD_PPPM_SOLVE_WIDE", "1 / 0: the in-LDS PPPM solve with 1 024 threads and three LDS grids / 512 threads and two (default: by batch size)"},
diff --git a/scema_amd/csrc/engine/engine_debug.cpp b/scema_amd/csrc/engine/engine_debug.cpp
--- a/scema_amd/csrc/engine/engine_debug.cpp
+++ b/scema_amd/csrc/engine/engine_debug.cpp
@@ -2,6 +2,20 @@
 #include "../md_env.h"
 
 namespace scema_eng {
+
+int skin_band_stats(const scema_md_engine *e, int pos, unsigned long long *out) {
+  const int n = 2 * MD_SKIN_BANDS + 3;
+  unsigned long long *d = nullptr;
+  if (hipMalloc(&d, n * sizeof *d) != hipSuccess) return SCEMA_MD_ERR_DEVICE;
+  hipError_t err = hipMemsetAsync(d, 0, n * sizeof *d, e->stream);
+  if (err == hipSuccess) {
+    mdk_band_stats(e->stream, e->d_sims.as<SimDev>() + pos, d);
+    err = hipMemcpyAsync(out, d, n * sizeof *d, hipMemcpyDeviceToHost, e->stream);
+  }
+  if (err == hipSuccess) err = hipStreamSynchronize(e->stream);
+  (void)hipFree(d);
+  return err == hipSuccess ? SCEMA_MD_OK : SCEMA_MD_ERR_DEVICE;
+}
 
 void print_run_timing(const scema_md_engine *e, int ns, double layout_ms, double kspace_ms, double box_ms, double grid_ms, double rest_ms) {
   if (!scema_env("SCEMA_MD_TIMING") || ns <= 0) return;
@@ -12,7 +26,14 @@
           (double)c.nentries / S0.natoms, c.nbuilds);
   fprintf(stderr, "[scema_md] host: %.2f ms laying out %d simulations before the first launch of this run (k-space set-up on host threads %.2f, box range %.2f, cell grid %.2f, rest of the loop %.2f)\n",
           layout_ms, ns, kspace_ms, box_ms, grid_ms, rest_ms);
-  fprintf(stderr, "[scema_md] sim 0: far skin band walked on %d of %d steps; list skin %.2f A\n", c.nfar_steps, c.step, S0.skin);
+  if (S0.dslot) {
+    unsigned long long bs[2 * MD_SKIN_BANDS + 3];
+    if (skin_band_stats(e, 0, bs) == SCEMA_MD_OK) {
+      fprintf(stderr, "[scema_md] sim 0 after %d steps, list skin %.2f A: skin entries walked / listed per band:", c.step, S0.skin);
+      for (int b = 0; b < MD_SKIN_BANDS; b++) fprintf(stderr, " %llu / %llu", bs[MD_SKIN_BANDS + b], bs[b]);
+      fprintf(stderr, "; rows with skin entries %llu, with a band open %llu, with all open %llu\n", bs[2 * MD_SKIN_BANDS], bs[2 * MD_SKIN_BANDS + 1], bs[2 * MD_SKIN_BANDS + 2]);
+    }
+  }
 #ifdef PAIR_COUNT
   fprintf(stderr, "[scema_md] k_pair lanes (sim 0, this run): %llu wave-chunks (%llu with work); atom blocks run %llu = %.2f per working chunk, %.1f lanes of 64 in them; "
           "LJ block run in %llu of them with %.1f lanes; coulomb block in %llu with %.1f lanes; pairs inside the LJ cutoff %llu, inside the coulomb cutoff %llu\n",
@@ -97,6 +118,17 @@
   return SCEMA_MD_OK;
 }
 
+int scema_md_debug_skin_bands(scema_md_engine *e, int32_t pos, uint64_t *out, int32_t cap) {
+  if (!e || !out || pos < 0 || pos >= (int)e->h_sims.size() || cap < 2 * MD_SKIN_BANDS + 4) return SCEMA_MD_ERR_ARG;
+  if (!e->h_sims[pos].dslot) return fail(e, SCEMA_MD_ERR_ARG, "the last run kept no cluster rows with skin bands");
+  HIPCHK(hipSetDevice(e->p.device));
+  unsigned long long bs[2 * MD_SKIN_BANDS + 3];
+  if (skin_band_stats(e, pos, bs)) return fail(e, SCEMA_MD_ERR_DEVICE, "the statistics launch of the skin bands failed");
+  out[0] = MD_SKIN_BANDS;
+  for (int k = 0; k < 2 * MD_SKIN_BANDS + 3; k++) out[1 + k] = bs[k];
+  return SCEMA_MD_OK;
+}
+
 int scema_md_debug_run(scema_md_engine *e, int32_t qp_id, const char *matid, int32_t replica, int32_t nsteps, double dt,
                        double temperature, int32_t nvt, int32_t use_shake, const double *rates, double *press_avg) {
   if (e) (void)settle_pending(e, false);
diff --git a/scema_amd/csrc/engine/engine_rows.cpp b/scema_amd/csrc/engine/engine_rows.cpp
--- a/scema_amd/csrc/engine/engine_rows.cpp
+++ b/scema_amd/csrc/engine/engine_rows.cpp
@@ -198,6 +198,11 @@
 
 bool keep_list_switch() {
   static const bool on = !(scema_env("SCEMA_MD_KEEP_LIST") && atoi(scema_env("SCEMA_MD_KEEP_LIST")) == 0);
+  return on;
+}
+
+bool skin_bands_switch() {
+  static const bool on = !(scema_env("SCEMA_MD_SKIN_BANDS") && atoi(scema_env("SCEMA_MD_SKIN_BANDS")) == 0);
   return on;
 }
 
@@ -267,7 +272,6 @@
   S.neigh_delay = 0;
   S.tdof = 3.0 * n - 3.0;
   S.skin = N.skin;
-  S.far_band = N.skin;
   e->h_zerotab.push_back(MdkZero{sl.wrapn.as<int>(), 3 * (long long)n});
   if ((rc = stage.bind(pos, A, sl, S, N))) return rc;
   e->h_sims[pos] = S;
diff --git a/scema_amd/csrc/engine/engine_run.cpp b/scema_amd/csrc/engine/engine_run.cpp
--- a/scema_amd/csrc/engine/engine_run.cpp
+++ b/scema_amd/csrc/engine/engine_run.cpp
@@ -24,7 +24,8 @@
     HIPCHK(sl.xq.ensure((size_t)npad * 32));
     HIPCHK(sl.stype.ensure((size_t)npad * 4));
     HIPCHK(sl.perm.ensure((size_t)npad * 4));
-    HIPCHK(sl.numneigh.ensure((size_t)npad * 4));
+    HIPCHK(sl.numneigh.ensure((size_t)(npad / MD_CLUSTER) * MD_BAND_CNT * 2));
+    HIPCHK(sl.dslot.ensure((size_t)npad * 4));
     sl.cap_atoms = natoms;
     sl.cap_pad = npad;
     sl.cap_neigh = 0;
@@ -343,10 +344,15 @@
     const double m = 0.1 * P.skin;
     S.seg_a2 = (P.cut_coul + m) * (P.cut_coul + m);
     S.seg_b2 = (P.cut_lj + m) * (P.cut_lj + m);
-    double frac = 0.65;
-    S.far_band = frac * skin_i;
-    const double cm = std::max(P.cut_coul, P.cut_lj) + S.far_band;
-    S.seg_c2 = cm * cm;
+    const double cmax = std::max(P.cut_coul, P.cut_lj);
+    for (int b = 0; b < MD_SKIN_BANDS; b++) {
+      const double w = m + b * (skin_i - m) / MD_SKIN_BANDS;
+      S.band_e2[b] = (cmax + w) * (cmax + w);
+      S.band_w[b] = skin_down(w);
+    }
+    S.dquant = (float)(skin_i / MD_DLEVELS);
+    S.dquant_inv = (float)(MD_DLEVELS / skin_i);
+    S.skin_bands = skin_bands_switch() ? 1 : 0;
   }
   S.natoms = T.natoms;
   S.npad = padded_slots(T.natoms, S.ncells);
@@ -387,7 +393,7 @@
   S.free_at = T.d_free_at.as<int>(); S.nfree = T.nfree;
   S.xq = sl.xq.as<double4>(); S.stype = sl.stype.as<int>(); S.perm = sl.perm.as<int>(); S.slot_tmp = sl.slot_tmp.as<int>();
   S.cell_of = sl.cell_of.as<int>(); S.ckey = sl.ckey.as<int>(); S.cell_start = sl.cell_start.as<int>();
-  S.cell_fill = sl.cell_fill.as<int>(); S.numneigh = sl.numneigh.as<int>(); S.neigh = sl.neigh.as<int>();
+  S.cell_fill = sl.cell_fill.as<int>(); S.numneigh = sl.numneigh.as<int>(); S.neigh = sl.neigh.as<int>(); S.dslot = sl.dslot.as<float>();
   S.fs = sl.fs.as<double>(); S.fb = sl.fb.as<double>(); S.slot_of = sl.slot_of.as<int>(); S.tile_nj = sl.tile_nj.as<int>(); S.tile_jtab = sl.tile_jtab.as<int>(); S.tile_order = sl.tile_order.as<int>(); S.tile_wstart = sl.tile_wstart.as<int>(); S.virp = sl.virp.as<double>(); S.virb = sl.virb.as<double>();
   S.kvec = sl.kvec.as<double>();
   if (S.nk > 0) {
diff --git a/scema_amd/csrc/md_equil.hip b/scema_amd/csrc/md_equil.hip
--- a/scema_amd/csrc/md_equil.hip
+++ b/scema_amd/csrc/md_equil.hip
@@ -120,9 +120,8 @@
     }
     const double delta = 0.5 * (S.skin - (d1 + d2));
     sc.deltasq = (delta > 0.0) ? delta * delta : -1.0;
-    const double far = 0.5 * (S.far_band - (d1 + d2));
-    sc.far_dsq = (far > 0.0) ? far * far * (1.0 - 1.0e-9) : -1.0;
-    sc.need_far = 0;
+    sc.corner = d1 + d2;
+    sc.walk_all = 1;
     for (int k = 0; k < 6; k++) sc.ke[k] = 0.0;
     for (int k = 0; k < MD_NPART * 6; k++) sc.vir[k] = 0.0;
     for (int k = 0; k < MD_NPART; k++) sc.eng[k] = 0.0;
@@ -161,14 +160,12 @@
     dsq += d * d;
   }
   if (sc.check && dsq > sc.deltasq) sc.rebuild = 1;
-  if (dsq >= sc.far_dsq) sc.need_far = 1;
 }
 
 __global__ void k_post_nh(const SimDev *sims) {
   const SimDev &S = sims[blockIdx.x];
   SimScalars &sc = *S.sc;
   if (threadIdx.x != 0) return;
-  sc.nfar_steps += sc.need_far;
   double f2 = 1.0;
   if (S.npt) {
     const double fp = exp(-0.25 * S.dt * (sc.omega_dot + sc.mtk_term2));
@@ -215,9 +212,8 @@
     sc.check = 1;
     const double delta = 0.5 * S.skin;
     sc.deltasq = delta * delta;
-    const double far = 0.5 * S.far_band;
-    sc.far_dsq = far * far * (1.0 - 1.0e-9);
-    sc.need_far = 0;
+    sc.corner = 0.0;
+    sc.walk_all = 1;
     for (int k = 0; k < 6; k++) sc.ke[k] = 0.0;
     for (int k = 0; k < MD_NPART * 6; k++) sc.vir[k] = 0.0;
     for (int k = 0; k < MD_NPART; k++) sc.eng[k] = 0.0;
@@ -247,7 +243,6 @@
     dsq += d * d;
   }
   if (dsq > sc.deltasq) sc.rebuild = 1;
-  if (dsq >= sc.far_dsq) sc.need_far = 1;
 }
 __global__ __launch_bounds__(TPB) void k_min_reduce(const SimDev *sims, double *const *hs) {
   const SimDev &S = sims[blockIdx.y];
diff --git a/scema_amd/csrc/md_kernels.h b/scema_amd/csrc/md_kernels.h
--- a/scema_amd/csrc/md_kernels.h
+++ b/scema_amd/csrc/md_kernels.h
@@ -9,6 +9,7 @@
 void mdk_neighbor(hipStream_t st, const SimDev *d, int ns, int maxatoms, int maxpad, int maxcells, int maxrow, int capj, bool pack = true, bool together = false);
 void mdk_neigh_build(hipStream_t st, const SimDev *d, int ns, int maxcells, int maxrow, int capj);
 size_t mdk_pair_lds_bytes(int capj);
+void mdk_band_stats(hipStream_t st, const SimDev *d, unsigned long long *out);
 size_t mdk_neigh_lds_bytes(int capj, int maxrow);
 void mdk_pair(hipStream_t st, const SimDev *d, int ns, int maxcells, int capj, int vir, int eng, int npoly, int cle = 0);
 void mdk_bonded(hipStream_t st, const SimDev *d, int ns, int maxtiles, int maxloc, int maxcoef, int parts);
diff --git a/scema_amd/csrc/md_kernels.hip b/scema_amd/csrc/md_kernels.hip
--- a/scema_amd/csrc/md_kernels.hip
+++ b/scema_amd/csrc/md_kernels.hip
@@ -42,9 +42,8 @@
     sc.check = 1;
     sc.rebuild = keep ? 0 : 1;
     sc.force_rebuild = 0;
-    sc.far_dsq = 1.0e300;
-    sc.need_far = keep ? 1 : 0;
-    sc.nfar_steps = 0;
+    sc.corner = 0.0;
+    sc.walk_all = keep ? 1 : 0;
 #if defined(PAIR_TIMING) || defined(PAIR_COUNT)
     for (int k = 0; k < 20; k++) sc.dbg[k] = 0;
     for (int k = 0; k < 8; k++) sc.dbg2[k] = 0;
@@ -105,9 +104,8 @@
     sc.check = (sc.ago >= S.neigh_delay) ? 1 : 0;
     const double delta = 0.5 * (S.skin - (d1 + d2));
     sc.deltasq = delta > 0.0 ? delta * delta : 0.0;
-    const double far = 0.5 * (S.far_band - (d1 + d2));
-    sc.far_dsq = (far > 0.0) ? far * far * (1.0 - 1.0e-9) : -1.0;
-    sc.need_far = 0;
+    sc.corner = d1 + d2;
+    sc.walk_all = 0;
     if (S.nvt) sc.vscale *= nhc_half(S, sc);
     for (int k = 0; k < 6; k++) sc.ke[k] = 0.0;
     for (int k = 0; k < MD_NPART * 6; k++) sc.vir[k] = 0.0;
@@ -157,7 +155,12 @@
     dsq += d * d;
   }
   if (sc.check && dsq > sc.deltasq) sc.rebuild = 1;
-  if (dsq >= sc.far_dsq) sc.need_far = 1;
+  if (S.dslot) {
+    const float dup = sqrtf((float)dsq) * 1.00001f;
+    S.dslot[S.slot_of[i]] = dup;
+    const int lev = skin_level(dup, S.dquant_inv);
+    if (sc.dflag[lev] == 0) sc.dflag[lev] = 1;
+  }
   if (PACK) {
     BoxD b;
     box_derive(sc.box, b);
@@ -187,9 +190,10 @@
   if (blockIdx.x == 0 && threadIdx.x == 0) {
     box_corners(sc.box, sc.corners_hold);
     sc.force_rebuild = 0;
-    sc.far_dsq = 1.0e300;
-    sc.need_far = 0;
-  }
+    sc.corner = 0.0;
+    sc.walk_all = 0;
+  }
+  if (blockIdx.x == 0 && threadIdx.x < MD_DLEVELS) sc.dflag[threadIdx.x] = 0;
   BoxD b;
   box_derive(sc.box, b);
   int nsub[3];
@@ -320,6 +324,7 @@
   if (a < 0) { xy[0] = 1.0e15 + 1.0e6 * (double)s; xy[1] = 1.0e15; zq[0] = 1.0e15; zq[1] = 0.0; S.stype[s] = 0; }
   else { xy[0] = x; xy[1] = y; zq[0] = z; zq[1] = S.q[a]; S.stype[s] = S.type[a]; }
   S.fs[s] = 0.0; S.fs[(size_t)S.npad + s] = 0.0; S.fs[2 * (size_t)S.npad + s] = 0.0;
+  if (S.dslot) S.dslot[s] = 0.0f;
 }
 
 #define CB_TPB 1024
@@ -341,9 +346,10 @@
   if (threadIdx.x == 0) {
     box_corners(sc.box, sc.corners_hold);
     sc.force_rebuild = 0;
-    sc.far_dsq = 1.0e300;
-    sc.need_far = 0;
-  }
+    sc.corner = 0.0;
+    sc.walk_all = 0;
+  }
+  if (threadIdx.x < MD_DLEVELS) sc.dflag[threadIdx.x] = 0;
   BoxD b;
   box_derive(sc.box, b);
   int nsub[3];
@@ -1113,7 +1119,6 @@
   for (int k = threadIdx.x; k < S.ncells; k += blockDim.x) S.cell_count[k] = 0;
 }
 __device__ __forceinline__ void post_scalars(const SimDev &S, SimScalars &sc) {
-  sc.nfar_steps += sc.need_far;
   sc.t_current = (sc.ke[0] + sc.ke[1] + sc.ke[2]) / (S.tdof * MD_BOLTZ);
   double f2 = 1.0;
   if (S.nvt) f2 = nhc_half(S, sc);
diff --git a/scema_amd/csrc/md_neigh.hip b/scema_amd/csrc/md_neigh.hip
--- a/scema_amd/csrc/md_neigh.hip
+++ b/scema_amd/csrc/md_neigh.hip
@@ -23,6 +23,11 @@
 __device__ __forceinline__ float nb_eps(double M, double r2) {
   const double r = sqrt(r2);
   return (float)(1.0001 * 5.9604644775390625e-8 * (96.0 * M * r + 8.0 * r2));
+}
+__device__ __forceinline__ void nb_store_counts(const SimDev &S, int cl, const int *cum) {
+  unsigned short *c = (unsigned short *)S.numneigh + (size_t)MD_BAND_CNT * cl;
+#pragma unroll
+  for (int k = 0; k <= MD_SKIN_BANDS; k++) c[k] = (unsigned short)(cum ? cum[k] : 0);
 }
 __device__ __forceinline__ float nb_up(double t, float eps) { return (float)(t * (1.0 + 2.4e-7)) + eps; }
 
@@ -241,7 +246,7 @@
   }
   if (!runs_ok || nj > capjs || nown / NI > 64 * TW) {
     if (threadIdx.x == 0) { S.tile_nj[cell] = 0; atomicOr(&sc.overflow, 1 | 4); atomicMax(&sc.maxj_seen, runs_ok ? nj : 2 * S.capj); }
-    for (int cl = cs / NI + threadIdx.x; cl < ce / NI; cl += TT) { S.numneigh[2 * cl] = 0; S.numneigh[2 * cl + 1] = 0; }
+    for (int cl = cs / NI + threadIdx.x; cl < ce / NI; cl += TT) nb_store_counts(S, cl, nullptr);
     return;
   }
   if (threadIdx.x == 0) { S.tile_nj[cell] = nj; atomicMax(&sc.maxj_seen, nj); }
@@ -258,15 +263,34 @@
   const unsigned long long tb1 = __builtin_readcyclecounter();
 #endif
   const int maxrow = S.maxneigh;
-  const double ra2 = S.seg_a2, rb2 = fmax(S.seg_a2, S.seg_b2), rc2 = fmax(rb2, S.seg_c2), excl2 = S.excl_cut2;
+  const double ra2 = S.seg_a2, rb2 = fmax(S.seg_a2, S.seg_b2), excl2 = S.excl_cut2;
+  constexpr int KB = MD_SKIN_BANDS, NR = (KB + 2) / 2;
+  double eb2[KB];
+  eb2[0] = rb2;
+#pragma unroll
+  for (int b = 1; b < KB; b++) eb2[b] = fmax(eb2[b - 1], S.band_e2[b]);
   unsigned int npairs = 0, npairs_ref = 0;
   unsigned long long nrowent = 0;
   const bool wider = S.rlist_ref2 < S.rlist2;
   const bool exact = exact_mode == 1 || (exact_mode != 0 && sc.step == 0);
   const bool count_ref = wider && exact && sc.step == 0;
-  const float ra2e = nb_up(ra2, eps), rb2e = nb_up(rb2, eps), rc2e = nb_up(rc2, eps), excl2e = nb_up(excl2, eps);
+  const float ra2e = nb_up(ra2, eps), excl2e = nb_up(excl2, eps);
+  float eb2e[KB];
+#pragma unroll
+  for (int b = 0; b < KB; b++) eb2e[b] = nb_up(eb2[b], eps);
   const GLOBAL_AS int *gjr = (const GLOBAL_AS int *)gj;
-  const int capD = capB >> 2, capBC = capB - capD;
+  int rbnd[NR + 1];
+  {
+    const double v0 = ra2 * sqrt(ra2), vt = rl2 * sqrt(rl2) - v0;
+    rbnd[0] = 0;
+#pragma unroll
+    for (int g = 1; g < NR; g++) {
+      const double e2 = eb2[2 * g - 1];
+      const double share = (vt > 0.0) ? (e2 * sqrt(e2) - v0) / vt : (double)g / NR;
+      rbnd[g] = __builtin_amdgcn_readfirstlane(min(max((int)(share * capB), rbnd[g - 1]), capB));
+    }
+    rbnd[NR] = capB;
+  }
   int nmax = 0, over = 0;
   for (int cl = cs / NI + wave; cl < ce / NI; cl += TW) {
     const int s0slot = cl * NI;
@@ -281,7 +305,7 @@
       ci.x[a] = XQ_X(S, s0slot + a); ci.y[a] = XQ_Y(S, s0slot + a); ci.z[a] = XQ_Z(S, s0slot + a);
     }
     if (ci.atom[0] < 0) {
-      if (lane == 0) { S.numneigh[2 * cl] = 0; S.numneigh[2 * cl + 1] = 0; }
+      if (lane == 0) nb_store_counts(S, cl, nullptr);
       continue;
     }
     GLOBAL_AS int *row = as_global_w(S.neigh) + (size_t)cl * maxrow;
@@ -300,7 +324,9 @@
     }
     const unsigned long long exvalid = __ballot(exv >= 0);
     const bool exlong = max(max(exn[0], exn[1]), max(exn[2], exn[3])) > 16;
-    int nA = 0, nB = 0, nC = 0, nD = 0;
+    int nA = 0, nL[KB + 1];
+#pragma unroll
+    for (int t = 0; t <= KB; t++) nL[t] = 0;
     int qq = 0;
 #pragma unroll
     for (int q = 1; q < NQ; q++) qq += (cl - cs / NI >= (q * nclus_cell) / NQ) ? 1 : 0;
@@ -322,7 +348,7 @@
     bool own_chunks = true;
     const int dump = maxrow - 64 + lane;
     int posA_prev = dump, entA_prev = 0;
-#define NB_CHUNK_TAIL(RMIN, RA, RB, RC, EXCL)                                                                                            \
+#define NB_CHUNK_TAIL(RMIN, RA, EB, EXCL)                                                                                                \
       const int l = lt & 0xFFF;                                                                                                           \
       const int j = jt & MD_JMASK;                                                                                                        \
       if (own_chunks) {                        \
@@ -358,24 +384,35 @@
         }                                                                                                                                 \
       }                                                                                                                                   \
        \
-            \
+                      \
         \
-                          \
+                   \
       {                                                                                                                                   \
         typedef decltype(RMIN) nb_rm_t;                                                                                                   \
         const nb_rm_t rmx = mask ? RMIN : (nb_rm_t)3.0e38f;                                                                               \
-        const bool inA = rmx < RA, inAB = rmx < RB, inABC = rmx < RC, inAll = mask != 0;                                                  \
-        const unsigned long long mA = __ballot(inA), mAB = __ballot(inAB), mABC = __ballot(inABC), mAll = __ballot(inAll);                \
-        const unsigned long long mB = mAB & ~mA, mC = mABC & ~mAB, mD = mAll & ~mABC;                                                     \
-        const int pB = nB + popc_below(mB), pC = capBC - 1 - (nC + popc_below(mC)), pD = capBC + nD + popc_below(mD);                     \
-        const int idx = min(max(inAB ? pB : (inABC ? pC : pD), 0), capB - 1);                                                             \
+        const bool inA = rmx < RA, inAll = mask != 0;                                                                                     \
+        const unsigned long long mA = __ballot(inA), mAll = __ballot(inAll);                                                              \
+                                                         \
+        bool below[KB + 1];                                                                                                               \
+        unsigned long long mbelow[KB + 1];                                                                                                \
+        _Pragma("unroll") for (int t = 0; t < KB; t++) { below[t] = rmx < EB[t]; mbelow[t] = __ballot(below[t]); }                         \
+        below[KB] = inAll; mbelow[KB] = mAll;                                                                                             \
+        int idx = 0;                                                                                                                      \
+        _Pragma("unroll") for (int t = KB; t >= 0; t--) {                                                                                 \
+          const unsigned long long mt = mbelow[t] & ~(t ? mbelow[t - 1] : mA);                                                            \
+          const int pt = nL[t] + popc_below(mt);                                                                                          \
+          const int it = (t & 1) ? rbnd[(t >> 1) + 1] - 1 - pt : rbnd[t >> 1] + pt;                                                       \
+          idx = (t == KB || below[t]) ? it : idx;                                                                                         \
+          nL[t] += __popcll(mt);                                                                                                          \
+        }                                                                                                                                 \
+        idx = min(max(idx, 0), capB - 1);                                                                                                 \
         if (inAll && !inA) lb[idx] = (unsigned short)((base + lane) | (mask << 12));                                                      \
         if (inA) {                                                                                                                        \
           const int pos = nA + popc_below(mA);                                                                                            \
           const int ty = qall ? (int)((unsigned)jt >> 28) : (lt >> 12);                                                                   \
           if (pos < maxrow - 64) { posA_prev = pos; entA_prev = l | (ty << E_TYPE_SHIFT) | (mask << E_MASK_SHIFT); }                      \
         }                                                                                                                                 \
-        nA += __popcll(mA); nB += __popcll(mB); nC += __popcll(mC); nD += __popcll(mD);                                                   \
+        nA += __popcll(mA);                                                                                                               \
       }                                                                                                                                   \
       npairs += __popc(mask);
 
@@ -416,7 +453,7 @@
           }
           const double rmin = vmin_f64(vmin_f64(r2a[0], r2a[1]), vmin_f64(r2a[2], r2a[3]));
           if (!in) { mask = 0; refm = 0; }
-          NB_CHUNK_TAIL(rmin, ra2, rb2, rc2, excl2)
+          NB_CHUNK_TAIL(rmin, ra2, eb2, excl2)
           if (CREF) npairs_ref += __popc(refm);
         }
       };
@@ -444,7 +481,7 @@
           r2a[a] = r2;
         }
         const float rmin = vmin3_f32(vmin_f32(r2a[0], r2a[1]), r2a[2], r2a[3]);
-        NB_CHUNK_TAIL(rmin, ra2e, rb2e, rc2e, excl2e)
+        NB_CHUNK_TAIL(rmin, ra2e, eb2e, excl2e)
       };
       int ltA = list_at(lane), ltB = list_at(64 + lane);
       float xA = s_rx[ltA & 0xFFF], yA = s_ry[ltA & 0xFFF], zA = s_rz[ltA & 0xFFF];
@@ -465,8 +502,14 @@
 #ifdef PAIR_TIMING
     const unsigned long long tr2 = __builtin_readcyclecounter();
 #endif
-    const int n = nA + nB + nC + nD;
-    const bool bad = nB + nC > capBC || nD > capD || n > maxrow - 64;
+    int cum[KB + 1];
+    bool bad = false;
+#pragma unroll
+    for (int t = 0; t <= KB; t++) cum[t] = (t ? cum[t - 1] : nA) + nL[t];
+#pragma unroll
+    for (int g = 0; g < NR; g++) bad = bad || nL[2 * g] + ((2 * g + 1 <= KB) ? nL[2 * g + 1] : 0) > rbnd[g + 1] - rbnd[g];
+    const int n = cum[KB];
+    bad = bad || n > maxrow - 64;
     if (bad) over = 1;
     if (!bad) {
       auto expand = [&](int e16) -> int {
@@ -474,14 +517,14 @@
         const int ty = qall ? (int)((unsigned)gjr[l] >> 28) : (lt >> 12);
         return l | (ty << E_TYPE_SHIFT) | ((e16 >> 12) << E_MASK_SHIFT);
       };
-      for (int k = lane; k < nB; k += 64) row[nA + k] = expand(lb[k]);
-      for (int k = lane; k < nC; k += 64) row[nA + nB + k] = expand(lb[capBC - 1 - k]);
-      for (int k = lane; k < nD; k += 64) row[nA + nB + nC + k] = expand(lb[capBC + k]);
+#pragma unroll
+      for (int t = 0; t <= KB; t++) {
+        const int off = t ? cum[t - 1] : nA;
+        for (int k = lane; k < nL[t]; k += 64) row[off + k] = expand(lb[(t & 1) ? rbnd[(t >> 1) + 1] - 1 - k : rbnd[t >> 1] + k]);
+      }
       if (n + lane < ((n + 63) & ~63)) row[n + lane] = 0;
     }
-    if (lane == 0) {
-      S.numneigh[2 * cl] = bad ? 0 : nA + nB + nC; S.numneigh[2 * cl + 1] = bad ? 0 : nD;
-    }
+    if (lane == 0) nb_store_counts(S, cl, bad ? nullptr : cum);
     nmax = max(nmax, n);
     nrowent += n;
 #ifdef PAIR_TIMING
diff --git a/scema_amd/csrc/md_pair.hip b/scema_amd/csrc/md_pair.hip
--- a/scema_amd/csrc/md_pair.hip
+++ b/scema_amd/csrc/md_pair.hip
@@ -49,7 +49,13 @@
   const int lane = lane_id();
   const int wave = __builtin_amdgcn_readfirstlane(threadIdx.x >> 6);
   const int maxrow = S.maxneigh;
-  const int need_far = __builtin_amdgcn_readfirstlane(S.sc->need_far);
+  float d_gc;
+  {
+    const unsigned long long dflags = __ballot(sc.dflag[lane] != 0);
+    const float d_g = skin_level_bound(dflags ? 63 - __builtin_clzll(dflags) : 0, S.dquant), d_c = skin_up(sc.corner);
+    const bool banded = S.skin_bands != 0 && sc.walk_all == 0;
+    d_gc = __int_as_float(__builtin_amdgcn_readfirstlane(__float_as_int(banded ? (d_g + d_c) * 1.000001f : 3.0e38f)));
+  }
   const int p_begin = S.tile_wstart[(size_t)cell * (TW + 1) + wave], p_end = S.tile_wstart[(size_t)cell * (TW + 1) + wave + 1];
   const int nrows = __builtin_amdgcn_readfirstlane((nj > 0) ? min(p_end - p_begin, 64) : 0);
   if (p_end - p_begin > 64 && lane == 0) atomicOr(&sc.overflow, 1 | 4);
@@ -57,7 +63,12 @@
   if (lane < nrows) {
     const int ent = S.tile_order[2 * (cs / NI) + p_begin + lane];
     h_cl = ent & 0xFFFFF;
-    const int n = S.numneigh[2 * h_cl] + (need_far ? S.numneigh[2 * h_cl + 1] : 0);
+    const unsigned short *cnt = (const unsigned short *)S.numneigh + (size_t)MD_BAND_CNT * h_cl;
+    const float4 dv = *(const float4 *)(S.dslot + (size_t)NI * h_cl);
+    const int nopen = skin_bands_open(fmaxf(fmaxf(dv.x, dv.y), fmaxf(dv.z, dv.w)), d_gc, 0.0f, S.band_w);
+    int n = cnt[0];
+#pragma unroll
+    for (int b = 0; b < MD_SKIN_BANDS; b++) n = (nopen > b) ? (int)cnt[b + 1] : n;
     const int C = (n + 63) >> 6, pa = (ent >> 20) & 31, pb = (ent >> 25) & 31;
     const int kb = 64 * ((C * pa) >> 4), ke = 64 * ((C * pb) >> 4);
     h_nn = (max(ke, kb) << 16) | kb;
@@ -353,6 +364,31 @@
 }
 
 
+__global__ __launch_bounds__(256) void k_band_stats(const SimDev *sim, unsigned long long *out) {
+  const SimDev &S = *sim;
+  const SimScalars &sc = *S.sc;
+  const bool banded = S.skin_bands != 0 && sc.walk_all == 0;
+  int lev = 0;
+  for (int l = 0; l < MD_DLEVELS; l++) if (sc.dflag[l] != 0) lev = l;
+  const float d_g = skin_level_bound(lev, S.dquant), d_c = skin_up(sc.corner);
+  const int nclus = S.cell_start[S.ncells] / NI;
+  for (int cl = blockIdx.x * blockDim.x + threadIdx.x; cl < nclus; cl += gridDim.x * blockDim.x) {
+    const unsigned short *cnt = (const unsigned short *)S.numneigh + (size_t)MD_BAND_CNT * cl;
+    const float4 dv = *(const float4 *)(S.dslot + (size_t)NI * cl);
+    const int nopen = banded ? skin_bands_open(fmaxf(fmaxf(dv.x, dv.y), fmaxf(dv.z, dv.w)), d_g, d_c, S.band_w) : MD_SKIN_BANDS;
+    if (cnt[MD_SKIN_BANDS] == cnt[0]) continue;
+    for (int b = 0; b < MD_SKIN_BANDS; b++) {
+      const unsigned long long nb = (unsigned long long)(cnt[b + 1] - cnt[b]);
+      atomicAdd(&out[b], nb);
+      if (nopen > b) atomicAdd(&out[MD_SKIN_BANDS + b], nb);
+    }
+    atomicAdd(&out[2 * MD_SKIN_BANDS], 1ull);
+    if (nopen > 0) atomicAdd(&out[2 * MD_SKIN_BANDS + 1], 1ull);
+    if (nopen == MD_SKIN_BANDS) atomicAdd(&out[2 * MD_SKIN_BANDS + 2], 1ull);
+  }
+}
+void mdk_band_stats(hipStream_t st, const SimDev *d, unsigned long long *out) { hipLaunchKernelGGL(k_band_stats, dim3(16), dim3(256), 0, st, d, out); }
+
 size_t mdk_pair_lds_bytes(int capj) { return (size_t)capj * (3 * sizeof(double) + sizeof(int)); }
 template <bool VIR, bool ENG, int NP, bool CLE = false>
 static void launch_pair_v(hipStream_t st, const SimDev *d, int ns, int ntiles, int capj) {
diff --git a/scema_amd/csrc/md_pair_dev.h b/scema_amd/csrc/md_pair_dev.h
--- a/scema_amd/csrc/md_pair_dev.h
+++ b/scema_amd/csrc/md_pair_dev.h
@@ -10,7 +10,6 @@
 #define E_LMASK 0x1FFF
 #define E_TYPE_SHIFT 13
 #define E_MASK_SHIFT 17
-#define E_FAR (1 << 21)
 #define CODE_HOME 13
 
 #define XQ_X(S, s) (((const double *)(S).xq)[2 * (size_t)(s)])
diff --git a/scema_amd/csrc/md_skin_bands.h b/scema_amd/csrc/md_skin_bands.h
--- /dev/null
+++ b/scema_amd/csrc/md_skin_bands.h
@@ -0,0 +1,30 @@
+#pragma once
+
+#ifndef MD_SKIN_BANDS
+#define MD_SKIN_BANDS 2
+#endif
+#define MD_BAND_CNT (MD_SKIN_BANDS < 4 ? 4 : (MD_SKIN_BANDS < 8 ? 8 : 16))
+#define MD_DLEVELS 64
+
+#if defined(__HIPCC__) || defined(__CUDACC__)
+#define MD_HD __host__ __device__ __forceinline__
+#else
+#define MD_HD inline
+#endif
+
+MD_HD float skin_up(double v) { return (float)v * 1.000001f; }
+MD_HD float skin_down(double v) { return (float)v * 0.999999f; }
+
+MD_HD int skin_level(float d_up, float inv_quantum) {
+  const int l = (int)(d_up * 1.00001f * inv_quantum) + 1;
+  return l < MD_DLEVELS - 1 ? l : MD_DLEVELS - 1;
+}
+MD_HD float skin_level_bound(int level, float quantum) { return (float)level * quantum * 1.000001f; }
+
+MD_HD int skin_bands_open(float d_i, float d_g, float corner, const float *w) {
+  const float s = ((d_i + d_g) + corner) * 1.000001f;
+  int n = 0;
+#pragma unroll
+  for (int b = 0; b < MD_SKIN_BANDS; b++) n += (s >= w[b]) ? 1 : 0;
+  return n;
+}
diff --git a/scema_amd/csrc/md_types.h b/scema_amd/csrc/md_types.h
--- a/scema_amd/csrc/md_types.h
+++ b/scema_amd/csrc/md_types.h
@@ -1,5 +1,7 @@
 #pragma once
 #include <stdint.h>
+
+#include "md_skin_bands.h"
 
 #define MD_MAXCHAIN 8
 #define MD_NPART 8
@@ -45,7 +47,7 @@
   double vscale;
   double psum[6];
   double deltasq;
-  double far_dsq;
+  double corner;
   double corners_hold[24];
   unsigned long long nentries;
   unsigned long long nentries_ref;
@@ -58,8 +60,8 @@
   int force_rebuild;
   int overflow;
   int maxneigh_seen;
-  int nfar_steps;
-  int need_far;
+  int walk_all;
+  int pad_walk_;
   int maxj_seen;
   int nbuilds;
   int keep_nh;
@@ -77,6 +79,7 @@
   double min_alpha_now, min_alpha_next;
   double min_alpha, min_alphamax, min_fdothall, min_eorig, min_eprev, min_fhprev, min_engprev, min_alphaprev, min_fh_trial, min_ecur, min_einit;
   double min_dots[4];
+  int dflag[MD_DLEVELS];
 #if defined(PAIR_TIMING) || defined(PAIR_COUNT)
   unsigned long long dbg[20];
   unsigned long long dbg2[8];
@@ -118,8 +121,11 @@
   int keep_list;
   double rlist_ref2;
   double seg_a2, seg_b2;
-  double far_band;
-  double seg_c2;
+  double band_e2[MD_SKIN_BANDS];
+  float band_w[MD_SKIN_BANDS];
+  float dquant, dquant_inv;
+  int skin_bands;
+  int pad_bands_;
   const int MD_G *type;
   const double MD_G *q, *mass;
   const double MD_G *lj;
@@ -152,6 +158,7 @@
   double MD_G *xhold;
   int MD_G *cell_of, *ckey, *cell_count, *cell_start, *cell_fill;
   int MD_G *numneigh, *neigh;
+  float MD_G *dslot;
   const int MD_G *kn;
   const int MD_G *krun;
   const int MD_G *kgrp;
```
